# chihyaoma/cyclical-visual-captioning

Hardware: AMD Instinct MI355X
Metric: caption decode-steps/sec (BxT) at N=100,D=2048 (higher is better)
Workload: dtype f32; 1 GPU; cfg2: greedy caption decode; B_per_gpu=64, N=100, F=480, D=2048, A=1024, E=1024, V=5000, T=20, beam=1, hip_graph=True, parallelism=clips sharded over 1 rank(s), no collective, schedule=embedding-gate table (att-LSTM GEMM over K = 2R + one table row per word)

## Files before the change

cyclical-visual-captioning_amd/csrc/blocks.hip:

```cpp
#include <string.h>
#include "cvc_common.h"

namespace {
struct Entry { const char* name; void* fn; };
#define CVC_B(f) {#f, (void*)&f}
const Entry table[] = {
    CVC_B(cvc_attn_scores),
    CVC_B(cvc_attn_wsum),
    CVC_B(cvc_attn_scores_qparts),
    CVC_B(cvc_attn_wsum_quad),
    CVC_B(cvc_attn_wsum_frag),
    CVC_B(cvc_attn_wsum_quad_rm),
    CVC_B(cvc_attn_bwd_pair),
    CVC_B(cvc_ctxfeat_bwd_steps),
    CVC_B(cvc_tile_gemm_big),
    CVC_B(cvc_tile_gemm_plan),
    CVC_B(cvc_dproj_bwd_steps),
    CVC_B(cvc_linear_splitk_fwd),
    CVC_B(cvc_linear_top2_fwd),
    CVC_B(cvc_top2_final),
    CVC_B(cvc_packed_lstm_fwd),
    CVC_B(cvc_packed_linear_fwd),
    CVC_B(cvc_packed_lstm_embgate_fwd),
    CVC_B(cvc_packed_lstm_embgate_ex_fwd),
    CVC_B(cvc_packed_lstm_late_fwd),
    CVC_B(cvc_packed_lstm_train_fwd),
    CVC_B(cvc_packed_lstm_train_pre_fwd),
    CVC_B(cvc_packed_lstm_train_drop_fwd),
    CVC_B(cvc_lstm_pointwise_bwd),
    CVC_B(cvc_lstm_pointwise_bwd3),
    CVC_B(cvc_lstm_pointwise_bwd3_drop),
    CVC_B(cvc_pack_lstm_weights),
    CVC_B(cvc_linear_nn_planes_fwd),
    CVC_B(cvc_linear_nn_planes2_fwd),
    CVC_B(cvc_gru_seq_train_fwd),
    CVC_B(cvc_lstm_pointwise_bwd4_pair),
    CVC_B(cvc_beam_select_parts),
    CVC_B(cvc_sample_select_parts),
    CVC_B(cvc_sample_select_trunc_parts),
    CVC_B(cvc_sample_advance),
    CVC_B(cvc_forced_select_parts),
    CVC_B(cvc_constrained_select_parts),
    CVC_B(cvc_beam_select_hist_parts),
    CVC_B(cvc_beam_select_groups_parts),
    CVC_B(cvc_beam_rank),
    CVC_B(cvc_beam_select_force_parts),
    CVC_B(cvc_beam_rank_force),
    CVC_B(cvc_beam_backtrack_from),
    CVC_B(cvc_tile_lstm_finish),
    CVC_B(cvc_tile_lstm_finish_embgate),
    CVC_B(cvc_tile_reorder_pack),
    CVC_B(cvc_decode_num_launches),
    CVC_B(cvc_gemm_force_generic),
    CVC_B(cvc_tile_gemm_loaders),
    CVC_B(cvc_gru_persistent_waves8),
    CVC_B(cvc_relu_dropout_fwd),
    CVC_B(cvc_relu_dropout_bwd),
    CVC_B(cvc_bn_workspace),
    CVC_B(cvc_bn_relu_train_fwd),
    CVC_B(cvc_bn_relu_train_bwd),
    CVC_B(cvc_class_softmax_bwd),
    CVC_B(cvc_layernorm_cat_bwd),
    CVC_B(cvc_attn_weighted_rows),
    CVC_B(cvc_stable_order),
    CVC_B(cvc_col_sum),
    CVC_B(cvc_col_sum_ws),
    CVC_B(cvc_lstm_persistent_sync_words),
    CVC_B(cvc_lstm_seq_persistent_fwd),
    CVC_B(cvc_lstm_seq_persistent_train_fwd),
    CVC_B(cvc_lstm_seq_fwd),
    CVC_B(cvc_lstm_seq_train_fwd),
    CVC_B(cvc_lstm_seq_bwd_work),
    CVC_B(cvc_lstm_seq_bwd),
    CVC_B(cvc_packed_lstm_bf16w_fwd),
    CVC_B(cvc_packed_linear_bf16w_fwd),
#ifdef CVC_EXPERIMENTAL
    CVC_B(cvc_gsk_plan),
    CVC_B(cvc_gsk_gemm),
    CVC_B(cvc_attn_scores_qslab),
    CVC_B(cvc_top2_slab),
    CVC_B(cvc_packed_lstm_ks_slices),
    CVC_B(cvc_packed_lstm_ks_fwd),
    CVC_B(cvc_packed_lstm_ksf_fwd),
    CVC_B(cvc_packed_lstm_ksx_local),
    CVC_B(cvc_packed_lstm_ksx_fwd),
    CVC_B(cvc_packed_lstm_wg_blocks),
    CVC_B(cvc_packed_linear_select_fwd),
    CVC_B(cvc_gru_persistent_halves),
#endif
};
}

extern "C" void* cvc_block(const char* name) {
    if (name == nullptr) return nullptr;
    for (const Entry& e : table)
        if (strcmp(e.name, name) == 0) return e.fn;
    return nullptr;
}
```

cyclical-visual-captioning_amd/csrc/decode_driver.hip:

```cpp
#include <hip/hip_runtime.h>
#include <new>
#include <stdint.h>
#include "../../include/cvc_hip.h"
#include "../../include/cvc_hip_blocks.h"
#include "../../include/cvc_hip_experimental.h"

struct gsk_launch {
    int U;
    int unit0[2], maxseg[2];
};
struct cvc_decode_plan {
    cvc_decode_desc d;
    int launches;
    gsk_launch ga, go, gl;
};

namespace {

#define CVC_TRY(expr)            \
    do {                         \
        int rc_ = (expr);        \
        ++n;                     \
        if (rc_ != 0) return rc_; \
    } while (0)

inline float* quad_off(float* buf, int k0) { return buf + (size_t)(k0 / 4) * 64 * 4; }
inline void* frag_off(void* xb, int k0) { return (char*)xb + (size_t)(k0 / 16) * 3 * 1024; }

int hip_rc(hipError_t e) { return e == hipSuccess ? 0 : (int)e; }

__global__ __launch_bounds__(256) void reset_kernel(uint4* dst, const uint4* src, size_t n16) {
    const size_t i = (size_t)blockIdx.x * 256 + threadIdx.x;
    if (i < n16) dst[i] = src != nullptr ? src[i] : uint4{0, 0, 0, 0};
}
int reset(void* dst, const void* src, size_t bytes, hipStream_t st) {
    if ((bytes & 15) || ((uintptr_t)dst & 15) || ((uintptr_t)src & 15)) {
        return hip_rc(src ? hipMemcpyAsync(dst, src, bytes, hipMemcpyDeviceToDevice, st) : hipMemsetAsync(dst, 0, bytes, st));
    }
    const size_t n16 = bytes / 16;
    hipLaunchKernelGGL(reset_kernel, dim3((unsigned)((n16 + 255) / 256)), dim3(256), 0, st, (uint4*)dst, (const uint4*)src, n16);
    return hip_rc(hipGetLastError());
}

void attn_sets(const cvc_decode_desc& d, int t, int rows, cvc_attn_set* sets) {
    sets[0] = cvc_attn_set{d.ppool, d.pool, d.mask, nullptr, d.scores_r, nullptr, d.att_steps + (size_t)t * rows * d.N, nullptr,
                           d.N, d.stream_r};
    sets[1] = cvc_attn_set{d.pconv, d.conv, nullptr, nullptr, d.scores_f, nullptr, d.attn_f, nullptr, d.F, d.stream_f};
}

int run_packed(cvc_decode_plan* p, hipStream_t st) {
    const cvc_decode_desc& d = p->d;
    const int rows = d.B, R = d.R, E = d.E, A = d.A, V = d.V, N = d.N;
    const size_t qbytes = (size_t)64 * 4 * sizeof(float);
    int n = 0;
    CVC_TRY(reset(d.xa[0], d.xa0_init, (size_t)((2 * R + E) / 4) * qbytes, st));
    CVC_TRY(reset(d.xl[0], nullptr, (size_t)(3 * R / 4) * qbytes, st));
    CVC_TRY(reset(d.ca[0], nullptr, (size_t)(R / 4) * qbytes, st));
    CVC_TRY(reset(d.cl[0], nullptr, (size_t)(R / 4) * qbytes, st));
    CVC_TRY(reset(d.words, nullptr, (size_t)rows * sizeof(int64_t), st));
    cvc_gemm_seg seg{d.fc, nullptr, d.w_fc, R, R, d.ld_w_fc, 0};
    CVC_TRY(cvc_linear_fwd(&seg, 1, d.b_ih_att, d.b_hh_att, rows, 4 * R, d.gate_fc, 4 * R, st));
    const int nblk_v = (V + 31) / 32;
    for (int t = 0; t < d.T; ++t) {
        const int rd = t & 1, wr = (t + 1) & 1;
        float *XA_r = d.xa[rd], *XA_w = d.xa[wr], *XL_r = d.xl[rd], *XL_w = d.xl[wr];
        CVC_TRY(cvc_packed_lstm_fwd((const float*)d.w_att, XA_r, 2 * R + E, nullptr, nullptr, d.gate_fc, d.ca[rd], rows, R,
                                    quad_off(XL_r, R), quad_off(XA_w, R + E), d.ca[wr], st));
        CVC_TRY(cvc_packed_linear_fwd((const float*)d.w_h, quad_off(XL_r, R), R, nullptr, rows, A, d.qsplit, d.q_parts, A, nullptr, st));
        cvc_attn_set sets[2];
        attn_sets(d, t, rows, sets);
        CVC_TRY(cvc_attn_scores_qparts(d.attn_kind, d.q_parts, d.qsplit, d.b_h, d.w_a, d.b_a, d.inv_temp, sets, 2, d.B, 1, A, st));
        CVC_TRY(cvc_attn_wsum_quad(sets, 2, d.B, 1, R, XL_r, st));
#ifdef CVC_EXPERIMENTAL
        if (d.lang_ksx)
            CVC_TRY(cvc_packed_lstm_ksx_fwd((const float*)d.w_lang, XL_r, 3 * R, d.b_ih_lang, d.b_hh_lang, nullptr, nullptr, nullptr, d.cl[rd],
                                            rows, R, XA_w, quad_off(XL_w, 2 * R), d.cl[wr], d.ksx_slab, d.ksx_flags, (unsigned)(t + 1), st));
        else
#endif
        CVC_TRY(cvc_packed_lstm_fwd((const float*)d.w_lang, XL_r, 3 * R, d.b_ih_lang, d.b_hh_lang, nullptr, d.cl[rd], rows, R, XA_w,
                                    quad_off(XL_w, 2 * R), d.cl[wr], st));
        CVC_TRY(cvc_packed_linear_fwd((const float*)d.w_o, XA_w, R, d.b_o, rows, V, 1, nullptr, V, d.top2_part, st));
        CVC_TRY(cvc_top2_final(d.top2_part, nblk_v, rows, d.unk_idx, d.words + (size_t)(t + 1) * rows, 1,
                               d.logprob ? d.logprob + (size_t)t * rows : nullptr, d.embed, E, quad_off(XA_w, R), 0, st));
    }
    p->launches = n;
    return 0;
}

int run_packed_eg(cvc_decode_plan* p, hipStream_t st) {
    const cvc_decode_desc& d = p->d;
    const int rows = d.B, R = d.R, A = d.A, V = d.V;
    const size_t qbytes = (size_t)64 * 4 * sizeof(float);
    int n = 0;
    CVC_TRY(reset(d.xa[0], nullptr, (size_t)(2 * R / 4) * qbytes, st));
    CVC_TRY(reset(d.xl[0], nullptr, (size_t)(3 * R / 4) * qbytes, st));
    CVC_TRY(reset(d.ca[0], nullptr, (size_t)(R / 4) * qbytes, st));
    CVC_TRY(reset(d.cl[0], nullptr, (size_t)(R / 4) * qbytes, st));
    CVC_TRY(reset(d.words, nullptr, (size_t)rows * sizeof(int64_t), st));
    cvc_gemm_seg seg{d.fc, nullptr, d.w_fc, R, R, d.ld_w_fc, 0};
    CVC_TRY(cvc_linear_fwd(&seg, 1, d.b_ih_att, d.b_hh_att, rows, 4 * R, d.gate_fc, 4 * R, st));
    const long long ws_att = (long long)(2 * R / 4) * 128, ws_lang = (long long)(3 * R / 4) * 128;
    const bool split2 = cvc_gemm_packed_split(-1) == 2;
    for (int t = 0; t < d.T; ++t) {
        const int rd = t & 1, wr = (t + 1) & 1;
        float *XA_r = d.xa[rd], *XA_w = d.xa[wr], *XL_r = d.xl[rd], *XL_w = d.xl[wr];
        const bool first = t == 0 && split2;
        CVC_TRY(cvc_packed_lstm_embgate_ex_fwd((const float*)d.w_att, ws_att, XA_r, first ? 32 : 2 * R, nullptr, nullptr, d.gate_fc,
                                               d.emb_gate, d.words + (size_t)t * rows, d.ca[rd], rows, R, quad_off(XL_r, R),
                                               quad_off(XA_w, R), d.ca[wr], d.att_w_cached, st));
        CVC_TRY(cvc_packed_linear_fwd((const float*)d.w_h, quad_off(XL_r, R), R, nullptr, rows, A, d.qsplit, d.q_parts, A, nullptr, st));
        cvc_attn_set sets[2];
        attn_sets(d, t, rows, sets);
        CVC_TRY(cvc_attn_scores_qparts(d.attn_kind, d.q_parts, d.qsplit, d.b_h, d.w_a, d.b_a, d.inv_temp, sets, 2, d.B, 1, A, st));
        CVC_TRY(cvc_attn_wsum_quad(sets, 2, d.B, 1, R, XL_r, st));
        if (first)
            CVC_TRY(cvc_packed_lstm_late_fwd((const float*)d.w_lang, ws_lang, XL_r, 2 * R, d.b_ih_lang, d.b_hh_lang, nullptr, d.cl[rd], rows,
                                             R, XA_w, quad_off(XL_w, 2 * R), d.cl[wr], nullptr, st));
#ifdef CVC_EXPERIMENTAL
        else if (d.lang_ksx)
            CVC_TRY(cvc_packed_lstm_ksx_fwd((const float*)d.w_lang, XL_r, 3 * R, d.b_ih_lang, d.b_hh_lang, nullptr, nullptr, nullptr, d.cl[rd],
                                            rows, R, XA_w, quad_off(XL_w, 2 * R), d.cl[wr], d.ksx_slab, d.ksx_flags, (unsigned)(t + 1), st));
#endif
        else
        CVC_TRY(cvc_packed_lstm_fwd((const float*)d.w_lang, XL_r, 3 * R, d.b_ih_lang, d.b_hh_lang, nullptr, d.cl[rd], rows, R, XA_w,
                                    quad_off(XL_w, 2 * R), d.cl[wr], st));
        CVC_TRY(cvc_packed_linear_fwd((const float*)d.w_o, XA_w, R, d.b_o, rows, V, 1, nullptr, V, d.top2_part, st));
        CVC_TRY(cvc_top2_final(d.top2_part, (V + 31) / 32, rows, d.unk_idx, d.words + (size_t)(t + 1) * rows, 1,
                               d.logprob ? d.logprob + (size_t)t * rows : nullptr, nullptr, 0, nullptr, 0, st));
    }
    p->launches = n;
    return 0;
}

#ifdef CVC_EXPERIMENTAL
int run_packed_gsk(cvc_decode_plan* p, hipStream_t st) {
    const cvc_decode_desc& d = p->d;
    const int rows = d.B, R = d.R, E = d.E, A = d.A, V = d.V;
    const size_t qbytes = (size_t)64 * 4 * sizeof(float);
    int n = 0;
    CVC_TRY(reset(d.xa[0], d.xa0_init, (size_t)((2 * R + E) / 4) * qbytes, st));
    CVC_TRY(reset(d.xl[0], nullptr, (size_t)(3 * R / 4) * qbytes, st));
    CVC_TRY(reset(d.ca[0], nullptr, (size_t)(R / 4) * qbytes, st));
    CVC_TRY(reset(d.cl[0], nullptr, (size_t)(R / 4) * qbytes, st));
    CVC_TRY(reset(d.words, nullptr, (size_t)rows * sizeof(int64_t), st));
    cvc_gemm_seg seg{d.fc, nullptr, d.w_fc, R, R, d.ld_w_fc, 0};
    CVC_TRY(cvc_linear_fwd(&seg, 1, d.b_ih_att, d.b_hh_att, rows, 4 * R, d.gate_fc, 4 * R, st));
    const long long ws_att = (long long)((2 * R + E) / 4) * 128, ws_lang = (long long)(3 * R / 4) * 128, ws_r = (long long)(R / 4) * 128;
    const float* w_att = (const float*)d.w_att;
    const float* w_lang = (const float*)d.w_lang;
    const int nblk_v = (V + 31) / 32;
    const cvc_gsk_segs seg_att{d.slab_att, p->ga.unit0[0], 2 * R / 32, p->ga.U, p->ga.maxseg[0]};
    const cvc_gsk_segs seg_o_a{d.slab_o, p->ga.unit0[1], R / 32, p->ga.U, p->ga.maxseg[1]};
    const cvc_gsk_segs seg_o_o{d.slab_o, 0, R / 32, p->go.U, p->go.maxseg[0]};
    const cvc_gsk_segs seg_lang{d.slab_lang, p->gl.unit0[0], 2 * R / 32, p->gl.U, p->gl.maxseg[0]};
    const cvc_gsk_segs seg_q{d.slab_q, p->gl.unit0[1], R / 32, p->gl.U, p->gl.maxseg[1]};
    for (int t = 0; t < d.T; ++t) {
        const int rd = t & 1, wr = (t + 1) & 1;
        float *XA_r = d.xa[rd], *XA_w = d.xa[wr], *XL_r = d.xl[rd], *XL_w = d.xl[wr];
        CVC_TRY(cvc_packed_lstm_late_fwd(w_att + (size_t)(R / 4) * 128, ws_att, quad_off(XA_r, R), E, nullptr, nullptr, d.gate_fc,
                                         d.ca[rd], rows, R, quad_off(XL_r, R), quad_off(XA_w, R + E), d.ca[wr],
                                         t == 0 ? nullptr : &seg_att, st));
        cvc_gsk_group gl[2] = {
            {w_lang, ws_lang, XL_r, R / 8, 2 * R / 32, 0, R / 32, d.slab_lang, p->gl.maxseg[0]},
            {(const float*)d.w_h, ws_r, quad_off(XL_r, R), A / 32, R / 32, 0, 0, d.slab_q, p->gl.maxseg[1]}};
        CVC_TRY(cvc_gsk_gemm(gl, 2, p->gl.U, st));
        cvc_attn_set sets[2];
        attn_sets(d, t, rows, sets);
        CVC_TRY(cvc_attn_scores_qslab(d.attn_kind, &seg_q, d.b_h, d.w_a, d.b_a, d.inv_temp, sets, 2, d.B, 1, A, st));
        CVC_TRY(cvc_attn_wsum_quad(sets, 2, d.B, 1, R, XL_r, st));
        CVC_TRY(cvc_packed_lstm_late_fwd(w_lang, ws_lang, XL_r, R, d.b_ih_lang, d.b_hh_lang, nullptr, d.cl[rd], rows, R, XA_w,
                                         quad_off(XL_w, 2 * R), d.cl[wr], &seg_lang, st));
        const bool last = t + 1 == d.T;
        cvc_gsk_group ga[2] = {
            {w_att, ws_att, XA_w, R / 8, 2 * R / 32, R / 32, E / 32, d.slab_att, p->ga.maxseg[0]},
            {(const float*)d.w_o, ws_r, XA_w, nblk_v, R / 32, 0, 0, d.slab_o, last ? p->go.maxseg[0] : p->ga.maxseg[1]}};
        if (last) CVC_TRY(cvc_gsk_gemm(ga + 1, 1, p->go.U, st));
        else CVC_TRY(cvc_gsk_gemm(ga, 2, p->ga.U, st));
        CVC_TRY(cvc_top2_slab(last ? &seg_o_o : &seg_o_a, d.b_o, V, rows, d.unk_idx, d.words + (size_t)(t + 1) * rows, 1,
                              d.logprob ? d.logprob + (size_t)t * rows : nullptr, d.embed, E, quad_off(XA_w, R), 0, st));
    }
    p->launches = n;
    return 0;
}

#endif

int run_tile(cvc_decode_plan* p, hipStream_t st) {
    const cvc_decode_desc& d = p->d;
    const int B = d.B, beam = d.beam, rows = B * beam, R = d.R, E = d.E, A = d.A, V = d.V;
    int n = 0;
    CVC_TRY(reset(d.words, nullptr, (size_t)rows * sizeof(int64_t), st));
    if (beam > 1) {
        CVC_TRY(reset(d.score, nullptr, (size_t)2 * rows * sizeof(float), st));
        CVC_TRY(reset(d.done, nullptr, (size_t)2 * rows, st));
    }
    CVC_TRY(cvc_tile_pack_rows(d.fc, R, nullptr, 0, B, R, d.xff, d.xff_stride, st));
    CVC_TRY(cvc_tile_gemm(d.w_fc_frag, d.xff, d.xff_stride, R, B, 4 * R, d.ks_fc, d.parts_fc, 4 * R, (long long)B * 4 * R, st));
    CVC_TRY(cvc_tile_linear_finish(d.parts_fc, d.ks_fc, (long long)B * 4 * R, 4 * R, d.b_ih_att, d.b_hh_att, B, 4 * R, d.gate_fc,
                                   4 * R, st));
    void* xl_hatt = frag_off(d.xlf, R);
    void* xl_hlang = frag_off(d.xlf, 2 * R);
    const bool eg = d.emb_gate != nullptr;
    const int E_pack = eg ? 0 : E, ka = 2 * R + E_pack;
    CVC_TRY(cvc_tile_reorder_pack(nullptr, d.words, beam, d.zero_state, d.zero_state, d.zero_state, d.zero_state, d.embed, E_pack, V,
                                  d.c_att_prev, d.c_lang_prev, d.xaf, d.xaf_stride, xl_hlang, d.xlf_stride, rows, R, st));
    const long long gs = (long long)rows * 4 * R;
    for (int t = 0; t < d.T; ++t) {
        CVC_TRY(cvc_tile_gemm(d.w_att, d.xaf, d.xaf_stride, ka, rows, 4 * R, d.ks_gate, d.parts_gate, 4 * R, gs, st));
        if (eg)
            CVC_TRY(cvc_tile_lstm_finish_embgate(d.parts_gate, d.ks_gate, gs, nullptr, nullptr, d.gate_fc, beam, d.emb_gate,
                                                 d.words + (size_t)t * rows, V, d.c_att_prev, rows, R, d.c_att, d.h_att, xl_hatt,
                                                 d.xlf_stride, nullptr, 0, st));
        else
            CVC_TRY(cvc_tile_lstm_finish(d.parts_gate, d.ks_gate, gs, nullptr, nullptr, d.gate_fc, beam, d.c_att_prev, rows, R, d.c_att,
                                         d.h_att, xl_hatt, d.xlf_stride, nullptr, 0, st));
        CVC_TRY(cvc_tile_gemm(d.w_h, xl_hatt, d.xlf_stride, R, rows, A, d.ks_q, d.q_parts, A, (long long)rows * A, st));
        CVC_TRY(cvc_tile_linear_finish(d.q_parts, d.ks_q, (long long)rows * A, A, d.b_h, nullptr, rows, A, d.q, A, st));
        cvc_attn_set sets[2];
        attn_sets(d, t, rows, sets);
        CVC_TRY(cvc_attn_scores(d.attn_kind, d.q, d.w_a, d.b_a, d.inv_temp, sets, 2, B, beam, A, st));
        CVC_TRY(cvc_attn_wsum_frag(sets, 2, B, beam, R, d.xlf, d.xlf_stride, st));
        CVC_TRY(cvc_tile_gemm(d.w_lang, d.xlf, d.xlf_stride, 3 * R, rows, 4 * R, d.ks_gate, d.parts_gate, 4 * R, gs, st));
        CVC_TRY(cvc_tile_lstm_finish(d.parts_gate, d.ks_gate, gs, d.b_ih_lang, d.b_hh_lang, nullptr, 1, d.c_lang_prev, rows, R,
                                     d.c_lang, d.h_lang, d.xhf, d.xhf_stride, nullptr, 0, st));
        CVC_TRY(cvc_tile_gemm(d.w_o, d.xhf, d.xhf_stride, R, rows, V, d.ks_o, d.parts_o, V, (long long)rows * V, st));
        static const bool keep_finish = [] { const char* e = getenv("CVC_BEAM_FINISH"); return e && e[0] == '1'; }();
        const bool fused_sel = beam > 1 && !keep_finish && (V & 3) == 0 && (d.ks_o == 2 || d.ks_o == 4 || d.ks_o == 6 || d.ks_o == 8);
        if (!fused_sel)
            CVC_TRY(cvc_tile_linear_finish(d.parts_o, d.ks_o, (long long)rows * V, V, d.b_o, nullptr, rows, V, d.logits, V, st));
        int64_t* word_next = d.words + (size_t)(t + 1) * rows;
        const int64_t* parent = nullptr;
        if (beam == 1) {
            CVC_TRY(cvc_top2_unk(d.logits, rows, V, d.unk_idx, word_next, 1, d.logprob ? d.logprob + (size_t)t * rows : nullptr, st));
        } else {
            const int srd = t & 1, swr = (t + 1) & 1;
            int64_t* par = d.parent + (size_t)t * rows;
            CVC_TRY(cvc_beam_select_parts(fused_sel ? d.parts_o : d.logits, fused_sel ? d.ks_o : 1, fused_sel ? (long long)rows * V : 0,
                                          fused_sel ? d.b_o : nullptr, d.score + (size_t)srd * rows, d.done + (size_t)srd * rows, B, beam, V,
                                          d.unk_idx, t == 0 ? 1 : 0, par, word_next, d.score + (size_t)swr * rows,
                                          d.done + (size_t)swr * rows, d.beam_ws, st));
            parent = par;
        }
        if (t + 1 < d.T)
            CVC_TRY(cvc_tile_reorder_pack(parent, word_next, beam, d.h_att, d.c_att, d.h_lang, d.c_lang, d.embed, E_pack, V, d.c_att_prev,
                                          d.c_lang_prev, d.xaf, d.xaf_stride, xl_hlang, d.xlf_stride, rows, R, st));
    }
    p->launches = n;
    return 0;
}

int validate(const cvc_decode_desc& d) {
    if (d.B < 1 || d.beam < 1 || d.beam > 8 || d.T < 1 || d.N < 1 || d.F < 1 || d.V < 2) return CVC_E_BADARG;
    if (d.attn_kind != CVC_ATTN_ADDITIVE && d.attn_kind != CVC_ATTN_DOT) return CVC_E_BADARG;
    if (!d.fc || !d.conv || !d.pconv || !d.pool || !d.ppool || !d.words || !d.att_steps || !d.embed || !d.b_o || !d.b_h) return CVC_E_BADARG;
    if (d.attn_kind == CVC_ATTN_ADDITIVE && !d.w_a) return CVC_E_BADARG;
    if (!d.w_att || !d.w_lang || !d.w_h || !d.w_o || !d.gate_fc || !d.scores_r || !d.scores_f || !d.attn_f || !d.q_parts) return CVC_E_BADARG;
#ifndef CVC_EXPERIMENTAL
    if (d.gsk_nwg > 0 || d.lang_ksx) return CVC_E_BADARG;
#endif
    if (d.path == 0) {
        if (d.beam != 1 || d.B > 64 || (d.R & 31) || (d.E & 31) || (d.A & 31) || d.qsplit < 1) return CVC_E_BADARG;
        if (!d.w_fc || !d.top2_part || !d.xa[0] || !d.xa[1] || !d.xl[0] || !d.xl[1] || !d.ca[0] || !d.ca[1] || !d.cl[0] || !d.cl[1] ||
            (!d.xa0_init && !d.emb_gate))
            return CVC_E_BADARG;
        if (d.emb_gate != nullptr && d.gsk_nwg > 0) return CVC_E_BADARG;
        if (d.lang_ksx && (!d.ksx_slab || !d.ksx_flags || d.R != 2048 || d.T < 2 || d.gsk_nwg > 0)) return CVC_E_BADARG;
        if (d.gsk_nwg < 0 || (d.gsk_nwg > 0 && ((d.R & 63) || !d.slab_att || !d.slab_lang || !d.slab_q || !d.slab_o))) return CVC_E_BADARG;
    } else if (d.path == 1) {
        if ((d.R & 15) || (d.E & 15) || d.ks_gate < 1 || d.ks_q < 1 || d.ks_o < 1 || d.ks_fc < 1) return CVC_E_BADARG;
        if (!d.w_fc_frag || !d.xaf || !d.xlf || !d.xhf || !d.xff || !d.parts_gate || !d.parts_o || !d.parts_fc || !d.logits || !d.q ||
            !d.h_att || !d.c_att || !d.h_lang || !d.c_lang || !d.c_att_prev || !d.c_lang_prev || !d.zero_state)
            return CVC_E_BADARG;
        if (d.beam > 1 && (!d.score || !d.done || !d.parent || !d.beam_ws)) return CVC_E_BADARG;
    } else {
        return CVC_E_BADARG;
    }
    return 0;
}

}

extern "C" int cvc_decode_plan_create(const cvc_decode_desc* desc, cvc_decode_plan** plan) {
    if (!desc || !plan) return CVC_E_BADARG;
    int rc = validate(*desc);
    if (rc) return rc;
    cvc_decode_plan* p = new (std::nothrow) cvc_decode_plan;
    if (!p) return CVC_E_BADARG;
    p->d = *desc;
    p->launches = 0;
#ifdef CVC_EXPERIMENTAL
    if (desc->path == 0 && desc->gsk_nwg > 0) {
        const int R = desc->R, nt_r = R / 64, nt_v = ((desc->V + 31) / 32 + 7) / 8, nt_a = (desc->A / 32 + 7) / 8;
        const int nta[2] = {nt_r, nt_v}, nca[2] = {2 * R / 32, R / 32};
        const int ntl[2] = {nt_r, nt_a};
        rc = cvc_gsk_plan(nta, nca, 2, desc->gsk_nwg, &p->ga.U, p->ga.unit0, p->ga.maxseg);
        if (!rc) rc = cvc_gsk_plan(nta + 1, nca + 1, 1, desc->gsk_nwg, &p->go.U, p->go.unit0, p->go.maxseg);
        if (!rc) rc = cvc_gsk_plan(ntl, nca, 2, desc->gsk_nwg, &p->gl.U, p->gl.unit0, p->gl.maxseg);
        if (rc) { delete p; return rc; }
    }
#endif
    *plan = p;
    return 0;
}

extern "C" int cvc_decode_plan_set_features(cvc_decode_plan* plan, const float* fc, const float* conv, const float* pconv,
                                            const float* pool, const float* ppool, const uint8_t* mask) {
    if (!plan || !fc || !conv || !pconv || !pool || !ppool) return CVC_E_BADARG;
    plan->d.fc = fc; plan->d.conv = conv; plan->d.pconv = pconv; plan->d.pool = pool; plan->d.ppool = ppool; plan->d.mask = mask;
    return 0;
}

extern "C" void cvc_decode_plan_destroy(cvc_decode_plan* plan) { delete plan; }

extern "C" int cvc_decode_num_launches(const cvc_decode_plan* plan) { return plan ? plan->launches : 0; }

extern "C" int cvc_decode_greedy(cvc_decode_plan* plan, cvc_stream_t stream) {
    if (!plan || plan->d.beam != 1) return CVC_E_BADARG;
    if (plan->d.path == 0) {
        if (plan->d.emb_gate != nullptr) return run_packed_eg(plan, (hipStream_t)stream);
#ifdef CVC_EXPERIMENTAL
        if (plan->d.gsk_nwg > 0) return run_packed_gsk(plan, (hipStream_t)stream);
#endif
        return run_packed(plan, (hipStream_t)stream);
    }
    return run_tile(plan, (hipStream_t)stream);
}

extern "C" int cvc_decode_beam(cvc_decode_plan* plan, cvc_stream_t stream) {
    if (!plan || plan->d.beam < 2 || plan->d.path != 1) return CVC_E_BADARG;
    return run_tile(plan, (hipStream_t)stream);
}
```

cyclical-visual-captioning_amd/csrc/gemm_packed.hip:

```cpp
#include "cvc_common.h"
#include "gemm_split.h"
#include "gsk.h"
#include "dropout_rng.h"

struct PackedArgs {
    const float* wp;
    const float* xq;
    int nquad;
    int M, Nout, R;
    const float* bias;
    const float* bias2;
    const float* gate_bias;
    const float* c_prev_q;
    float* c_out_q;
    float* h_dst1_q;
    float* h_dst2_q;
    float* y;
    int ldy;
    int ksplit;
    long long split_stride;
    float* top2_part;
    const float* c_prev_rm;
    float* h_rm;
    float* c_rm;
    float* gates_rm;
    float* h_rm2;
    float* h_rm3;
    long long gru_w_stride;
    long long gru_h_stride;
    const float* gru_gi[2];
    long long gru_gi_ld;
    float* gru_y[2];
    long long gru_y_ld;
    float* gru_gates[2];
    long long gru_g_ld;
    const float* emb_gate;
    const int64_t* word;
    unsigned* sel_counter;
    int64_t* sel_word; int sel_word_stride; float* sel_logprob; int sel_unk;
    int w_cached;
    DropSpec h3_drop;
    long long wstride;
    GskSegs early;
};

#ifdef CVC_TS
__device__ unsigned long long cvc_ts_buf[2 * 256 * 8 * 4];
extern "C" int cvc_debug_ts_read(unsigned long long* dst) {
    return hipMemcpyFromSymbol(dst, HIP_SYMBOL(cvc_ts_buf), sizeof(cvc_ts_buf)) == hipSuccess ? 0 : -1;
}
#define CVC_TS_MARK(k) do { if (LSTM && !GRU && lane == 0 && blockIdx.x < 256) ts_[k] = wall_clock64(); } while (0)
#else
#define CVC_TS_MARK(k) do {} while (0)
#endif

#ifndef CVC_LIN_W_NT
#define CVC_LIN_W_NT 0
#endif

template <int MT>
struct PFrag {
    f32x4 w[4];
    f32x4 x[MT][4];
#if defined(CVC_PABL) && CVC_PABL == 6
    f32x4 x2[MT][2];
#endif
};
template <int MT>
struct BFrag {
    u32x4 w[2];
    f32x4 x[MT][4];
};

template <int NW>
__device__ __forceinline__ float sum_partials(const float* red, int row, int ldm, int m) {
    float v = (red[(0 * 32 + row) * ldm + m] + red[(1 * 32 + row) * ldm + m]) +
              (red[(2 * 32 + row) * ldm + m] + red[(3 * 32 + row) * ldm + m]);
    if constexpr (NW == 8)
        v += (red[(4 * 32 + row) * ldm + m] + red[(5 * 32 + row) * ldm + m]) +
             (red[(6 * 32 + row) * ldm + m] + red[(7 * 32 + row) * ldm + m]);
    return v;
}

struct SelState { float t1, t2, gm, gs; int j1, j2; };
__device__ __forceinline__ SelState sel_init() { return SelState{-__builtin_inff(), -__builtin_inff(), -__builtin_inff(), 0.f, 0x7fffffff, 0x7fffffff}; }
__device__ __forceinline__ bool sel_better(float va, int ia, float vb, int ib) { return (va > vb) | ((va == vb) & (ia < ib)); }
__device__ __forceinline__ SelState sel_merge(SelState s, float u1, int k1, float u2, int k2, float um, float us) {
    if (sel_better(u1, k1, s.t1, s.j1)) {
        if (sel_better(s.t1, s.j1, u2, k2)) { s.t2 = s.t1; s.j2 = s.j1; } else { s.t2 = u2; s.j2 = k2; }
        s.t1 = u1; s.j1 = k1;
    } else if (sel_better(u1, k1, s.t2, s.j2)) { s.t2 = u1; s.j2 = k1; }
    const float nm = fmaxf(s.gm, um);
    s.gs = (nm == -__builtin_inff()) ? 0.f : s.gs * __expf(s.gm - nm) + us * __expf(um - nm);
    s.gm = nm;
    return s;
}

template <int MT, bool LSTM, int DEPTH, bool SPLIT, int NW, bool GRU = false, int NB = 1, bool SLAB = false, bool WC = false, bool WB16 = false>
__global__ __launch_bounds__(NW * 64) void skinny_gemm_packed_kernel(PackedArgs a) {
    static_assert(!WB16 || (SPLIT && NW == 8 && !GRU && NB == 1 && !SLAB), "bf16-stored weights: 8-wave split-product form only");
    using Frag = std::conditional_t<WB16, BFrag<MT>, PFrag<MT>>;
    using WT = std::conditional_t<WB16, uint16_t, float>;
    static_assert(!GRU || LSTM, "the GRU step shares the LSTM form's work split");
    static_assert(!SLAB || (LSTM && !GRU && NB == 1 && NW == 8), "slab sum: LSTM decode form, 8 waves, one block per workgroup");
    static_assert(NB == 1 || (LSTM && !GRU && NW == 8 && NB == 2), "two blocks per workgroup: LSTM form, 8 waves");
    constexpr int NWK = NW / NB;
    if constexpr (GRU) {
        a.wp += (size_t)blockIdx.y * a.gru_w_stride;
        a.xq += (size_t)blockIdx.y * a.gru_h_stride;
        a.h_dst1_q += (size_t)blockIdx.y * a.gru_h_stride;
        a.bias += (size_t)blockIdx.y * 3 * a.R;
        a.bias2 += (size_t)blockIdx.y * 3 * a.R;
    }
    static_assert(NW == 4 || NW == 8, "4 or 8 waves per workgroup");
    constexpr int LDM = MT * 32 + 1;
    __shared__ float red[(NW + (SLAB ? 1 : 0)) * 32 * LDM + NW * 64 * 6];
    const int tid = threadIdx.x, lane = tid & 63;
    const int wave = __builtin_amdgcn_readfirstlane(tid >> 6);
    const int i = lane & 31, kh = lane >> 5;
    const int M = a.M, R = a.R;
#ifdef CVC_TS
    unsigned long long ts_[4] = {0, 0, 0, 0};
#endif
    CVC_TS_MARK(0);

    int nchunk = a.nquad >> 3, c0 = 0;
    if (!LSTM && a.ksplit > 1) {
        const int lo = nchunk * (int)blockIdx.y / a.ksplit, hi = nchunk * ((int)blockIdx.y + 1) / a.ksplit;
        c0 = lo;
        nchunk = hi - lo;
    }
    const int wblk = NB == 1 ? 0 : wave / NWK, kw = NB == 1 ? wave : wave % NWK;
    const int n_my = nchunk > kw ? (nchunk - kw + NWK - 1) / NWK : 0;
    const WT* wl = reinterpret_cast<const WT*>(a.wp) + (size_t)((int)blockIdx.x * NB + wblk) * a.wstride + (size_t)i * (WB16 ? 8 : 4) +
                   (size_t)(c0 + kw) * 8 * 128 + kh * 4 * 128;
    const float* xl = a.xq + (size_t)i * 4 + (size_t)(c0 + kw) * 8 * 256 + kh * 4 * 256;
    constexpr size_t WSTEP = (size_t)NWK * 8 * 128, XSTEP = (size_t)NWK * 8 * 256;
#ifndef CVC_ROT_MUL
#define CVC_ROT_MUL 5
#endif
    const int rot = n_my > 0 ? (int)((blockIdx.x * CVC_ROT_MUL) % (unsigned)n_my) : 0;

    auto load = [&](Frag& f, int j) __attribute__((always_inline)) {
#if defined(CVC_PABL) && CVC_PABL == 1
        if (j > 0) { asm volatile("" : "+v"(f.w[0])); return; }
#endif
        int jr = j + rot;
        jr = jr >= n_my ? jr - n_my : jr;
        const WT* w = wl + (size_t)jr * WSTEP;
#if defined(CVC_PABL) && CVC_PABL == 4
        const float* x = a.xq + (size_t)i * 4 + kh * 4 * 256;
#else
        const float* x = xl + (size_t)jr * XSTEP;
#endif
        if constexpr (WB16) {
#pragma unroll
            for (int s2 = 0; s2 < 2; ++s2) {
                if constexpr (LSTM && !WC) f.w[s2] = __builtin_nontemporal_load(reinterpret_cast<const u32x4*>(w + s2 * 256));
                else f.w[s2] = *reinterpret_cast<const u32x4*>(w + s2 * 256);
#pragma unroll
                for (int q = 2 * s2; q < 2 * s2 + 2; ++q)
#pragma unroll
                    for (int mt = 0; mt < MT; ++mt) f.x[mt][q] = ld4(x + q * 256 + mt * 128);
            }
        } else {
#pragma unroll
            for (int q = 0; q < 4; ++q) {
                if constexpr (((LSTM && !GRU) || CVC_LIN_W_NT) && !WC) f.w[q] = __builtin_nontemporal_load(reinterpret_cast<const f32x4*>(w + q * 128));
                else f.w[q] = ld4(w + q * 128);
#if defined(CVC_PABL) && CVC_PABL == 3
                if (j > 0) continue;
#endif
#pragma unroll
                for (int mt = 0; mt < MT; ++mt) f.x[mt][q] = ld4(x + q * 256 + mt * 128);
            }
#if defined(CVC_PABL) && CVC_PABL == 6
            {
                int ja = jr + (n_my >> 1);
                ja = ja >= n_my ? ja - n_my : ja;
                const float* xa = xl + (size_t)ja * XSTEP;
#pragma unroll
                for (int s2 = 0; s2 < 2; ++s2)
#pragma unroll
                    for (int mt = 0; mt < MT; ++mt) f.x2[mt][s2] = ld4(xa + (s2 + 2) * 256 + mt * 128 + 64);
            }
#endif
        }
    };

    f32x4 eadd4[4] = {{0, 0, 0, 0}, {0, 0, 0, 0}, {0, 0, 0, 0}, {0, 0, 0, 0}};
    if constexpr (LSTM && !GRU) {
        if (a.emb_gate != nullptr && tid < NB * 2 * 64) {
            const int em0 = tid & 63;
            const long long eword = a.word[em0 < a.M ? em0 : a.M - 1];
            const float* trow = a.emb_gate + (size_t)eword * 4 * a.R + (size_t)((int)blockIdx.x * NB + (tid >> 7)) * 8 + ((tid >> 6) & 1) * 4;
#pragma unroll
            for (int g = 0; g < 4; ++g) eadd4[g] = ld4(trow + (size_t)g * a.R);
        }
    }

    f32x16 acc[MT];
#pragma unroll
    for (int mt = 0; mt < MT; ++mt)
#pragma unroll
        for (int r = 0; r < 16; ++r) acc[mt][r] = 0.f;

    auto mma = [&](const Frag& f) __attribute__((always_inline)) {
        if constexpr (WB16) {
#pragma unroll
            for (int s2 = 0; s2 < 2; ++s2) {
#pragma unroll
                for (int mt = 0; mt < MT; ++mt) {
                    const Split3 X = split8(f.x[mt][2 * s2], f.x[mt][2 * s2 + 1]);
                    acc[mt] = mfma_bf16(f.w[s2], X.lo, acc[mt]);
                    acc[mt] = mfma_bf16(f.w[s2], X.mid, acc[mt]);
                    acc[mt] = mfma_bf16(f.w[s2], X.hi, acc[mt]);
                }
            }
        } else {
#if defined(CVC_PABL) && CVC_PABL >= 2 && CVC_PABL <= 4
#pragma unroll
            for (int q = 0; q < 4; ++q) {
                asm volatile("" ::"v"(f.w[q]));
#pragma unroll
                for (int mt = 0; mt < MT; ++mt) asm volatile("" ::"v"(f.x[mt][q]));
            }
            return;
#endif
            if constexpr (SPLIT) {
#pragma unroll
                for (int s2 = 0; s2 < 2; ++s2) {
                    const Split3 W = split8(f.w[2 * s2], f.w[2 * s2 + 1]);
#pragma unroll
                    for (int mt = 0; mt < MT; ++mt) {
#if defined(CVC_PABL) && (CVC_PABL == 5 || CVC_PABL == 6)
                        Split3 X;
                        X.hi = __builtin_bit_cast(u32x4, f.x[mt][2 * s2]); X.mid = __builtin_bit_cast(u32x4, f.x[mt][2 * s2 + 1]);
#if CVC_PABL == 6
                        X.lo = __builtin_bit_cast(u32x4, f.x2[mt][s2]);
#else
                        X.lo = X.hi;
#endif
#else
                        const Split3 X = split8(f.x[mt][2 * s2], f.x[mt][2 * s2 + 1]);
#endif
                        acc[mt] = mfma_bf16(W.mid, X.mid, acc[mt]);
                        acc[mt] = mfma_bf16(W.lo, X.hi, acc[mt]);
                        acc[mt] = mfma_bf16(W.hi, X.lo, acc[mt]);
                        acc[mt] = mfma_bf16(W.mid, X.hi, acc[mt]);
                        acc[mt] = mfma_bf16(W.hi, X.mid, acc[mt]);
                        acc[mt] = mfma_bf16(W.hi, X.hi, acc[mt]);
                    }
                }
            } else {
#pragma unroll
                for (int q = 0; q < 4; ++q)
#pragma unroll
                    for (int e = 0; e < 4; ++e)
#pragma unroll
                        for (int mt = 0; mt < MT; ++mt)
                            acc[mt] = __builtin_amdgcn_mfma_f32_32x32x2f32(f.w[q][e], f.x[mt][q][e], acc[mt], 0, 0, 0);
            }
        }
    };

    Frag ring[DEPTH];
    if (n_my >= DEPTH) {
#pragma unroll
        for (int s = 0; s < DEPTH - 1; ++s) load(ring[s], s);
        int j = 0;
        for (; j + 2 * DEPTH - 1 <= n_my; j += DEPTH) {
#pragma unroll
            for (int s = 0; s < DEPTH; ++s) {
                load(ring[(s + DEPTH - 1) % DEPTH], j + s + DEPTH - 1);
                mma(ring[s]);
#ifdef CVC_TS
                if (s == 0 && j == 0) CVC_TS_MARK(1);
// ... 15 lines not shown
#pragma unroll
                    for (int g = 0; g < 4 + 4 * MT; ++g) {
                        __builtin_amdgcn_sched_group_barrier(0x002, 18, 0);
                        __builtin_amdgcn_sched_group_barrier(0x008, MT, 0);
                        __builtin_amdgcn_sched_group_barrier(0x020, 1, 0);
                    }
                } else {
#pragma unroll
                    for (int g = 0; g < 4 + 4 * MT; ++g) {
                        __builtin_amdgcn_sched_group_barrier(0x008, 2, 0);
                        __builtin_amdgcn_sched_group_barrier(0x020, 1, 0);
                        __builtin_amdgcn_sched_group_barrier(0x002, 2, 0);
                    }
                }
                __builtin_amdgcn_sched_barrier(0);
            }
        }
#pragma unroll
        for (int s = 0; s < DEPTH; ++s) {
            if (j + s + DEPTH - 1 < n_my) load(ring[(s + DEPTH - 1) % DEPTH], j + s + DEPTH - 1);
            if (j + s < n_my) mma(ring[s]);
        }
#pragma unroll
        for (int s = 0; s < DEPTH - 1; ++s)
            if (j + DEPTH + s < n_my) mma(ring[s]);
    } else {
        for (int j = 0; j < n_my; ++j) {
            load(ring[0], j);
            mma(ring[0]);
        }
    }

    CVC_TS_MARK(2);
    const int em = tid & 63, eqd = (tid >> 6) & 1, eb = tid >> 7;
    const bool ework = LSTM && tid < NB * 2 * 64 && em < M && em < MT * 32;
    const int ejq = ((int)blockIdx.x * NB + eb) * 8 + eqd * 4;
    const float* ered = red + (NB == 1 ? 0 : eb * NWK * 32 * LDM);
    const size_t eqoff = ((size_t)(ejq / 4) * 64 + em) * 4;
    f32x4 ecp = {0, 0, 0, 0}, eadd[4] = {{0, 0, 0, 0}, {0, 0, 0, 0}, {0, 0, 0, 0}, {0, 0, 0, 0}};
    f32x4 eadd2[4] = {{0, 0, 0, 0}, {0, 0, 0, 0}, {0, 0, 0, 0}, {0, 0, 0, 0}}, eadd3[4] = {{0, 0, 0, 0}, {0, 0, 0, 0}, {0, 0, 0, 0}, {0, 0, 0, 0}};

    if (GRU && ework) {
        const float* gi = (blockIdx.y == 0 ? a.gru_gi[0] : a.gru_gi[1]) + (size_t)em * a.gru_gi_ld + ejq;
        ecp = ld4(a.xq + eqoff);
#pragma unroll
        for (int g = 0; g < 3; ++g) {
            eadd[g] = ld4(gi + g * R) + ld4(a.bias + g * R + ejq);
            if (g < 2) eadd[g] += ld4(a.bias2 + g * R + ejq);
        }
        eadd[3] = ld4(a.bias2 + 2 * R + ejq);
    } else if (ework) {
        ecp = a.c_prev_rm != nullptr ? ld4(a.c_prev_rm + (size_t)em * R + ejq) : ld4(a.c_prev_q + eqoff);
        if (a.bias != nullptr) {
#pragma unroll
            for (int g = 0; g < 4; ++g) eadd[g] = ld4(a.bias + g * R + ejq);
        }
        if (a.bias2 != nullptr) {
#pragma unroll
            for (int g = 0; g < 4; ++g) eadd2[g] = ld4(a.bias2 + g * R + ejq);
        }
        if (a.gate_bias != nullptr) {
#pragma unroll
            for (int g = 0; g < 4; ++g) eadd3[g] = ld4(a.gate_bias + (size_t)em * 4 * R + g * R + ejq);
        }
    }

    constexpr int SLAB_MAXS = 10;
    f32x4 sv[SLAB ? SLAB_MAXS : 1];
    int s_nseg = 0;
    const float* s_p0 = nullptr;
    if constexpr (SLAB) {
        const int tile = (int)blockIdx.x >> 3, j = (int)blockIdx.x & 7;
        s_nseg = gsk_nseg(a.early, tile);
        s_p0 = gsk_part(a.early, tile, 0, j) + (size_t)tid * 4;
#pragma unroll
        for (int s = 0; s < SLAB_MAXS; ++s) sv[s] = ld4(s_p0 + (size_t)(s < s_nseg ? s : s_nseg - 1) * (8 * 2048));
    }

    constexpr int ECPW = 32 / NW;
    float ebias[ECPW];
#pragma unroll
    for (int c = 0; c < ECPW; ++c) {
        const int n = (int)blockIdx.x * 32 + wave * ECPW + c;
        ebias[c] = (!LSTM && a.top2_part != nullptr && a.bias != nullptr) ? a.bias[n < a.Nout ? n : a.Nout - 1] : 0.f;
    }

#pragma unroll
    for (int mt = 0; mt < MT; ++mt)
#pragma unroll
        for (int r = 0; r < 16; ++r) {
            const int row = (r & 3) + 8 * (r >> 2) + 4 * kh;
            red[(wave * 32 + row) * LDM + mt * 32 + i] = acc[mt][r];
        }
    if constexpr (SLAB) {
        f32x4 t = sv[0];
#pragma unroll
        for (int s = 1; s < SLAB_MAXS; ++s) t += s < s_nseg ? sv[s] : f32x4{0.f, 0.f, 0.f, 0.f};
        for (int s = SLAB_MAXS; s < s_nseg; ++s) t += ld4(s_p0 + (size_t)s * (8 * 2048));
        if ((tid >> 3) < MT * 32) {
#pragma unroll
            for (int e = 0; e < 4; ++e) red[(NW * 32 + (tid & 7) * 4 + e) * LDM + (tid >> 3)] = t[e];
        }
    }
    __syncthreads();

    if constexpr (GRU) {
        if (ework) {
            f32x4 hv, gr, gz, gn, gh;
#pragma unroll
            for (int e = 0; e < 4; ++e) {
                const int jj = eqd * 4 + e;
                float pre[3];
#pragma unroll
                for (int g = 0; g < 3; ++g) pre[g] = sum_partials<NWK>(ered, g * 8 + jj, LDM, em);
                const float rg = fast_sigmoid(pre[0] + eadd[0][e]), zg = fast_sigmoid(pre[1] + eadd[1][e]);
                const float hn = pre[2] + eadd[3][e];
                const float ng = fast_tanh(eadd[2][e] + rg * hn);
                hv[e] = ng + zg * (ecp[e] - ng);
                gr[e] = rg; gz[e] = zg; gn[e] = ng; gh[e] = hn;
            }
            st4(a.h_dst1_q + eqoff, hv);
            st4((blockIdx.y == 0 ? a.gru_y[0] : a.gru_y[1]) + (size_t)em * a.gru_y_ld + ejq, hv);
            float* gp = blockIdx.y == 0 ? a.gru_gates[0] : a.gru_gates[1];
            if (gp != nullptr) {
                gp += (size_t)em * a.gru_g_ld + ejq;
                st4(gp, gr); st4(gp + a.R, gz); st4(gp + 2 * a.R, gn); st4(gp + 3 * a.R, gh);
            }
        }
    } else if (LSTM) {
        if (ework) {
            f32x4 hv, cv, gv[4];
#pragma unroll
            for (int g = 0; g < 4; ++g) eadd[g] = ((eadd[g] + eadd2[g]) + eadd3[g]) + eadd4[g];
#pragma unroll
            for (int e = 0; e < 4; ++e) {
                const int jj = eqd * 4 + e;
                float pre[4];
#pragma unroll
                for (int g = 0; g < 4; ++g) {
                    float sp = sum_partials<NWK>(ered, g * 8 + jj, LDM, em);
                    if constexpr (SLAB) sp += red[(NW * 32 + g * 8 + jj) * LDM + em];
                    pre[g] = sp + eadd[g][e];
                }
                const float ig = fast_sigmoid(pre[0]), fg = fast_sigmoid(pre[1]);
                const float gg = fast_tanh(pre[2]), og = fast_sigmoid(pre[3]);
                const float c2 = fg * ecp[e] + ig * gg;
                cv[e] = c2;
                hv[e] = og * fast_tanh(c2);
                gv[0][e] = ig; gv[1][e] = fg; gv[2][e] = gg; gv[3][e] = og;
            }
            if (a.c_out_q != nullptr) st4(a.c_out_q + eqoff, cv);
            if (a.h_dst1_q != nullptr) st4(a.h_dst1_q + eqoff, hv);
            if (a.h_dst2_q != nullptr) st4(a.h_dst2_q + eqoff, hv);
            if (a.h_rm != nullptr) st4(a.h_rm + (size_t)em * R + ejq, hv);
            if (a.h_rm2 != nullptr) st4(a.h_rm2 + (size_t)em * R + ejq, hv);
            if (a.h_rm3 != nullptr) {
                f32x4 hd = hv;
                if (a.h3_drop.state != nullptr) {
                    const uint32_t s0 = a.h3_drop.state[0], s1 = a.h3_drop.state[1], s2 = a.h3_drop.state[2];
                    const uint32_t i0 = (uint32_t)em * (uint32_t)R + (uint32_t)ejq;
#pragma unroll
                    for (int e = 0; e < 4; ++e) hd[e] *= cvc_drop_mult(a.h3_drop, s0, s1, s2, i0 + e);
                }
                st4(a.h_rm3 + (size_t)em * R + ejq, hd);
            }
            if (a.c_rm != nullptr) st4(a.c_rm + (size_t)em * R + ejq, cv);
            if (a.gates_rm != nullptr) {
#pragma unroll
                for (int g = 0; g < 4; ++g) st4(a.gates_rm + (size_t)em * 4 * R + g * R + ejq, gv[g]);
            }
        }
#ifdef CVC_TS
        asm volatile("s_waitcnt vmcnt(0)" ::: "memory");
        CVC_TS_MARK(3);
        if (lane == 0 && blockIdx.x < 256) {
            unsigned long long* d = cvc_ts_buf + ((size_t)((a.nquad >= 1536 ? 0 : 1) * 256 + blockIdx.x) * 8 + wave) * 4;
            d[0] = ts_[0]; d[1] = ts_[1]; d[2] = ts_[2]; d[3] = ts_[3];
        }
#endif
    } else {
        const int n0 = blockIdx.x * 32;
        const bool lead = blockIdx.y == 0;
        float* y = a.y != nullptr ? a.y + (long long)blockIdx.y * a.split_stride : nullptr;
        if (y != nullptr) {
            for (int u = tid; u < 32 * MT * 32; u += NW * 64) {
                const int nl = u & 31, m = u >> 5;
                const int n = n0 + nl;
                if (m >= M || n >= a.Nout) continue;
                float v = sum_partials<NW>(red, nl, LDM, m);
                if (lead && a.bias != nullptr) v += a.bias[n];
                y[(size_t)m * a.ldy + n] = v;
            }
        }
        if (a.top2_part != nullptr) {
            float* scratch = red + NW * 32 * LDM;
            float v1 = -__builtin_inff(), v2 = -__builtin_inff(), mx = -__builtin_inff(), se = 0.f;
            int i1 = 0x7fffffff, i2 = 0x7fffffff;
            const int m = lane < MT * 32 ? lane : MT * 32 - 1;
            constexpr int CPW = 32 / NW;
#pragma unroll
            for (int c = 0; c < CPW; ++c) {
                const int nl = wave * CPW + c, n = n0 + nl;
                if (n >= a.Nout) break;
                const float v = sum_partials<NW>(red, nl, LDM, m) + ebias[c];
                if (v > v1) { v2 = v1; i2 = i1; v1 = v; i1 = n; }
                else if (v > v2) { v2 = v; i2 = n; }
                const float nm = fmaxf(mx, v);
                se = se * __expf(mx - nm) + __expf(v - nm);
                mx = nm;
            }
            float* r4 = scratch + ((size_t)wave * 64 + lane) * 6;
            r4[0] = v1; r4[1] = __int_as_float(i1); r4[2] = v2; r4[3] = __int_as_float(i2); r4[4] = mx; r4[5] = se;
            __syncthreads();
            if (wave == 0 && lane < M) {
                for (int w = 1; w < NW; ++w) {
                    const float* q4 = scratch + ((size_t)w * 64 + lane) * 6;
                    const float u1 = q4[0], u2 = q4[2];
                    const int k1 = __float_as_int(q4[1]), k2 = __float_as_int(q4[3]);
                    if (u1 > v1) { if (v1 >= u2) { v2 = v1; i2 = i1; } else { v2 = u2; i2 = k2; } v1 = u1; i1 = k1; }
                    else if (u1 > v2) { v2 = u1; i2 = k1; }
                    const float nm = fmaxf(mx, q4[4]);
                    se = (nm == -__builtin_inff()) ? 0.f : se * __expf(mx - nm) + q4[5] * __expf(q4[4] - nm);
                    mx = nm;
                }
                float* rec = a.top2_part + ((size_t)blockIdx.x * 64 + lane) * 6;
                if (a.sel_counter != nullptr) {
                    const float r6[6] = {v1, __int_as_float(i1), v2, __int_as_float(i2), mx, se};
#pragma unroll
                    for (int k = 0; k < 6; ++k) __hip_atomic_store(rec + k, r6[k], __ATOMIC_RELAXED, __HIP_MEMORY_SCOPE_AGENT);
                } else {
                    rec[0] = v1; rec[1] = __int_as_float(i1); rec[2] = v2; rec[3] = __int_as_float(i2); rec[4] = mx; rec[5] = se;
                }
            }
            if (a.sel_counter != nullptr) {
                asm volatile("s_waitcnt vmcnt(0)" ::: "memory");
                __syncthreads();
                int* flag = reinterpret_cast<int*>(scratch);
                if (tid == 0) {
                    const unsigned old = __hip_atomic_fetch_add(a.sel_counter, 1u, __ATOMIC_RELAXED, __HIP_MEMORY_SCOPE_AGENT);
                    const bool last = old == gridDim.x - 1;
                    if (last) {
                        __hip_atomic_store(a.sel_counter, 0u, __ATOMIC_RELAXED, __HIP_MEMORY_SCOPE_AGENT);
                        __builtin_amdgcn_fence(__ATOMIC_ACQUIRE, "agent");
                    }
                    flag[0] = last ? 1 : 0;
                }
                __syncthreads();
                if (flag[0] == 0) return;
                __syncthreads();
                const int nb = (int)gridDim.x;
                SelState ss = sel_init();
                const int mrow = lane < M ? lane : M - 1;
                constexpr int RB = 8;
                for (int b0 = wave; b0 < nb; b0 += NW * RB) {
                    f32x2 r0[RB], r1[RB], r2[RB];
#pragma unroll
                    for (int k = 0; k < RB; ++k) {
                        const int b = b0 + k * NW;
                        const f32x2* q2 = reinterpret_cast<const f32x2*>(a.top2_part + ((size_t)(b < nb ? b : nb - 1) * 64 + mrow) * 6);
                        r0[k] = q2[0]; r1[k] = q2[1]; r2[k] = q2[2];
                    }
#pragma unroll
                    for (int k = 0; k < RB; ++k)
                        if (b0 + k * NW < nb) ss = sel_merge(ss, r0[k].x, __float_as_int(r0[k].y), r1[k].x, __float_as_int(r1[k].y), r2[k].x, r2[k].y);
                }
                float* r8 = scratch + ((size_t)wave * 64 + lane) * 6;
                r8[0] = ss.t1; r8[1] = __int_as_float(ss.j1); r8[2] = ss.t2; r8[3] = __int_as_float(ss.j2); r8[4] = ss.gm; r8[5] = ss.gs;
                __syncthreads();
                if (wave == 0 && lane < M) {
                    for (int w = 1; w < NW; ++w) {
                        const float* q4 = scratch + ((size_t)w * 64 + lane) * 6;
                        ss = sel_merge(ss, q4[0], __float_as_int(q4[1]), q4[2], __float_as_int(q4[3]), q4[4], q4[5]);
                    }
                    const bool use2 = (ss.j1 == a.sel_unk) && ss.j2 != 0x7fffffff;
                    int wsel = use2 ? ss.j2 : ss.j1;
                    if (wsel == 0x7fffffff || wsel < 0) wsel = 0;
                    a.sel_word[(size_t)lane * a.sel_word_stride] = wsel;
// ... 308 lines not shown
    long long ldx[6];
    int nseg, M;
    float* xq;
};

__global__ __launch_bounds__(256) void pack_quad_segs_kernel(PackXArgs a) {
    const int t = blockIdx.x * 256 + threadIdx.x;
    const int m = t & 63, q = t >> 6;
    if (q >= a.q_end[a.nseg - 1]) return;
    int s = 0;
#pragma unroll
    for (int i = 0; i < 5; ++i) s += (i < a.nseg - 1 && q >= a.q_end[i]) ? 1 : 0;
    const int qs = q - (s ? a.q_end[s - 1] : 0);
    f32x4 v = {0, 0, 0, 0};
    if (m < a.M) v = ld4(a.x[s] + (size_t)m * a.ldx[s] + qs * 4);
    st4(a.xq + ((size_t)q * 64 + m) * 4, v);
}

}

extern "C" int cvc_pack_lstm_segs(const float* const* ws, const long long* lds, const int* widths, int nseg, int R, float* wp,
                                  cvc_stream_t stream) {
    if (!ws || !lds || !widths || !wp || nseg < 1 || nseg > 4 || R < 8 || (R & 7)) return CVC_E_BADARG;
    PackWArgs a{};
    int q = 0;
    for (int s = 0; s < nseg; ++s) {
        if (!ws[s] || widths[s] < 4 || (widths[s] & 3) || lds[s] < widths[s] || (lds[s] & 3) || ((uintptr_t)ws[s] & 15)) return CVC_E_BADARG;
        q += widths[s] / 4;
        a.w[s] = ws[s]; a.ld[s] = lds[s]; a.q_end[s] = q;
    }
    if (q & 7) return CVC_E_BADARG;
    a.nseg = nseg; a.R = R; a.wp = wp;
    hipLaunchKernelGGL(pack_lstm_w_kernel, dim3(R / 8, (q + 63) / 64), dim3(256), 0, (hipStream_t)stream, a);
    return cvc_launch_status();
}

extern "C" int cvc_pack_lstm_weights(const float* w_ih, int K_ih, const float* w_hh, int K_hh, int R, float* wp,
                                     cvc_stream_t stream) {
    if (!w_ih || !w_hh || !wp || K_ih < 4 || K_hh < 4 || (K_ih & 3) || (K_hh & 3) || ((K_ih + K_hh) & 31) || R < 8 || (R & 7))
        return CVC_E_BADARG;
    const float* ws[2] = {w_ih, w_hh};
    const long long lds[2] = {K_ih, K_hh};
    const int widths[2] = {K_ih, K_hh};
    return cvc_pack_lstm_segs(ws, lds, widths, 2, R, wp, stream);
}

extern "C" int cvc_pack_quad_segs(const float* const* xs, const long long* ldx, const int* widths, int nseg, int M, float* xq,
                                  cvc_stream_t stream) {
    if (!xs || !ldx || !widths || !xq || nseg < 1 || nseg > 6 || M < 1 || M > 64) return CVC_E_BADARG;
    PackXArgs a{};
    int q = 0;
    for (int s = 0; s < nseg; ++s) {
        if (!xs[s] || widths[s] < 4 || (widths[s] & 3) || (ldx[s] & 3) || ((uintptr_t)xs[s] & 15)) return CVC_E_BADARG;
        q += widths[s] / 4;
        a.x[s] = xs[s]; a.ldx[s] = ldx[s]; a.q_end[s] = q;
    }
    a.nseg = nseg; a.M = M; a.xq = xq;
    hipLaunchKernelGGL(pack_quad_segs_kernel, dim3((q * 64 + 255) / 256), dim3(256), 0, (hipStream_t)stream, a);
    return cvc_launch_status();
}

extern "C" int cvc_packed_linear_select_fwd(const float* wp, const float* xq, int K, const float* bias, int M, int Nout,
                                            float* top2_part, unsigned* counter, int unk_idx, int64_t* word, int word_stride,
                                            float* logprob, cvc_stream_t stream) {
    if (!wp || !xq || (K & 31) || Nout < 2 || !top2_part || !counter || !word || word_stride < 1 || M < 1 || M > 64) return CVC_E_BADARG;
    PackedArgs a{};
    a.wp = wp; a.xq = xq; a.nquad = K / 4; a.M = M; a.Nout = Nout; a.R = 0;
    a.bias = bias; a.ksplit = 1; a.top2_part = top2_part;
    a.sel_counter = counter; a.sel_unk = unk_idx; a.sel_word = word; a.sel_word_stride = word_stride; a.sel_logprob = logprob;
    return launch_packed<false>(a, (Nout + 31) / 32, (hipStream_t)stream);
}

extern "C" int cvc_packed_linear_fwd(const float* wp, const float* xq, int K, const float* bias, int M, int Nout,
                                     int ksplit, float* y, int ldy, float* top2_part, cvc_stream_t stream) {
    if (!wp || !xq || (K & 31) || Nout < 1 || ksplit < 1 || (!y && !top2_part)) return CVC_E_BADARG;
    if (ksplit > 1 && top2_part != nullptr) return CVC_E_BADARG;
    if (y != nullptr && ldy < Nout) return CVC_E_BADARG;
    PackedArgs a{};
    a.wp = wp; a.xq = xq; a.nquad = K / 4; a.M = M; a.Nout = Nout; a.R = 0;
    a.bias = bias; a.y = y; a.ldy = ldy; a.ksplit = ksplit; a.split_stride = (long long)M * ldy; a.top2_part = top2_part;
    return launch_packed<false>(a, (Nout + 31) / 32, (hipStream_t)stream);
}

extern "C" int cvc_packed_linear_bf16w_fwd(const uint16_t* wp, const float* xq, int K, const float* bias, int M, int Nout,
                                           int ksplit, float* y, int ldy, float* top2_part, cvc_stream_t stream) {
    if (!wp || !xq || (K & 31) || K < 32 || Nout < 1 || ksplit < 1 || (!y && !top2_part) || M < 1 || M > 64) return CVC_E_BADARG;
    if (ksplit > 1 && top2_part != nullptr) return CVC_E_BADARG;
    if (y != nullptr && ldy < Nout) return CVC_E_BADARG;
    if (((uintptr_t)wp & 15) || ((uintptr_t)xq & 15)) return CVC_E_BADARG;
    PackedArgs a{};
    a.wp = reinterpret_cast<const float*>(wp); a.xq = xq; a.nquad = K / 4; a.M = M; a.Nout = Nout; a.R = 0;
    a.bias = bias; a.y = y; a.ldy = ldy; a.ksplit = ksplit; a.split_stride = (long long)M * ldy; a.top2_part = top2_part;
    return launch_packed_bf16w<false>(a, (Nout + 31) / 32, (hipStream_t)stream);
}
```

cyclical-visual-captioning_amd/csrc/vocab.hip:

```cpp
#include "row_block.h"
#include "gsk.h"
#include "dropout_rng.h"
#include <math.h>

namespace {

__global__ __launch_bounds__(WG) void embed_relu_fwd_kernel(const float* table, const int64_t* idx, const float* drop, DropSpec rng,
                                                            int M, int E, float* out) {
    const int m = blockIdx.y;
    const int e = (blockIdx.x * WG + threadIdx.x) * 4;
    if (e >= E) return;
    f32x4 v = ld4(table + (size_t)idx[m] * E + e);
    v.x = fmaxf(v.x, 0.f); v.y = fmaxf(v.y, 0.f); v.z = fmaxf(v.z, 0.f); v.w = fmaxf(v.w, 0.f);
    if (drop != nullptr) v *= ld4(drop + (size_t)m * E + e);
    if (rng.state != nullptr) {
        const uint32_t s0 = rng.state[0], s1 = rng.state[1], s2 = rng.state[2], i0 = (uint32_t)m * (uint32_t)E + (uint32_t)e;
#pragma unroll
        for (int k = 0; k < 4; ++k) v[k] *= cvc_drop_mult(rng, s0, s1, s2, i0 + k);
    }
    st4(out + (size_t)m * E + e, v);
}

__global__ __launch_bounds__(WG) void dropout_rng_kernel(const float* x, DropSpec rng, size_t n, float* y) {
    const size_t i = ((size_t)blockIdx.x * WG + threadIdx.x) * 4;
    if (i >= n) return;
    const uint32_t s0 = rng.state[0], s1 = rng.state[1], s2 = rng.state[2];
    if (i + 4 <= n) {
        f32x4 v = ld4(x + i);
#pragma unroll
        for (int k = 0; k < 4; ++k) v[k] *= cvc_drop_mult(rng, s0, s1, s2, (uint32_t)(i + k));
        st4(y + i, v);
    } else {
        for (size_t k = i; k < n; ++k) y[k] = x[k] * cvc_drop_mult(rng, s0, s1, s2, (uint32_t)k);
    }
}

constexpr int EMB_CHUNK = 16;

__global__ __launch_bounds__(WG) void embed_bwd_pieces_kernel(const int64_t* idx, const int64_t* order, const float* drop, DropSpec rng,
                                                              const float* d_out, int M, int E, float* part) {
    const int r0 = blockIdx.y * EMB_CHUNK;
    const int e = (blockIdx.x * WG + threadIdx.x) * 4;
    if (e >= E) return;
    const int r1 = min(M, r0 + EMB_CHUNK);
    int start = r0;
    int64_t w = idx[order[r0]];
    f32x4 acc = {0, 0, 0, 0};
    for (int r = r0; r < r1; ++r) {
        const int64_t m = order[r];
        const int64_t wr = idx[m];
        if (wr != w) {
            st4(part + (size_t)start * E + e, acc);
            acc = f32x4{0, 0, 0, 0};
            start = r;
            w = wr;
        }
        f32x4 g = ld4(d_out + (size_t)m * E + e);
        if (drop != nullptr) g *= ld4(drop + (size_t)m * E + e);
        if (rng.state != nullptr) {
            const uint32_t s0 = rng.state[0], s1 = rng.state[1], s2 = rng.state[2], i0 = (uint32_t)m * (uint32_t)E + (uint32_t)e;
#pragma unroll
            for (int k = 0; k < 4; ++k) g[k] *= cvc_drop_mult(rng, s0, s1, s2, i0 + k);
        }
        acc += g;
    }
    st4(part + (size_t)start * E + e, acc);
}

__global__ __launch_bounds__(WG) void embed_bwd_runs_kernel(const float* table, const int64_t* idx, const int64_t* order,
                                                            const float* part, int M, int E, float* d_table) {
    const int r0 = blockIdx.y;
    const int64_t w = idx[order[r0]];
    if (r0 > 0 && idx[order[r0 - 1]] == w) return;
    const int e = (blockIdx.x * WG + threadIdx.x) * 4;
    if (e >= E) return;
    f32x4 acc = ld4(part + (size_t)r0 * E + e);
    for (int r = (r0 / EMB_CHUNK + 1) * EMB_CHUNK; r < M && idx[order[r]] == w; r += EMB_CHUNK)
        acc += ld4(part + (size_t)r * E + e);
    const f32x4 t = ld4(table + (size_t)w * E + e);
    acc.x = t.x > 0.f ? acc.x : 0.f; acc.y = t.y > 0.f ? acc.y : 0.f;
    acc.z = t.z > 0.f ? acc.z : 0.f; acc.w = t.w > 0.f ? acc.w : 0.f;
    st4(d_table + (size_t)w * E + e, ld4(d_table + (size_t)w * E + e) + acc);
}
// ... 49 lines not shown
    const int row = blockIdx.x;
    const float* x = logits + (size_t)row * V;
    Top2 t{-INFINITY, 0x7fffffff, -INFINITY, 0x7fffffff};
    for (int v = threadIdx.x; v < V; v += WG) {
        const float xv = x[v];
        if (better(xv, v, t.v1, t.i1)) { t.v2 = t.v1; t.i2 = t.i1; t.v1 = xv; t.i1 = v; }
        else if (better(xv, v, t.v2, t.i2)) { t.v2 = xv; t.i2 = v; }
    }
#pragma unroll
    for (int o = 32; o > 0; o >>= 1) {
        Top2 u;
        u.v1 = __shfl_xor(t.v1, o, 64); u.i1 = __shfl_xor(t.i1, o, 64);
        u.v2 = __shfl_xor(t.v2, o, 64); u.i2 = __shfl_xor(t.i2, o, 64);
        t = merge(t, u);
    }
    const int lane = threadIdx.x & 63, wave = threadIdx.x >> 6;
    if (lane == 0) tred[wave] = t;
    __syncthreads();
    t = merge(merge(tred[0], tred[1]), merge(tred[2], tred[3]));
    const float m = t.v1;
    float s = 0.f;
    for (int v = threadIdx.x; v < V; v += WG) s += expf(x[v] - m);
    s = block_sum(s, red);
    if (threadIdx.x == 0) {
        const bool use2 = (t.i1 == unk) && V > 1;
        int w = use2 ? t.i2 : t.i1;
        if ((unsigned)w >= (unsigned)V) w = 0;
        word[(size_t)row * wstride] = w;
        if (logprob != nullptr) logprob[row] = (use2 ? t.v2 : t.v1) - (m + logf(s));
    }
}

__global__ __launch_bounds__(WG) void top2_final_kernel(const float* part, int nblocks, int unk, int64_t* word, int wstride,
                                                        float* logprob, const float* table, int E, float* emb_out, int emb_ld) {
    __shared__ float red[4];
    __shared__ Top2 tred[4];
    __shared__ int chosen;
    const int row = blockIdx.x;
    Top2 t{-INFINITY, 0x7fffffff, -INFINITY, 0x7fffffff};
    float mx = -INFINITY;
    for (int b = threadIdx.x; b < nblocks; b += WG) {
        const float* rec = part + ((size_t)b * 64 + row) * 6;
        Top2 u{rec[0], __float_as_int(rec[1]), rec[2], __float_as_int(rec[3])};
        t = merge(t, u);
        mx = fmaxf(mx, rec[4]);
    }
#pragma unroll
    for (int o = 32; o > 0; o >>= 1) {
        Top2 u;
        u.v1 = __shfl_xor(t.v1, o, 64); u.i1 = __shfl_xor(t.i1, o, 64);
        u.v2 = __shfl_xor(t.v2, o, 64); u.i2 = __shfl_xor(t.i2, o, 64);
        t = merge(t, u);
    }
    const int lane = threadIdx.x & 63, wave = threadIdx.x >> 6;
    if (lane == 0) tred[wave] = t;
    mx = block_max(mx, red);
    t = merge(merge(tred[0], tred[1]), merge(tred[2], tred[3]));
    float se = 0.f;
    for (int b = threadIdx.x; b < nblocks; b += WG) {
        const float* rec = part + ((size_t)b * 64 + row) * 6;
        se += rec[5] * expf(rec[4] - mx);
    }
    se = block_sum(se, red);
    if (threadIdx.x == 0) {
        const bool use2 = (t.i1 == unk) && t.i2 != 0x7fffffff;
        int w = use2 ? t.i2 : t.i1;
        if (w == 0x7fffffff || w < 0) w = 0;
        word[(size_t)row * wstride] = w;
        if (logprob != nullptr) logprob[row] = (use2 ? t.v2 : t.v1) - (mx + logf(se));
        chosen = w;
    }
    if (emb_out != nullptr) {
        __syncthreads();
        const float* src = table + (size_t)chosen * E;
        for (int e = threadIdx.x * 4; e < E; e += WG * 4) {
            f32x4 v = ld4(src + e);
            v.x = fmaxf(v.x, 0.f); v.y = fmaxf(v.y, 0.f); v.z = fmaxf(v.z, 0.f); v.w = fmaxf(v.w, 0.f);
            if (emb_ld > 0) st4(emb_out + (size_t)row * emb_ld + e, v);
            else st4(emb_out + ((size_t)(e >> 2) * 64 + row) * 4, v);
        }
    }
}

template <int ITEMS>
__global__ __launch_bounds__(WG) void top2_slab_kernel(GskSegs g, const float* bias, int V, int unk, int64_t* word, int wstride,
                                                       float* logprob, const float* table, int E, float* emb_out, int emb_ld) {
    __shared__ float red[4];
    __shared__ Top2 tred[4];
    __shared__ int chosen;
    constexpr int MAXS = 6;
    const int row = blockIdx.x;
    const int nitem = ((V + 31) >> 5) * 8;
    f32x4 sv[ITEMS][MAXS], bv[ITEMS];
    int nseg[ITEMS], col0[ITEMS];
    const float* p0[ITEMS];
#pragma unroll
    for (int k = 0; k < ITEMS; ++k) {
        const int it = min((int)threadIdx.x + k * WG, nitem - 1);
        const int blk = it >> 3, rq = it & 7;
        nseg[k] = gsk_nseg(g, blk >> 3);
        col0[k] = (int)threadIdx.x + k * WG < nitem ? blk * 32 + rq * 4 : V;
        p0[k] = gsk_part(g, blk >> 3, 0, blk & 7) + (size_t)row * 32 + rq * 4;
#pragma unroll
        for (int s = 0; s < MAXS; ++s) sv[k][s] = ld4(p0[k] + (size_t)(s < nseg[k] ? s : nseg[k] - 1) * (8 * 2048));
#pragma unroll
        for (int e = 0; e < 4; ++e) bv[k][e] = (bias != nullptr && col0[k] + e < V) ? bias[col0[k] + e] : 0.f;
    }
    Top2 t{-INFINITY, 0x7fffffff, -INFINITY, 0x7fffffff};
    float mx = -INFINITY;
    f32x4 val[ITEMS];
#pragma unroll
    for (int k = 0; k < ITEMS; ++k) {
        f32x4 x = sv[k][0];
#pragma unroll
        for (int s = 1; s < MAXS; ++s) x += s < nseg[k] ? sv[k][s] : f32x4{0.f, 0.f, 0.f, 0.f};
        for (int s = MAXS; s < nseg[k]; ++s) x += ld4(p0[k] + (size_t)s * (8 * 2048));
        x += bv[k];
#pragma unroll
        for (int e = 0; e < 4; ++e) {
            const int v = col0[k] + e;
            const float xv = v < V ? x[e] : -INFINITY;
            val[k][e] = xv;
            if (v < V) {
                if (better(xv, v, t.v1, t.i1)) { t.v2 = t.v1; t.i2 = t.i1; t.v1 = xv; t.i1 = v; }
                else if (better(xv, v, t.v2, t.i2)) { t.v2 = xv; t.i2 = v; }
                mx = fmaxf(mx, xv);
            }
        }
    }
#pragma unroll
    for (int o = 32; o > 0; o >>= 1) {
        Top2 u;
        u.v1 = __shfl_xor(t.v1, o, 64); u.i1 = __shfl_xor(t.i1, o, 64);
        u.v2 = __shfl_xor(t.v2, o, 64); u.i2 = __shfl_xor(t.i2, o, 64);
        t = merge(t, u);
    }
    const int lane = threadIdx.x & 63, wave = threadIdx.x >> 6;
    if (lane == 0) tred[wave] = t;
    mx = block_max(mx, red);
    t = merge(merge(tred[0], tred[1]), merge(tred[2], tred[3]));
    float se = 0.f;
#pragma unroll
    for (int k = 0; k < ITEMS; ++k)
#pragma unroll
        for (int e = 0; e < 4; ++e) se += val[k][e] == -INFINITY ? 0.f : expf(val[k][e] - mx);
    se = block_sum(se, red);
    if (threadIdx.x == 0) {
        const bool use2 = (t.i1 == unk) && t.i2 != 0x7fffffff;
        int w = use2 ? t.i2 : t.i1;
        if (w == 0x7fffffff || w < 0) w = 0;
        word[(size_t)row * wstride] = w;
        if (logprob != nullptr) logprob[row] = (use2 ? t.v2 : t.v1) - (mx + logf(se));
        chosen = w;
    }
    if (emb_out != nullptr) {
        __syncthreads();
        const float* src = table + (size_t)chosen * E;
        for (int e = threadIdx.x * 4; e < E; e += WG * 4) {
            f32x4 v = ld4(src + e);
            v.x = fmaxf(v.x, 0.f); v.y = fmaxf(v.y, 0.f); v.z = fmaxf(v.z, 0.f); v.w = fmaxf(v.w, 0.f);
            if (emb_ld > 0) st4(emb_out + (size_t)row * emb_ld + e, v);
            else st4(emb_out + ((size_t)(e >> 2) * 64 + row) * 4, v);
        }
    }
}

// ... 126 lines not shown
    hipLaunchKernelGGL(embed_relu_fwd_kernel, dim3((E / 4 + WG - 1) / WG, M), dim3(WG), 0, (hipStream_t)stream, table, idx,
                       drop, rng, M, E, out);
    return cvc_launch_status();
}

static int embed_bwd_impl(const float* table, const int64_t* idx, const int64_t* order, const float* drop, DropSpec rng,
                          const float* d_out, int M, int E, float* d_table, float* workspace, cvc_stream_t stream) {
    if (!table || !idx || !order || !d_out || !d_table || !workspace || M < 1 || E < 4 || (E & 3)) return CVC_E_BADARG;
    const int gx = (E / 4 + WG - 1) / WG;
    hipLaunchKernelGGL(embed_bwd_pieces_kernel, dim3(gx, (M + EMB_CHUNK - 1) / EMB_CHUNK), dim3(WG), 0, (hipStream_t)stream, idx,
                       order, drop, rng, d_out, M, E, workspace);
    hipLaunchKernelGGL(embed_bwd_runs_kernel, dim3(gx, M), dim3(WG), 0, (hipStream_t)stream, table, idx, order, workspace, M, E,
                       d_table);
    return cvc_launch_status();
}

extern "C" int cvc_embed_relu_fwd(const float* table, const int64_t* idx, const float* drop, int M, int E, float* out,
                                  cvc_stream_t stream) {
    return embed_fwd_impl(table, idx, drop, cvc_drop_spec(nullptr, 0, 0.f), M, E, out, stream);
}

extern "C" int cvc_embed_relu_bwd(const float* table, const int64_t* idx, const int64_t* order, const float* drop,
                                  const float* d_out, int M, int E, float* d_table, float* workspace, cvc_stream_t stream) {
    return embed_bwd_impl(table, idx, order, drop, cvc_drop_spec(nullptr, 0, 0.f), d_out, M, E, d_table, workspace, stream);
}

extern "C" int cvc_embed_relu_rng_fwd(const float* table, const int64_t* idx, const uint32_t* rng_state, unsigned site, float p, int M,
                                      int E, float* out, cvc_stream_t stream) {
    if (!rng_state || p < 0.f || p >= 1.f) return CVC_E_BADARG;
    return embed_fwd_impl(table, idx, nullptr, cvc_drop_spec(rng_state, site, p), M, E, out, stream);
}

extern "C" int cvc_embed_relu_rng_bwd(const float* table, const int64_t* idx, const int64_t* order, const uint32_t* rng_state,
                                      unsigned site, float p, const float* d_out, int M, int E, float* d_table, float* workspace,
                                      cvc_stream_t stream) {
    if (!rng_state || p < 0.f || p >= 1.f) return CVC_E_BADARG;
    return embed_bwd_impl(table, idx, order, nullptr, cvc_drop_spec(rng_state, site, p), d_out, M, E, d_table, workspace, stream);
}

extern "C" int cvc_dropout_rng(const float* x, long long n, const uint32_t* rng_state, unsigned site, float p, float* y,
                               cvc_stream_t stream) {
    if (!x || !y || !rng_state || n < 1 || n > 0xffffffffll || p < 0.f || p >= 1.f || ((uintptr_t)x & 15) || ((uintptr_t)y & 15))
        return CVC_E_BADARG;
    hipLaunchKernelGGL(dropout_rng_kernel, dim3((unsigned)((n / 4 + WG) / WG)), dim3(WG), 0, (hipStream_t)stream, x,
                       cvc_drop_spec(rng_state, site, p), (size_t)n, y);
    return cvc_launch_status();
}

extern "C" int cvc_log_softmax_fwd(const float* logits, int M, int V, float* logp, cvc_stream_t stream) {
    if (!logits || !logp || M < 1 || V < 1) return CVC_E_BADARG;
    hipLaunchKernelGGL(log_softmax_kernel, dim3(M), dim3(WG), 0, (hipStream_t)stream, logits, V, logp);
    return cvc_launch_status();
}

extern "C" int cvc_log_softmax_bwd(const float* logp, const float* d_logp, int M, int V, float* d_logits,
                                   cvc_stream_t stream) {
    if (!logp || !d_logp || !d_logits || M < 1 || V < 1) return CVC_E_BADARG;
    hipLaunchKernelGGL(log_softmax_bwd_kernel, dim3(M), dim3(WG), 0, (hipStream_t)stream, logp, d_logp, V, d_logits);
    return cvc_launch_status();
}

extern "C" int cvc_nll_bwd(const int64_t* target, const float* w, const float* g, int M, int V, float* d_logp,
                           cvc_stream_t stream) {
    if (!target || !w || !g || !d_logp || M < 1 || V < 1) return CVC_E_BADARG;
    hipLaunchKernelGGL(nll_bwd_kernel, dim3((V + WG - 1) / WG, M), dim3(WG), 0, (hipStream_t)stream, target, w, g, V, d_logp);
    return cvc_launch_status();
}

extern "C" int cvc_top2_unk(const float* logits, int M, int V, int unk_idx, int64_t* word, int word_stride,
                            float* logprob, cvc_stream_t stream) {
    if (!logits || !word || M < 1 || V < 1 || word_stride < 1) return CVC_E_BADARG;
    hipLaunchKernelGGL(top2_unk_kernel, dim3(M), dim3(WG), 0, (hipStream_t)stream, logits, V, unk_idx, word, word_stride,
                       logprob);
    return cvc_launch_status();
}

extern "C" int cvc_top2_final(const float* part, int nblocks, int M, int unk_idx, int64_t* word, int word_stride,
                              float* logprob, const float* table, int E, float* emb_out, int emb_ld,
                              cvc_stream_t stream) {
    if (!part || !word || nblocks < 1 || M < 1 || M > 64 || word_stride < 1) return CVC_E_BADARG;
    if (emb_out != nullptr && (!table || E < 4 || (E & 3) || (emb_ld & 3) || (emb_ld != 0 && emb_ld < E))) return CVC_E_BADARG;
    hipLaunchKernelGGL(top2_final_kernel, dim3(M), dim3(WG), 0, (hipStream_t)stream, part, nblocks, unk_idx, word, word_stride,
                       logprob, table, E, emb_out, emb_ld);
    return cvc_launch_status();
}

extern "C" int cvc_top2_slab(const cvc_gsk_segs* logits, const float* bias, int V, int M, int unk_idx, int64_t* word,
                             int word_stride, float* logprob, const float* table, int E, float* emb_out, int emb_ld,
                             cvc_stream_t stream) {
    if (!logits || !logits->slab || logits->nchunk < 1 || logits->U < 1 || logits->maxseg < 1 || logits->unit0 < 0 || !word || V < 2 ||
        M < 1 || M > 64 || word_stride < 1)
        return CVC_E_BADARG;
    if (emb_out != nullptr && (!table || E < 4 || (E & 3) || (emb_ld & 3) || (emb_ld != 0 && emb_ld < E))) return CVC_E_BADARG;
    const int nitem = ((V + 31) / 32) * 8;
    hipStream_t st = (hipStream_t)stream;
    if (nitem <= 5 * WG)
        hipLaunchKernelGGL(top2_slab_kernel<5>, dim3(M), dim3(WG), 0, st, *logits, bias, V, unk_idx, word, word_stride, logprob, table, E,
                           emb_out, emb_ld);
    else if (nitem <= 8 * WG)
        hipLaunchKernelGGL(top2_slab_kernel<8>, dim3(M), dim3(WG), 0, st, *logits, bias, V, unk_idx, word, word_stride, logprob, table, E,
                           emb_out, emb_ld);
    else
        return CVC_E_TOOBIG;
    return cvc_launch_status();
}

extern "C" int cvc_nll_fwd(const float* logp, const int64_t* target, const float* w, int M, int V, float* loss_sum,
                           cvc_stream_t stream) {
    if (!logp || !target || !w || !loss_sum || M < 1 || V < 1) return CVC_E_BADARG;
    hipLaunchKernelGGL(nll_fwd_kernel, dim3(1), dim3(WG), 0, (hipStream_t)stream, logp, target, w, M, V, loss_sum);
    return cvc_launch_status();
}

extern "C" int cvc_vocab_nll_fwd(const float* logits, const int64_t* target, const float* w, int M, int V, float* lse,
                                 int64_t* argmax, float* row_loss, float* loss_sum, cvc_stream_t stream) {
    if (!logits || !target || !w || !lse || !row_loss || !loss_sum || M < 1 || V < 1) return CVC_E_BADARG;
    hipLaunchKernelGGL(vocab_nll_fwd_kernel, dim3(M), dim3(WG), 0, (hipStream_t)stream, logits, target, w, V, lse, argmax,
                       row_loss);
    hipLaunchKernelGGL(row_sum_kernel, dim3(1), dim3(WG), 0, (hipStream_t)stream, row_loss, M, loss_sum);
    return cvc_launch_status();
}

extern "C" int cvc_vocab_head_nll_fwd(const float* parts, int nparts, long long part_stride, int ld, const float* bias,
                                      const int64_t* target, const float* w, int M, int V, float* pre, int ld_pre, int64_t* argmax,
                                      float* row_loss, float* loss_sum, cvc_stream_t stream) {
    if (!parts || nparts < 1 || !target || !w || !pre || !row_loss || !loss_sum || M < 1 || V < 1 || V > WG * NLL_CACHE || ld < V ||
        ld_pre < V)
        return CVC_E_BADARG;
    hipLaunchKernelGGL(vocab_head_nll_kernel, dim3(M), dim3(WG), 0, (hipStream_t)stream, parts, nparts, part_stride, ld, bias, target, w, V,
                       pre, ld_pre, argmax, row_loss);
    hipLaunchKernelGGL(row_sum_kernel, dim3(1), dim3(WG), 0, (hipStream_t)stream, row_loss, M, loss_sum);
    return cvc_launch_status();
}

extern "C" int cvc_vocab_nll_bwd(const float* logits, const float* lse, const int64_t* target, const float* w,
                                 const float* g, int M, int V, float* d_logits, cvc_stream_t stream) {
    if (!logits || !lse || !target || !w || !g || !d_logits || M < 1 || V < 1) return CVC_E_BADARG;
    hipLaunchKernelGGL(vocab_nll_bwd_kernel, dim3((V + WG - 1) / WG, M), dim3(WG), 0, (hipStream_t)stream, logits, lse,
                       target, w, g, V, d_logits);
    return cvc_launch_status();
}
```

cyclical-visual-captioning_amd/cvc/decode/engine.py:

```python
from __future__ import annotations

import ctypes as C
import os
from typing import Dict, List, Optional, Tuple


import numpy as np
import torch

from .. import hip
from .weights import *
from .weights import _segs
from .path_packed import PackedPath
from .path_tile import TilePath
from .path_ring import RingPath
from .path_experimental import ExperimentalPaths

CONSTRAINT_T_MAX = 64
CONSTRAINT_LIST_MAX = 256


def _constraints(no_repeat_ngram, no_immediate_repeat, min_len, ban_words, bad_endings):
    is_int = lambda v: isinstance(v, (int, np.integer)) and not isinstance(v, bool)
    for name, v, hi in (("no_repeat_ngram", no_repeat_ngram, CONSTRAINT_T_MAX), ("min_len", min_len, None)):
        if not is_int(v) or v < 0 or (hi is not None and v > hi):
            raise RuntimeError(f"DecodeEngine: {name} must be an integer >= 0 (0 = off)" + (f" and <= {hi}" if hi else "") + f", got {v!r}")
    if not isinstance(no_immediate_repeat, (bool, np.bool_)) and no_immediate_repeat not in (0, 1):
        raise RuntimeError(f"DecodeEngine: no_immediate_repeat must be a bool, got {no_immediate_repeat!r}")
    lists = []
    for name, ids in (("ban_words", ban_words), ("bad_endings", bad_endings)):
        ids = [] if ids is None else list(ids) if isinstance(ids, (list, tuple, set, frozenset, np.ndarray)) else None
        if ids is None or not all(is_int(v) and v >= 0 for v in ids):
            raise RuntimeError(f"DecodeEngine: {name} must be a list of word ids (integers >= 0), got {ban_words if name == 'ban_words' else bad_endings!r}")
        ids = tuple(sorted({int(v) for v in ids}))
        if len(ids) > CONSTRAINT_LIST_MAX:
            raise RuntimeError(f"DecodeEngine: {name} takes at most {CONSTRAINT_LIST_MAX} ids, got {len(ids)}")
        lists.append(ids)
    return int(no_repeat_ngram), bool(no_immediate_repeat), int(min_len), lists[0], lists[1]


def _capture_mode() -> str:
    import torch.distributed as dist
    if dist.is_available() and dist.is_initialized() and dist.get_backend() == "nccl":
        return "thread_local"
    return "global"


class DecodeEngine(PackedPath, TilePath, RingPath, ExperimentalPaths):
    _warm = set()

    def __init__(self, weights: DecodeWeights, feats: Dict[str, torch.Tensor], T: int, unk_idx: int, beam: int = 1,
                 inv_temp: float = 1.0, own_features: bool = False, path: str = "auto", gate_ksplit: Optional[bool] = None,
                 driver: bool = True, gsk: Optional[bool] = None, embgate: Optional[bool] = None, lang_ksx: Optional[bool] = None,
                 sample_n: int = 1, temperature: Optional[float] = None, seed: Optional[int] = None, weights_dtype: str = "fp32",
                 top_k: int = 0, top_p: float = 1.0, forced_n: int = 0, no_repeat_ngram: int = 0, no_immediate_repeat: bool = False,
                 min_len: int = 0, ban_words=None, bad_endings=None, beam_groups: int = 1, diversity: float = 0.0,
                 length_penalty: float = 0.0, force_n: int = 0, beam_history: bool = False):
        W = self.W = weights
        self.T, self.unk, self.beam = int(T), int(unk_idx), int(beam)
        if weights_dtype not in WEIGHTS_DTYPES:
            raise RuntimeError(f"DecodeEngine: weights_dtype must be one of {WEIGHTS_DTYPES}, got {weights_dtype!r}")
        self.weights_dtype = weights_dtype
        self.bf16w = weights_dtype == "bf16"
        if isinstance(forced_n, bool) or not isinstance(forced_n, (int, np.integer)) or forced_n < 0:
            raise RuntimeError(f"DecodeEngine: forced_n must be an integer >= 0 (0 = off), got {forced_n!r}")
        self.forced = int(forced_n) >= 1
        if self.forced:
            if self.beam != 1:
                raise RuntimeError("DecodeEngine: the forced mode (forced_n) and beam search (beam > 1) exclude each other")
            if temperature is not None:
                raise RuntimeError("DecodeEngine: the forced mode (forced_n) follows given words: it takes no sampling temperature")
            if gsk or gate_ksplit or lang_ksx:
                raise RuntimeError("DecodeEngine: the forced mode runs on the default schedules only (no gsk / gate_ksplit / lang_ksx)")
            gate_ksplit, lang_ksx = False, False
        self.cons = _constraints(no_repeat_ngram, no_immediate_repeat, min_len, ban_words, bad_endings)
        self.constrained = bool(self.cons[0] or self.cons[1] or self.cons[2] or self.cons[3] or self.cons[4])
        if not isinstance(beam_history, (bool, np.bool_)):
            raise RuntimeError(f"DecodeEngine: beam_history must be a bool, got {beam_history!r}")
        self.beam_hist = bool(beam_history)
        if self.beam_hist:
            if self.beam == 1:
                raise RuntimeError("DecodeEngine: beam_history keeps the histories of beam search: it needs beam > 1")
            if self.T > CONSTRAINT_T_MAX:
                raise RuntimeError(f"DecodeEngine: beam_history covers T <= {CONSTRAINT_T_MAX} steps, got T = {self.T}")
            if gsk or gate_ksplit or lang_ksx:
                raise RuntimeError("DecodeEngine: beam_history runs on the default schedules only (no gsk / gate_ksplit / lang_ksx)")
        if isinstance(beam_groups, bool) or not isinstance(beam_groups, (int, np.integer)) or beam_groups < 1:
            raise RuntimeError(f"DecodeEngine: beam_groups must be an integer >= 1 (1 = off), got {beam_groups!r}")
        if not (0.0 <= float(diversity) < float("inf")):
            raise RuntimeError(f"DecodeEngine: diversity must be a finite number >= 0 (negative values are refused), got {diversity!r}")
        if not (0.0 <= float(length_penalty) < float("inf")):
            raise RuntimeError(f"DecodeEngine: length_penalty must be a finite number >= 0, got {length_penalty!r}")
        self.groups, self.diversity, self.length_penalty = int(beam_groups), float(diversity), float(length_penalty)
        self.grouped = self.groups > 1
        if isinstance(force_n, bool) or not isinstance(force_n, (int, np.integer)) or not 0 <= force_n <= 3:
            raise RuntimeError(f"DecodeEngine: force_n must be an integer in 0 .. 3 (0 = off), got {force_n!r}")
        self.force_n = int(force_n)
        self.forcing = self.force_n >= 1
        if self.forcing:
            if self.beam == 1:
                raise RuntimeError("DecodeEngine: force_n is an option of beam search: it needs beam > 1")
            if not self.beam_hist:
                raise RuntimeError("DecodeEngine: force_n needs beam_history=True (the forced words a hypothesis has met are read from "
                                   "its own history)")
            if self.beam % (self.force_n + 1) != 0:
                raise RuntimeError(f"DecodeEngine: force_n = {self.force_n} needs beam % (force_n + 1) == 0 (one bank per number of "
                                   f"forced words met), got beam = {self.beam}")
            if self.grouped:
                raise RuntimeError("DecodeEngine: force_n and beam_groups > 1 exclude each other (banks and groups both divide the "
                                   "clip's slots)")
        self.ranked = self.grouped or self.length_penalty != 0.0 or self.forcing
        if self.ranked:
            what = "beam_groups > 1" if self.grouped else "length_penalty != 0"
            if self.beam == 1:
                raise RuntimeError(f"DecodeEngine: {what} is an option of beam search: it needs beam > 1")
            if not self.beam_hist:
                raise RuntimeError(f"DecodeEngine: {what} needs beam_history=True (the groups and the ranking read the hypotheses' "
                                   "own histories)")
            if self.beam % self.groups != 0:
                raise RuntimeError(f"DecodeEngine: beam_groups = {self.groups} must divide beam = {self.beam}")
        if self.diversity != 0.0 and not self.grouped:
            raise RuntimeError("DecodeEngine: diversity acts between groups: it needs beam_groups > 1")
        if self.constrained:
            if self.beam != 1 and not self.beam_hist:
                raise RuntimeError("DecodeEngine: constrained decoding under beam search (beam > 1) needs beam_history=True (a "
                                   "hypothesis' history follows its parents: it has to travel with it)")
            if self.forced:
                raise RuntimeError("DecodeEngine: the forced mode (forced_n) follows given words: it takes no constraints")
            if gsk or gate_ksplit or lang_ksx:
                raise RuntimeError("DecodeEngine: constrained decoding runs on the default schedules only (no gsk / gate_ksplit / lang_ksx)")
            if self.T > CONSTRAINT_T_MAX:
                raise RuntimeError(f"DecodeEngine: constrained decoding covers T <= {CONSTRAINT_T_MAX} steps, got T = {self.T}")
            bad = [v for v in self.cons[3] + self.cons[4] if v >= W.V]
            if bad:
                raise RuntimeError(f"DecodeEngine: ban_words / bad_endings ids outside [0, V = {W.V}): {bad}")
            gate_ksplit, lang_ksx = False, False
        if self.bf16w:
            why = None
            if self.beam != 1:
                why = f"beam search (beam = {self.beam}) runs on the tile path"
# ... 86 lines not shown
        if self.sampling:
            self.rng = torch.zeros(4, device=dev, dtype=torch.int32)
            self.seed(0 if seed is None else seed)
        if self.forced:
            self.rank = torch.zeros(self.T, rows, dtype=torch.int32, device=dev)
            self.fmask = self.fm_steps = None
        if self.trunc:
            self.cutoff = z(self.T, rows)
            self.kept = torch.zeros(self.T, rows, dtype=torch.int32, device=dev)
        if self.constrained:
            n_, imm_, len_, ban_, bad_ = self.cons
            i32 = lambda ids: torch.tensor(list(ids) or [0], dtype=torch.int32, device=dev)
            self.nbanned = torch.zeros(self.T, rows, dtype=torch.int32, device=dev)
            self.ban_ids, self.bad_ids = i32(ban_), i32(bad_)
            self._cons_desc = hip.Constraint(n_, int(imm_), len_, len(ban_), self.ban_ids.data_ptr(), self.bad_ids.data_ptr(), len(bad_))
        if self.beam > 1:
            self.score = z(2, rows)
            self.done = torch.zeros(2, rows, dtype=torch.uint8, device=dev)
            self.parent = torch.zeros(self.T, rows, dtype=torch.int64, device=dev)
            self.bt_seq = torch.zeros(self.B, self.T, dtype=torch.int64, device=dev)
            self.bt_att = z(self.B, self.T, N)
            self.gather_tmp = [z(rows, R) for _ in range(4)]
            self.beam_ws = z((21 if self.forcing else 17) * rows)
            if self.beam_hist:
                self.bhist = torch.zeros(2, self.T, rows, dtype=torch.int64, device=dev)
            if self.ranked:
                self.order = torch.zeros(self.B, self.beam, dtype=torch.int64, device=dev)
                self.norm = z(self.B, self.beam)
                self.hyp_len = torch.zeros(self.B, self.beam, dtype=torch.int32, device=dev)
            if self.forcing:
                self.force_words = torch.full((self.B, self.force_n), -1, dtype=torch.int32, device=dev)
                self.nmet = torch.zeros(self.T, rows, dtype=torch.int32, device=dev)
                self.final_nmet = torch.zeros(self.B, self.beam, dtype=torch.int32, device=dev)
        self.inv_temp = float(inv_temp)
        self.graph: Optional[torch.cuda.CUDAGraph] = None
        self._keep: List = []
        self.packed = packed
        self.gate_ksplit = GATE_KSPLIT_DEFAULT if gate_ksplit is None else gate_ksplit
        self.gate_fused = self.gate_ksplit == "fused"
        self.gate_ksplit = bool(self.gate_ksplit)
        gsk_ok = self.packed and R % 64 == 0 and not self.gate_ksplit and hip.gemm_packed_split(-1) == 2
        if gsk and not gsk_ok:
            raise RuntimeError("DecodeEngine: the stream-K schedule needs the packed path, R % 64 == 0 and cvc_gemm_packed_split(2)")
        self.gsk = False if gsk is None else bool(gsk)
        self.tile = (not self.packed) and (self.nq > 1 or rows > 64 or path == "tile") and R % 16 == 0 and W.E % 16 == 0 and path != "ring"
        eg_ok = (self.packed and not self.gsk and not self.gate_ksplit) or self.tile
        if embgate and not eg_ok:
            raise RuntimeError("DecodeEngine: the embedding-gate schedule needs the packed path (without gsk / gate_ksplit) or the tile path")
        self.embgate = (eg_ok and 4 * V * 4 * R <= EMBGATE_MAX_BYTES) if embgate is None else bool(embgate)
        if self.given and self.packed and not self.embgate:
            raise RuntimeError(f"DecodeEngine: {'sampling' if self.sampling else 'the forced mode' if self.forced else 'constrained decoding'} on the packed path needs the "
                               "embedding-gate schedule (the attention cell reads the word from words[t])")
        if self.bf16w and not (self.packed and self.embgate):
            raise RuntimeError('DecodeEngine: weights_dtype="bf16" needs the embedding-gate schedule, and its table '
                               f"({4 * V * 4 * R} bytes) is over EMBGATE_MAX_BYTES")
        bpw = 2 if self.bf16w else 4
        keep = cache_plan(bpw * (V * R + A * R), {"ppool": nb(ppool), "pconv": nb(pconv), "pool": nb(pool), "conv": nb(conv)},
                          gate_weight_bytes=bpw * 4 * R * 2 * R if (self.packed and self.embgate and (rows > 32 or self.bf16w)) else None,
                          lang_weight_bytes=bpw * 4 * R * 3 * R if self.bf16w else None)
        self.cache_keep = keep
        self.att_w_cached = bool(keep.get("att_w", False))
        self.lang_w_cached = bool(keep.get("lang_w", False))
        self.stream_r = (0 if keep["ppool"] else 1) | (0 if keep["pool"] else 2)
        self.stream_f = (0 if keep["pconv"] else 1) | (0 if keep["conv"] else 2)
        self._plan = None
        self._driver = driver
        exp = hip.experimental_built()
        if not exp and (self.gsk or self.gate_ksplit or lang_ksx):
            raise RuntimeError("DecodeEngine: gsk / gate_ksplit / lang_ksx are experimental schedules (include/cvc_hip_experimental.h): "
                               "this libcvc_hip.so was built without CVC_EXPERIMENTAL=1")
        ksx_ok = (exp and self.packed and not self.gsk and not self.gate_ksplit and R == 2048 and self.T > 1 and
                  hip.gemm_packed_split(-1) == 2 and int(hip.lib().cvc_packed_lstm_ks_slices(3 * R, R)) == 8)
        if lang_ksx and not ksx_ok:
            raise RuntimeError("DecodeEngine: lang_ksx needs the packed path at R = 2048, T > 1, split-product arithmetic")
        self.lang_ksx = ksx_ok and not self.bf16w and (LANG_KSX_DEFAULT if lang_ksx is None else bool(lang_ksx))
        self._ksx_checked = False
        if self.lang_ksx:
            self.ksx_slab = torch.empty(8 * (R // 8) * 2048, device=dev, dtype=torch.float32)
            self.ksx_flags = torch.zeros(R // 8 + 1, device=dev, dtype=torch.int32)
        if self.packed:
            self._alloc_packed()
        elif self.tile:
            self._alloc_tile()
        self._launches = self._build_launches()
        if driver and not self.given and not self.bf16w and not self.beam_hist and (self.tile or (self.packed and not (self.ks_att or self.ks_lang))):
            self._bind_driver()


    def _bind_driver(self):
        W, L = self.W, hip.lib()
        ptr = lambda t: None if t is None else t.data_ptr()
        d = hip.DecodeDesc()
        d.B, d.beam, d.T, d.N, d.F, d.R, d.A, d.E, d.V = self.B, self.beam, self.T, self.N, self.F, W.R, W.A, W.E, W.V
        d.unk_idx, d.attn_kind, d.inv_temp = self.unk, W.kind, self.inv_temp
        d.stream_r, d.stream_f = self.stream_r, self.stream_f
        for k in ("b_ih_att", "b_hh_att", "b_ih_lang", "b_hh_lang", "b_h", "w_a", "b_a", "b_o", "embed"):
            setattr(d, k, ptr(getattr(W, k)))
        fc, conv, pconv, pool, ppool = self.feats
        d.fc, d.conv, d.pconv, d.pool, d.ppool, d.mask = ptr(fc), ptr(conv), ptr(pconv), ptr(pool), ptr(ppool), ptr(self.mask)
        d.words, d.att_steps, d.logprob = ptr(self.words), ptr(self.att_steps), ptr(self.logprob)
        d.scores_r, d.scores_f, d.attn_f = ptr(self.scores_r), ptr(self.scores_f), ptr(self.attn_f)
        if self.packed:
            R = W.R
            d.path, d.qsplit = 0, self.QSPLIT
            d.w_att, d.w_lang, d.w_h, d.w_o = ptr(W.p_att2 if self.embgate else W.p_att), ptr(W.p_lang), ptr(W.p_h), ptr(W.p_o)
            w_fc = W.w_ih_att[:, R:2 * R]
            d.w_fc, d.ld_w_fc = w_fc.data_ptr(), w_fc.stride(0)
            d.gate_fc, d.q_parts, d.top2_part = ptr(self.gate_fc), ptr(self.q_parts), ptr(self.top2_part)
            for name, bufs in (("xa", self.XA), ("xl", self.XL), ("ca", self.cA), ("cl", self.cL)):
                arr = getattr(d, name)
                arr[0], arr[1] = ptr(bufs[0]), ptr(bufs[1])
            d.xa0_init = ptr(self.XA0_init)
            if self.embgate:
                d.w_att = ptr(W.p_att2)
                d.emb_gate, d.sel_counter = ptr(W.t_embgate), ptr(self.sel_counter)
                d.att_w_cached = int(self.att_w_cached)
            if self.lang_ksx:
                d.lang_ksx, d.ksx_slab, d.ksx_flags = 1, ptr(self.ksx_slab), ptr(self.ksx_flags)
            if self.gsk:
                d.gsk_nwg = self.gsk_nwg
                d.slab_att, d.slab_lang, d.slab_q, d.slab_o = (ptr(self.slab_att), ptr(self.slab_lang), ptr(self.slab_q),
                                                              ptr(self.slab_o))
        else:
            d.path = 1
            d.ks_gate, d.ks_q, d.ks_o, d.ks_fc = self.ks_gate, self.ks_q, self.ks_o, self.ks_fc
            d.w_att, d.w_lang, d.w_h, d.w_o, d.w_fc_frag = ptr(W.t_att2 if self.embgate else W.t_att), ptr(W.t_lang), ptr(W.t_h), ptr(W.t_o), ptr(W.t_fc)
            if self.embgate:
                d.emb_gate = ptr(W.t_embgate)
            d.gate_fc, d.q, d.q_parts, d.logits = ptr(self.gate_fc_clip), ptr(self.q), ptr(self.parts_q), ptr(self.logits)
            for name, t in (("xaf", self.XAf), ("xlf", self.XLf), ("xhf", self.XHf), ("xff", self.XFf)):
                p_, s_ = hip._frag_ptr(t)
                setattr(d, name, p_)
                setattr(d, name + "_stride", s_)
            d.parts_gate, d.parts_o, d.parts_fc = ptr(self.parts_gate), ptr(self.parts_o), ptr(self.parts_fc)
            d.h_att, d.c_att, d.h_lang, d.c_lang = ptr(self.t_h_att), ptr(self.t_c_att), ptr(self.t_h_lang), ptr(self.t_c_lang)
            d.c_att_prev, d.c_lang_prev, d.zero_state = ptr(self.t_c_att_prev), ptr(self.t_c_lang_prev), ptr(self.t_zero)
            if self.beam > 1:
                d.score, d.done, d.parent, d.beam_ws = ptr(self.score), ptr(self.done), ptr(self.parent), ptr(self.beam_ws)
        plan = C.c_void_p()
        hip._check(L.cvc_decode_plan_create(C.byref(d), C.byref(plan)), "cvc_decode_plan_create")
        self._desc, self._plan = d, plan
        self._plan_call = L.cvc_decode_beam if self.beam > 1 else L.cvc_decode_greedy

    def __del__(self):
        plan = getattr(self, "_plan", None)
        if plan is not None and plan.value:
            try:
                hip.lib().cvc_decode_plan_destroy(plan)
            except Exception:
                pass
            self._plan = None

    def _run_driver(self):
        hip._check(self._plan_call(self._plan, torch.cuda.current_stream().cuda_stream), "cvc_decode_greedy/beam")


    def _reset(self):
        if self.tile:
            self.words[0].zero_()
            if self.beam > 1:
                self.score.zero_()
                self.done.zero_()
            return
        if self.packed:
            self.XA[0].copy_(self.XA0_init)
            self.XL[0].zero_()
            self.cA[0].zero_()
            self.cL[0].zero_()
            self.words[0].zero_()
            return
        for bufs in (self.h_att, self.c_att, self.h_lang, self.c_lang):
            bufs[0].zero_()
        self.words[0].zero_()
        if self.beam > 1:
            self.score.zero_()
            self.done.zero_()

    def _run_launches(self, timers=None):
        stream = torch.cuda.current_stream().cuda_stream
        for name, fn, args in self._python_launches():
            if timers is not None:
                e0, e1 = torch.cuda.Event(enable_timing=True), torch.cuda.Event(enable_timing=True)
                e0.record()
            if fn == "copy":
                args[0].copy_(args[1])
            else:
                rc = fn(*args, stream)
                if rc != 0:
                    hip._check(rc, name)
            if timers is not None:
                e1.record()
                timers.setdefault(name, []).append((e0, e1))

    def load_features(self, feats: Dict[str, torch.Tensor]):
        if not self.own_features:
            raise RuntimeError("DecodeEngine.load_features needs own_features=True")
        pool = feats["pool_feats"]
        mask = feats["pnt_mask"][:, 1:] if feats["pnt_mask"].shape[1] == pool.shape[1] + 1 else feats["pnt_mask"]
        for dst, src in zip(self.feats, (feats["fc_feats"], feats["conv_feats"], feats["p_conv_feats"], pool, feats["p_pool_feats"])):
            if dst.shape != src.shape:
                raise RuntimeError(f"DecodeEngine.load_features: shape {tuple(src.shape)} != bound {tuple(dst.shape)}")
            dst.copy_(src)
        self.mask.copy_(hip._mask(mask))
        return self

    def load_captions(self, words: torch.Tensor, frame_mask: Optional[torch.Tensor] = None):
        if not self.forced:
            raise RuntimeError("DecodeEngine.load_captions: this engine is not in the forced mode (forced_n = 0)")
        if tuple(words.shape) != (self.rows, self.T) or words.dtype != torch.int64:
            raise RuntimeError(f"DecodeEngine.load_captions: words must be int64 [{self.rows}, {self.T}], got {words.dtype} "
                               f"{tuple(words.shape)}")
        if frame_mask is not None:
            if tuple(frame_mask.shape) != (self.T, self.rows, self.N):
                raise RuntimeError(f"DecodeEngine.load_captions: frame_mask has shape {tuple(frame_mask.shape)}, expected "
                                   f"{(self.T, self.rows, self.N)}")
            if self.fmask is None:
                if self.graph is not None:
                    raise RuntimeError("DecodeEngine.load_captions: the captured graph has no frame-masked output; bind the first "
                                       "frame mask before capture()")
                dev = self.words.device
                self.fmask = torch.zeros(self.T, self.rows, self.N, dtype=torch.uint8, device=dev)
                self.fm_steps = torch.zeros(self.T, self.rows, self.N, dtype=torch.float32, device=dev)
                self._launches = None
            self.fmask.copy_(hip._mask(frame_mask))
        elif self.fmask is not None:
            self.fmask.zero_()
        self.words[1:].copy_(words.t())
        return self

    def load_force_words(self, words):
        if not self.forcing:
            raise RuntimeError("DecodeEngine.load_force_words: this engine forces no words (force_n = 0)")
        w = torch.as_tensor(np.asarray(words.cpu()) if isinstance(words, torch.Tensor) else np.asarray(words))
        if tuple(w.shape) != (self.B, self.force_n) or w.dtype.is_floating_point or w.dtype == torch.bool:
            raise RuntimeError(f"DecodeEngine.load_force_words: words must be integers [{self.B}, {self.force_n}], got {w.dtype} "
                               f"{tuple(w.shape)}")
        big = sorted({int(v) for v in w.reshape(-1).tolist() if v >= self.W.V})
        if big:
            raise RuntimeError(f"DecodeEngine.load_force_words: ids outside [0, V = {self.W.V}): {big}")
        both = sorted({int(v) for v in w.reshape(-1).tolist()} & set(self.cons[3]))
        if both:
            raise RuntimeError(f"DecodeEngine.load_force_words: words that ban_words forbids cannot be forced: {both}")
        self.force_words.copy_(w.to(torch.int32))
        return self

    def _region_set(self, t):
        fc, conv, pconv, pool, ppool = self.feats
        ptr = lambda x: None if x is None else x.data_ptr()
        fm_in = fm_out = None
        if self.forced and self.fmask is not None:
            fm_in, fm_out = ptr(self.fmask[t]), ptr(self.fm_steps[t])
        return hip.AttnSet(ptr(ppool), ptr(pool), ptr(self.mask), fm_in, ptr(self.scores_r), fm_out, ptr(self.att_steps[t]), None,
# ... 38 lines not shown
        tail = (self.rng.data_ptr(), t, self.words[t + 1].data_ptr(), 1, self.logprob[t].data_ptr())
        if not self.trunc:
            return ("word_select", L.cvc_sample_select_parts, head + tail)
        return ("word_select", L.cvc_sample_select_trunc_parts, head + (self.top_k, self.top_p) + tail +
                (self.cutoff[t].data_ptr(), self.kept[t].data_ptr()))

    def _word_select_beam(self, t, parts, nparts, part_stride, bias):
        L, B, beam, V = hip.lib(), self.B, self.beam, self.W.V
        srd, swr = t & 1, (t + 1) & 1
        head = (parts, nparts, part_stride, bias, self.score[srd].data_ptr(), self.done[srd].data_ptr(), B, beam, V, self.unk)
        tail = (self.parent[t].data_ptr(), self.words[t + 1].data_ptr(), self.score[swr].data_ptr(), self.done[swr].data_ptr())
        ws = self.beam_ws.data_ptr()
        if not self.beam_hist:
            return ("word_select", L.cvc_beam_select_parts, head + (1 if t == 0 else 0,) + tail + (ws,))
        cons = (self._cons_desc, self.nbanned[t].data_ptr()) if self.constrained else (None, None)
        hist = (t, self.bhist[srd].data_ptr(), self.bhist[swr].data_ptr(), self.rows, cons[0])
        if self.grouped:
            return ("word_select", L.cvc_beam_select_groups_parts, head + hist + (self.groups, self.diversity) + tail + (cons[1], ws))
        if self.forcing:
            return ("word_select", L.cvc_beam_select_force_parts, head + hist + (self.force_words.data_ptr(), self.force_n) + tail +
                    (cons[1], self.nmet[t].data_ptr(), ws))
        return ("word_select", L.cvc_beam_select_hist_parts, head + hist + tail + (cons[1], ws))

    def hypotheses(self, ranked: bool = False):
        if not self.beam_hist:
            raise RuntimeError("DecodeEngine.hypotheses needs beam_history=True")
        B, beam, T = self.B, self.beam, self.T
        seq, score = self.bhist[T & 1].view(T, B, beam).permute(1, 2, 0), self.score[T & 1].view(B, beam)
        if not ranked:
            return seq, score
        if not self.ranked:
            raise RuntimeError("DecodeEngine.hypotheses(ranked=True) needs beam_groups > 1, a length_penalty or force_n")
        o = self.order
        return (seq.gather(1, o.unsqueeze(2).expand(B, beam, T)), score.gather(1, o), self.norm.gather(1, o),
                self.final_nmet.gather(1, o) if self.forcing else o // (beam // self.groups))

    def _python_launches(self):
        if self._launches is None:
            self._keep = []
            self._launches = self._build_launches()
        return self._launches

    def run_timed(self):
        timers = {}
        self._reset()
        self._run_launches(timers)
        torch.cuda.synchronize()
        return {k: [a.elapsed_time(b) for a, b in v] for k, v in timers.items()}

    def _run_once(self):
        if self._plan is not None:
            self._run_driver()
        else:
            self._reset()
            self._run_launches()
        if self.beam > 1 and self.ranked:
            L, T = hip.lib(), self.T
            if self.forcing:
                hip._check(L.cvc_beam_rank_force(self.bhist[T & 1].data_ptr(), self.rows, self.score[T & 1].data_ptr(),
                                                 self.force_words.data_ptr(), self.force_n, self.B, self.beam, T, self.W.V, self.unk,
                                                 self.length_penalty, self.order.data_ptr(), self.norm.data_ptr(),
                                                 self.hyp_len.data_ptr(), self.final_nmet.data_ptr(), hip._stream()), "cvc_beam_rank_force")
            else:
                hip._check(L.cvc_beam_rank(self.bhist[T & 1].data_ptr(), self.rows, self.score[T & 1].data_ptr(), self.B, self.beam, T,
                                           self.length_penalty, self.order.data_ptr(), self.norm.data_ptr(), self.hyp_len.data_ptr(),
                                           hip._stream()), "cvc_beam_rank")
            hip._check(L.cvc_beam_backtrack_from(self.words[1:].data_ptr(), self.parent.data_ptr(), self.att_steps.data_ptr(), self.B,
                                                 self.beam, T, self.N, self.order.data_ptr(), self.beam, self.bt_seq.data_ptr(),
                                                 self.bt_att.data_ptr(), hip._stream()), "cvc_beam_backtrack_from")
        elif self.beam > 1:
            hip._check(hip.lib().cvc_beam_backtrack(self.words[1:].data_ptr(), self.parent.data_ptr(), self.att_steps.data_ptr(),
                                                    self.B, self.beam, self.T, self.N, self.bt_seq.data_ptr(),
                                                    self.bt_att.data_ptr(), hip._stream()), "cvc_beam_backtrack")

    def capture(self):
        if self.lang_ksx and not self._ksx_checked:
            s = torch.cuda.Stream()
            s.wait_stream(torch.cuda.current_stream())
            with torch.cuda.stream(s):
                self._run_once()
            torch.cuda.current_stream().wait_stream(s)
            self.check_ksx()
        key = (self.packed, self.tile, self.beam > 1, self.sampling, self.weights_dtype, self.trunc, self.forced, self.constrained,
               self.beam_hist, self.grouped, self.ranked, self.forcing)
        if key not in DecodeEngine._warm:
            saved = self.rng.clone() if self.sampling else None
            s = torch.cuda.Stream()
            s.wait_stream(torch.cuda.current_stream())
            with torch.cuda.stream(s):
                self._run_once()
            torch.cuda.current_stream().wait_stream(s)
            if saved is not None:
                self.rng.copy_(saved)
            DecodeEngine._warm.add(key)
        g = torch.cuda.CUDAGraph()
        with torch.cuda.graph(g, capture_error_mode=_capture_mode()):
            self._run_once()
        self.graph = g
        return self

    def seed(self, s: int):
        if not self.sampling:
            raise RuntimeError("DecodeEngine.seed: this engine does not sample (temperature=None)")
        s = int(s) & 0xFFFFFFFFFFFFFFFF
        words = np.array([s & 0xFFFFFFFF, s >> 32, 0, 0], dtype=np.uint32).view(np.int32)
        self.rng.copy_(torch.from_numpy(words))
        return self

    def run(self):
        if self.graph is not None:
            self.graph.replay()
        else:
            self._run_once()
            if self.lang_ksx and not self._ksx_checked and self.check_ksx():
                self._run_once()
        if self.forced:
            return self.words[1:].t(), self.att_steps.permute(1, 0, 2), self.logprob.t(), self.rank.t()
        if self.sampling or (self.constrained and self.beam == 1):
            return self.words[1:].t(), self.att_steps.permute(1, 0, 2), self.logprob.t()
        if self.beam == 1:
            return self.words[1:].t(), self.att_steps.permute(1, 0, 2)
        return self._backtrack()

    def _backtrack(self):
        return self.bt_seq, self.bt_att, self.score[self.T & 1].view(self.B, self.beam)

    def _backtrack_host(self):
        B, beam, T, N = self.B, self.beam, self.T, self.N
        words = self.words[1:].view(T, B, beam)
        parent = self.parent.view(T, B, beam)
        att = self.att_steps.view(T, B, beam, N)
        k = torch.zeros(B, dtype=torch.int64, device=words.device)
        ar = torch.arange(B, device=words.device)
        seq, atts = [], []
        for t in range(T - 1, -1, -1):
            seq.append(words[t, ar, k])
            k_parent = parent[t, ar, k]
            atts.append(att[t, ar, k_parent])
            k = k_parent
        seq.reverse()
        atts.reverse()
        final_scores = self.score[self.T & 1].view(B, beam)
        return torch.stack(seq, 1), torch.stack(atts, 1), final_scores
```

cyclical-visual-captioning_amd/cvc/decode/path_packed.py:

```python
from __future__ import annotations

import ctypes as C
import os
from typing import Dict, List, Optional, Tuple

import torch

from .. import hip
from .weights import *
from .weights import _segs


class PackedPath:
    def _alloc_packed(self):
        W, R, E = self.W, self.W.R, self.W.E
        dev = self.fc.device
        if self.bf16w:
            bind_bf16(W)
        if not self.embgate and not hasattr(W, "p_att"):
            W.p_att = pack_weights(torch.cat([W.w_ih_att[:, 0:R], W.w_ih_att[:, 2 * R:2 * R + E], W.w_hh_att], 1), R)
        if not self.bf16w and not hasattr(W, "p_lang"):
            W.p_lang = pack_weights(torch.cat([W.w_ih_lang, W.w_hh_lang], 1), R)
            W.p_h = pack_weights(W.w_h)
            W.p_o = pack_weights(W.w_o)
# ... 32 lines not shown
            self.slab_lang = slab(nt_r, self.plan_l["maxseg"][0])
            self.slab_q = slab(nt_a, self.plan_l["maxseg"][1])

    def _build_packed(self):
        L, W = hip.lib(), self.W
        B, N, Fr, R, A, E, V, rows = self.B, self.N, self.F, W.R, W.A, W.E, W.V, self.rows
        fc, conv, pconv, pool, ppool = self.feats
        ptr = lambda t: None if t is None else t.data_ptr()
        qoff = lambda buf, k0: buf.data_ptr() + (k0 // 4) * 64 * 4 * 4
        out = []
        seg_fc = _segs([(fc, None, W.r_w_fc if self.bf16w else W.w_ih_att[:, R:2 * R], False)])
        out.append(("gate_fc", L.cvc_linear_fwd, (seg_fc, 1, ptr(W.b_ih_att), ptr(W.b_hh_att), rows, 4 * R, ptr(self.gate_fc),
                                                  4 * R)))
        self._keep.append(seg_fc)
        nblk_v = (V + 31) // 32
        if self.gsk:
            return out + self._build_gsk_steps()
        if self.embgate:
            return out + self._build_embgate_steps()
        for t in range(self.T):
            rd, wr = t & 1, (t + 1) & 1
            XA_r, XA_w, XL_r, XL_w = self.XA[rd], self.XA[wr], self.XL[rd], self.XL[wr]
            if self.ks_att and self.gate_fused:
                out.append(("att_lstm", L.cvc_packed_lstm_ksf_fwd, (ptr(W.p_att), ptr(XA_r), 2 * R + E, None, None, ptr(self.gate_fc),
                                                                    ptr(self.cA[rd]), rows, R, qoff(XL_r, R), qoff(XA_w, R + E),
                                                                    ptr(self.cA[wr]), ptr(self.gate_slab), ptr(self.gate_counters))))
            elif self.ks_att:
                wp_att = W.p_att_ks if self.ks_pad else W.p_att
                out.append(("att_lstm", L.cvc_packed_lstm_ks_fwd, (ptr(wp_att), ptr(XA_r), 2 * R + E, None, None, ptr(self.gate_fc),
                                                                   ptr(self.cA[rd]), rows, R, qoff(XL_r, R), qoff(XA_w, R + E),
                                                                   ptr(self.cA[wr]), ptr(self.gate_slab), wp_att.stride(0))))
            else:
                out.append(("att_lstm", L.cvc_packed_lstm_fwd, (ptr(W.p_att), ptr(XA_r), 2 * R + E, None, None, ptr(self.gate_fc),
                                                                ptr(self.cA[rd]), rows, R, qoff(XL_r, R), qoff(XA_w, R + E),
                                                                ptr(self.cA[wr]))))
            out.append(("h2attn", L.cvc_packed_linear_fwd, (ptr(W.p_h), qoff(XL_r, R), R, None, rows, A, self.QSPLIT,
                                                            ptr(self.q_parts), A, None)))
            sets = (hip.AttnSet * 2)()
            sets[0] = hip.AttnSet(ptr(ppool), ptr(pool), ptr(self.mask), None, ptr(self.scores_r), None,
                                  ptr(self.att_steps[t]), None, N, self.stream_r)
            sets[1] = hip.AttnSet(ptr(pconv), ptr(conv), None, None, ptr(self.scores_f), None, ptr(self.attn_f), None, Fr,
                                  self.stream_f)
            out.append(("attn_scores", L.cvc_attn_scores_qparts, (W.kind, ptr(self.q_parts), self.QSPLIT, ptr(W.b_h), ptr(W.w_a),
                                                                  ptr(W.b_a), self.inv_temp, sets, 2, B, 1, A)))
            out.append(("attn_wsum", L.cvc_attn_wsum_quad, (sets, 2, B, 1, R, ptr(XL_r))))
            if self.ks_lang and self.gate_fused:
                out.append(("lang_lstm", L.cvc_packed_lstm_ksf_fwd, (ptr(W.p_lang), ptr(XL_r), 3 * R, ptr(W.b_ih_lang),
                                                                     ptr(W.b_hh_lang), None, ptr(self.cL[rd]), rows, R, ptr(XA_w),
                                                                     qoff(XL_w, 2 * R), ptr(self.cL[wr]), ptr(self.gate_slab),
                                                                     ptr(self.gate_counters))))
            elif self.ks_lang:
                wp_lang = W.p_lang_ks if self.ks_pad else W.p_lang
                out.append(("lang_lstm", L.cvc_packed_lstm_ks_fwd, (ptr(wp_lang), ptr(XL_r), 3 * R, ptr(W.b_ih_lang),
                                                                    ptr(W.b_hh_lang), None, ptr(self.cL[rd]), rows, R, ptr(XA_w),
                                                                    qoff(XL_w, 2 * R), ptr(self.cL[wr]), ptr(self.gate_slab),
                                                                    wp_lang.stride(0))))
            elif self.lang_ksx:
                out.append(self._lang_ksx_launch(t, XL_r, XA_w, XL_w, rd, wr))
            else:
                out.append(("lang_lstm", L.cvc_packed_lstm_fwd, (ptr(W.p_lang), ptr(XL_r), 3 * R, ptr(W.b_ih_lang), ptr(W.b_hh_lang),
                                                                 None, ptr(self.cL[rd]), rows, R, ptr(XA_w), qoff(XL_w, 2 * R),
                                                                 ptr(self.cL[wr]))))
            out.append(("logits", L.cvc_packed_linear_fwd, (ptr(W.p_o), ptr(XA_w), R, ptr(W.b_o), rows, V, 1, None, V,
                                                            ptr(self.top2_part))))
            out.append(("word_select", L.cvc_top2_final, (ptr(self.top2_part), nblk_v, rows, self.unk, ptr(self.words[t + 1]), 1,
                                                          ptr(self.logprob[t]), ptr(W.embed), E, qoff(XA_w, R), 0)))
            self._keep.append(sets)
        return out

    def _build_embgate_steps(self):
        L, W = hip.lib(), self.W
        B, N, Fr, R, A, V, rows = self.B, self.N, self.F, W.R, W.A, W.V, self.rows
        fc, conv, pconv, pool, ppool = self.feats
        ptr = lambda t: None if t is None else t.data_ptr()
        qoff = lambda buf, k0: buf.data_ptr() + (k0 // 4) * 64 * 4 * 4
        out = []
        nblk_v = (V + 31) // 32
        if self.bf16w:
            att_fn, linear_fn = L.cvc_packed_lstm_bf16w_fwd, L.cvc_packed_linear_bf16w_fwd
            w_att, att_stride, embgate, w_h, w_o = W.pb_att2, 2 * R * 32, W.r_embgate, W.pb_h, W.pb_o
        else:
            att_fn, linear_fn = L.cvc_packed_lstm_embgate_ex_fwd, L.cvc_packed_linear_fwd
            w_att, att_stride, embgate, w_h, w_o = W.p_att2, (2 * R // 4) * 128, W.t_embgate, W.p_h, W.p_o
        for t in range(self.T):
            rd, wr = t & 1, (t + 1) & 1
            XA_r, XA_w, XL_r, XL_w = self.XA[rd], self.XA[wr], self.XL[rd], self.XL[wr]
            first = t == 0 and (self.bf16w or hip.gemm_packed_split(-1) == 2)
            out.append(("att_lstm", att_fn, (ptr(w_att), att_stride, ptr(XA_r), 32 if first else 2 * R, None, None,
                                             ptr(self.gate_fc), ptr(embgate), ptr(self.words[t]), ptr(self.cA[rd]),
                                             rows, R, qoff(XL_r, R), qoff(XA_w, R), ptr(self.cA[wr]),
                                             1 if self.att_w_cached else 0)))
            out.append(("h2attn", linear_fn, (ptr(w_h), qoff(XL_r, R), R, None, rows, A, self.QSPLIT, ptr(self.q_parts), A, None)))
            sets = (hip.AttnSet * 2)()
            sets[0] = self._region_set(t)
            sets[1] = hip.AttnSet(ptr(pconv), ptr(conv), None, None, ptr(self.scores_f), None, ptr(self.attn_f), None, Fr,
                                  self.stream_f)
            out.append(("attn_scores", L.cvc_attn_scores_qparts, (W.kind, ptr(self.q_parts), self.QSPLIT, ptr(W.b_h), ptr(W.w_a),
                                                                  ptr(W.b_a), self.inv_temp, sets, 2, B, 1, A)))
            out.append(("attn_wsum", L.cvc_attn_wsum_quad, (sets, 2, B, 1, R, ptr(XL_r))))
            if self.bf16w:
                out.append(("lang_lstm", L.cvc_packed_lstm_bf16w_fwd, (ptr(W.pb_lang), 3 * R * 32, ptr(XL_r), 2 * R if first else 3 * R,
                                                                       ptr(W.b_ih_lang), ptr(W.b_hh_lang), None, None, None, ptr(self.cL[rd]),
                                                                       rows, R, ptr(XA_w), qoff(XL_w, 2 * R), ptr(self.cL[wr]),
                                                                       1 if self.lang_w_cached else 0)))
            elif first:
                out.append(("lang_lstm", L.cvc_packed_lstm_late_fwd, (ptr(W.p_lang), (3 * R // 4) * 128, ptr(XL_r), 2 * R, ptr(W.b_ih_lang),
                                                                      ptr(W.b_hh_lang), None, ptr(self.cL[rd]), rows, R, ptr(XA_w),
                                                                      qoff(XL_w, 2 * R), ptr(self.cL[wr]), None)))
            elif self.lang_ksx:
                out.append(self._lang_ksx_launch(t, XL_r, XA_w, XL_w, rd, wr))
            else:
                out.append(("lang_lstm", L.cvc_packed_lstm_fwd, (ptr(W.p_lang), ptr(XL_r), 3 * R, ptr(W.b_ih_lang), ptr(W.b_hh_lang),
                                                                 None, ptr(self.cL[rd]), rows, R, ptr(XA_w), qoff(XL_w, 2 * R),
                                                                 ptr(self.cL[wr]))))
            if self.given:
                out.append(("logits", linear_fn, (ptr(w_o), ptr(XA_w), R, ptr(W.b_o), rows, V, 1, ptr(self.logits), V, None)))
                out.append(self._word_select_sampled(t, ptr(self.logits), 1, 0, None))
            else:
                out.append(("logits", linear_fn, (ptr(w_o), ptr(XA_w), R, ptr(W.b_o), rows, V, 1, None, V, ptr(self.top2_part))))
                out.append(("word_select", L.cvc_top2_final, (ptr(self.top2_part), nblk_v, rows, self.unk, ptr(self.words[t + 1]), 1,
                                                              ptr(self.logprob[t]), None, 0, None, 0)))
            self._keep.append(sets)
        return out
```

cyclical-visual-captioning_amd/cvc/decode/weights.py:

```python
from __future__ import annotations

import ctypes as C
import os
from typing import Dict, List, Optional

import torch

from .. import hip


class DecodeWeights:

    def __init__(self, sd: Dict[str, torch.Tensor], softattn_type: str = "additive"):
        g = lambda k: sd[k].detach().contiguous()
        self.w_ih_att, self.w_hh_att = g("decoder_core.att_lstm.weight_ih"), g("decoder_core.att_lstm.weight_hh")
        self.b_ih_att, self.b_hh_att = g("decoder_core.att_lstm.bias_ih"), g("decoder_core.att_lstm.bias_hh")
        self.w_ih_lang, self.w_hh_lang = g("decoder_core.lang_lstm.weight_ih"), g("decoder_core.lang_lstm.weight_hh")
        self.b_ih_lang, self.b_hh_lang = g("decoder_core.lang_lstm.bias_ih"), g("decoder_core.lang_lstm.bias_hh")
        self.w_h, self.b_h = g("decoder_core.soft_attn.h2attn.weight"), g("decoder_core.soft_attn.h2attn.bias")
        self.kind = hip.ATTN_ADDITIVE if softattn_type == "additive" else hip.ATTN_DOT
        if self.kind == hip.ATTN_ADDITIVE:
            self.w_a = g("decoder_core.soft_attn.alpha_net.weight").reshape(-1)
            self.b_a = g("decoder_core.soft_attn.alpha_net.bias")
        else:
# ... 78 lines not shown
        out = torch.empty_like(w)
        out[lstm_packed_rows(lstm_R, w.device)] = w
        w = out
    return w if n is None else w[:n]


def bind_bf16(W: "DecodeWeights") -> "DecodeWeights":
    if hasattr(W, "pb_lang"):
        return W
    R, E = W.R, W.E
    W.pb_att2 = pack_weights_bf16(torch.cat([W.w_ih_att[:, 0:R], W.w_hh_att], 1), R)
    W.pb_h = pack_weights_bf16(W.w_h)
    W.pb_o = pack_weights_bf16(W.w_o)
    W.r_w_fc = bf16_round(W.w_ih_att[:, R:2 * R])
    W.r_embgate = hip.tile_mm(torch.relu(W.embed), bf16_round(W.w_ih_att[:, 2 * R:2 * R + E]))
    W.pb_lang = pack_weights_bf16(torch.cat([W.w_ih_lang, W.w_hh_lang], 1), R)
    return W


EMBGATE_MAX_BYTES = 1 << 30


def embgate_table(W: "DecodeWeights") -> torch.Tensor:
    R, E = W.R, W.E
    return hip.tile_mm(torch.relu(W.embed), W.w_ih_att[:, 2 * R:2 * R + E])


def to_quad(x: torch.Tensor) -> torch.Tensor:
    m, k = x.shape
    out = x.new_zeros(k // 4, 64, 4)
    out[:, :m] = x.view(m, k // 4, 4).permute(1, 0, 2)
    return out


def from_quad(xq: torch.Tensor, m: int) -> torch.Tensor:
    return xq[:, :m].permute(1, 0, 2).reshape(m, -1)


def split3_bf16(x: torch.Tensor):
    def top(v):
        return (v.view(torch.int32) & -65536).view(torch.float32)
    hi = top(x)
    r1 = x - hi
    mid = top(r1)
    lo = top(r1 - mid)
    bits = lambda v: (v.view(torch.int32) >> 16).to(torch.int16)
    return bits(hi), bits(mid), bits(lo)


def to_frag(x: torch.Tensor, rows_alloc: Optional[int] = None) -> torch.Tensor:
    m, k = x.shape
    assert k % 16 == 0, k
    ra = rows_alloc if rows_alloc is not None else (m + 31) // 32 * 32
    xp = x.new_zeros(ra, k)
    xp[:m] = x
    planes = torch.stack(split3_bf16(xp.contiguous()), 0)
    return planes.view(3, ra // 32, 32, k // 16, 2, 8).permute(1, 3, 0, 4, 2, 5).contiguous()


def from_frag(xb: torch.Tensor, m: int) -> torch.Tensor:
    nb, ks = xb.shape[0], xb.shape[1]
    f = (xb.to(torch.int32) << 16).view(torch.float32)
    x = f.sum(2).permute(0, 3, 1, 2, 4).reshape(nb * 32, ks * 16)
    return x[:m]


def pack_weights_tile(w: torch.Tensor, lstm_R: Optional[int] = None) -> torch.Tensor:
    n, k = w.shape
    assert k % 16 == 0, k
    if lstm_R is not None:
        R = lstm_R
        assert n == 4 * R and R % 8 == 0
        i = torch.arange(32, device=w.device)
        rows = ((i >> 3) * R + (i & 7)).view(1, 32) + (torch.arange(R // 8, device=w.device) * 8).view(-1, 1)
        w = w[rows.reshape(-1)]
    return to_frag(w, (n + 127) // 128 * 128)


GATE_KSPLIT_DEFAULT = False
KS_PAD_QUADS = 0

CACHE_BUDGET = int(os.environ.get("CVC_CACHE_BUDGET_MB", "208")) << 20
LANG_KSX_DEFAULT = os.environ.get("CVC_LANG_KSX", "0") == "1"
CACHE_LANG_GATE_WEIGHTS = os.environ.get("CVC_LANG_W_CACHED", "1") != "0"
CACHE_GATE_WEIGHTS = os.environ.get("CVC_ATT_W_CACHED", "1") != "0"


def cache_plan(linear_weight_bytes: int, feature_bytes: Dict[str, int], budget: int = CACHE_BUDGET,
               gate_weight_bytes: Optional[int] = None, lang_weight_bytes: Optional[int] = None) -> Dict[str, bool]:
    names = list(feature_bytes)
    room = budget - linear_weight_bytes
    plan = {}
    if gate_weight_bytes is not None:
        plan["att_w"] = bool(CACHE_GATE_WEIGHTS and 0 < gate_weight_bytes <= room)
        if plan["att_w"]:
            room -= gate_weight_bytes
    if lang_weight_bytes is not None:
        plan["lang_w"] = bool(CACHE_GATE_WEIGHTS and CACHE_LANG_GATE_WEIGHTS and plan.get("att_w", False) and 0 < lang_weight_bytes <= room)
        if plan["lang_w"]:
            room -= lang_weight_bytes
    best, best_bytes = (), 0
    for pick in range(1 << len(names)):
        chosen = [n for i, n in enumerate(names) if pick >> i & 1]
        tot = sum(feature_bytes[n] for n in chosen)
        if best_bytes < tot <= room:
            best, best_bytes = tuple(chosen), tot
    plan.update({n: n in best for n in names})
    return plan
```

cyclical-visual-captioning_amd/cvc/hip.py:

```python
from __future__ import annotations

import ctypes as C
import functools
import os
from typing import List, Optional, Sequence

import torch

_HERE = os.path.dirname(os.path.abspath(__file__))
LIB_PATH = os.environ.get("CVC_LIB") or os.path.join(_HERE, "lib", "libcvc_hip.so")

ATTN_ADDITIVE, ATTN_DOT = 0, 1


class AttnSet(C.Structure):
    _fields_ = [("proj", C.c_void_p), ("ctx", C.c_void_p), ("mask", C.c_void_p), ("frame_mask", C.c_void_p),
                ("scores", C.c_void_p), ("frame_masked", C.c_void_p), ("attn", C.c_void_p), ("ctx_out", C.c_void_p),
                ("n", C.c_int), ("stream", C.c_int)]


class GemmSeg(C.Structure):
    _fields_ = [("x", C.c_void_p), ("idx", C.c_void_p), ("w", C.c_void_p),
                ("k", C.c_int), ("ldx", C.c_int), ("ldw", C.c_int), ("relu", C.c_int)]


class NNSeg(C.Structure):
    _fields_ = [("w", C.c_void_p), ("dst", C.c_void_p), ("ldw", C.c_int), ("ncols", C.c_int), ("ld_dst", C.c_int)]


_P, _I, _F, _LL = C.c_void_p, C.c_int, C.c_float, C.c_longlong


class OptimSeg(C.Structure):
    _fields_ = [("p", C.c_void_p), ("g", C.c_void_p), ("m", C.c_void_p), ("v", C.c_void_p), ("step", C.c_void_p), ("n", C.c_longlong),
                ("lr", C.c_float), ("weight_decay", C.c_float)]


class OptimChunk(C.Structure):
    _fields_ = [("seg", C.c_int), ("pad", C.c_int), ("start", C.c_longlong)]


class GskGroup(C.Structure):
    _fields_ = [("wp", C.c_void_p), ("w_blk_stride", C.c_longlong), ("xq", C.c_void_p), ("nblk", C.c_int), ("nchunk", C.c_int),
                ("skip_at", C.c_int), ("skip_n", C.c_int), ("slab", C.c_void_p), ("maxseg", C.c_int)]


class GskSegs(C.Structure):
    _fields_ = [("slab", C.c_void_p), ("unit0", C.c_int), ("nchunk", C.c_int), ("U", C.c_int), ("maxseg", C.c_int)]


class DecodeDesc(C.Structure):
    _fields_ = (
        [(n, C.c_int) for n in ("B", "beam", "T", "N", "F", "R", "A", "E", "V", "unk_idx", "attn_kind")] +
        [("inv_temp", C.c_float)] +
        [(n, C.c_int) for n in ("stream_r", "stream_f", "path", "qsplit", "ks_gate", "ks_q", "ks_o", "ks_fc")] +
        [(n, C.c_void_p) for n in ("b_ih_att", "b_hh_att", "b_ih_lang", "b_hh_lang", "b_h", "w_a", "b_a", "b_o", "embed")] +
        [("w_fc", C.c_void_p), ("ld_w_fc", C.c_int)] +
        [(n, C.c_void_p) for n in ("w_att", "w_lang", "w_h", "w_o", "w_fc_frag")] +
        [(n, C.c_void_p) for n in ("fc", "conv", "pconv", "pool", "ppool", "mask")] +
        [(n, C.c_void_p) for n in ("words", "att_steps", "logprob", "score", "done", "parent")] +
        [(n, C.c_void_p) for n in ("gate_fc", "scores_r", "scores_f", "attn_f", "q", "q_parts", "top2_part")] +
        [("xa", C.c_void_p * 2), ("xl", C.c_void_p * 2), ("ca", C.c_void_p * 2), ("cl", C.c_void_p * 2), ("xa0_init", C.c_void_p)] +
        [(n, C.c_void_p) for n in ("xaf", "xlf", "xhf", "xff")] +
        [(n, C.c_longlong) for n in ("xaf_stride", "xlf_stride", "xhf_stride", "xff_stride")] +
        [(n, C.c_void_p) for n in ("parts_gate", "parts_o", "parts_fc", "logits")] +
        [(n, C.c_void_p) for n in ("h_att", "c_att", "h_lang", "c_lang", "c_att_prev", "c_lang_prev", "zero_state")] +
        [("beam_ws", C.c_void_p)] +
        [("gsk_nwg", C.c_int)] + [(n, C.c_void_p) for n in ("slab_att", "slab_lang", "slab_q", "slab_o", "emb_gate", "sel_counter")] +
        [("att_w_cached", C.c_int), ("lang_ksx", C.c_int), ("ksx_slab", C.c_void_p), ("ksx_flags", C.c_void_p)])

class GradSrc(C.Structure):
    _fields_ = [("p", C.c_void_p), ("ld", C.c_longlong), ("plane_stride", C.c_longlong), ("nplanes", C.c_int)]


class PwBwdArgs(C.Structure):
    _fields_ = ([("d_h", GradSrc * 3), ("d_hd", C.c_void_p), ("rng_state", C.c_void_p), ("site", C.c_uint), ("p", C.c_float)] +
                [(n, C.c_void_p) for n in ("d_c", "gates", "c_prev", "c_new")] + [("M", C.c_int)] +
                [(n, C.c_void_p) for n in ("d_gates", "d_c_prev", "d_gates_q", "dg_sum")] + [("q_row0", C.c_int)])


class LstmStep(C.Structure):
    _fields_ = ([("wp", C.c_void_p), ("xq", C.c_void_p), ("K", C.c_int), ("M", C.c_int), ("R", C.c_int)] +
                [(n, C.c_void_p) for n in ("b_ih", "b_hh", "gate_pre", "row_bias", "row_index", "c_prev", "c_out", "gates_out", "h_out",
                                           "h_out2", "h_drop_out", "rng_state")] +
                [("site", C.c_uint), ("p", C.c_float), ("h_dst1_q", C.c_void_p), ("h_dst2_q", C.c_void_p), ("w_cached", C.c_int)])


class Constraint(C.Structure):
    _fields_ = [("no_repeat_ngram", C.c_int), ("no_immediate_repeat", C.c_int), ("min_len", C.c_int), ("nban", C.c_int),
                ("ban", C.c_void_p), ("bad_end", C.c_void_p), ("nbad", C.c_int)]


class TrainLoop(C.Structure):
    _fields_ = (
        [(n, C.c_int) for n in ("kind", "B", "T", "R", "A", "N", "F", "attn_kind")] + [("inv_temp", C.c_float)] +
        [(n, C.c_void_p) for n in ("wp_att", "wp_lang", "b_ih_att", "b_hh_att", "b_ih_lang", "b_hh_lang", "w_ih_att", "w_hh_att",
                                   "w_ih_lang", "w_hh_lang")] +
        [("ld_ih_att", C.c_int), ("ld_ih_lang", C.c_int)] +
        [(n, C.c_void_p) for n in ("w_h", "b_h", "wp_h")] + [("q_split", C.c_int)] +
        [(n, C.c_void_p) for n in ("w_a", "b_a", "gpre_att", "row_bias", "row_index", "gpre_lang", "pool", "ppool", "conv",
                                   "pconv", "mask", "frame_mask", "rng_state")] +
        [("site0", C.c_uint), ("p", C.c_float)] +
        [(n, C.c_void_p) for n in ("out", "h_att", "h_att_prev", "h_lang_prev", "c_att", "c_lang", "g_att", "g_lang", "ctx", "q", "attn_r",
                                   "attn_f", "fm", "scores_ws")] +
        [("xa", C.c_void_p * 2), ("xl", C.c_void_p * 2)] +
        [(n, C.c_void_p) for n in ("d_out", "d_fm", "dg_att", "dg_lang", "dgsum_att", "dgsum_lang", "dq", "dwa_part", "ds_r", "ds_f", "d_pool", "d_ppool", "d_conv",
                                   "d_pconv", "bwd_ws", "d_ctx_all")])


SIGNATURES = {
    "cvc_packed_lstm_step_fwd": [C.POINTER(LstmStep), _P],
    "cvc_attn_wsum_quad_rm": [C.POINTER(AttnSet), _I, _I, _I, _P, _P, _P],
    "cvc_attn_bwd_pair": [_I, C.POINTER(GradSrc), _P, _P, _F, C.POINTER(AttnSet), _I, C.POINTER(GradSrc), _I, _I, _I, _I, _P, _P, _P,
                          C.POINTER(_P), C.POINTER(_P), _P],
    "cvc_ctxfeat_bwd_steps": [_P, _P, _I, _I, _I, _I, _P, _P],
    "cvc_tile_gemm_big": [_I, _I],
    "cvc_tile_gemm_plan": [_I, _I, _I, _P, _P, _P],
    "cvc_dproj_bwd_steps": [_P, _LL, _LL, _I, _P, _P, _P, _P, _I, _I, _I, _I, _P, _P],
    "cvc_lstm_pointwise_bwd4": [C.POINTER(GradSrc), _P, _P, C.c_uint, _F, _P, _P, _P, _P, _I, _I, _P, _P, _P, _P, _I, _P],
    "cvc_vocab_head_nll_fwd": [_P, _I, _LL, _I, _P, _P, _P, _I, _I, _P, _I, _P, _P, _P, _P],
    "cvc_scale_by_scalar": [_P, _P, _LL, _P, _P],
    "cvc_relu_dropout_fwd": [_P, _P, _LL, _I, _P, C.c_uint, _F, _P, _P],
    "cvc_relu_dropout_bwd": [_P, _P, _LL, _P, C.c_uint, _F, _P, _P],
    "cvc_bn_workspace": [_LL, _I],
    "cvc_bn_relu_train_fwd": [_P, _P, _P, _F, _F, _P, _P, _LL, _I, _P, _P, _P, _P, _P],
    "cvc_bn_relu_train_bwd": [_P, _P, _P, _P, _P, _P, _LL, _I, _P, _P, _P, _P, _P],
    "cvc_class_softmax_bwd": [_P, _P, _P, _P, _I, _I, _I, _P, _P],
    "cvc_layernorm_cat_bwd": [C.POINTER(_P), C.POINTER(_LL), C.POINTER(_I), _I, _LL, _F, _P, _LL, C.POINTER(_P), C.POINTER(_LL), _P],
    "cvc_bbox_overlaps_fwd": [_P, _I, _P, _I, _P, _P, _I, _I, _I, _I, _P, _P],
    "cvc_label_glue_fwd": [_P, _P, _LL, _LL, _LL, _P, _P, _I, _I, _I, _I, _P, _P, _P, _P],
    "cvc_attn_nll_fwd": [_P, _LL, _LL, _P, _LL, _LL, _P, _I, _I, _I, _P, _P, _P],
    "cvc_attn_nll_bwd": [_P, _LL, _LL, _P, _LL, _LL, _P, _I, _I, _I, _P, _P, _P, _P, _P, _P],
    "cvc_train_loop_bwd_ws": [_I, _I, _I],
    "cvc_train_loop_fwd": [C.POINTER(TrainLoop), _P],
    "cvc_train_loop_bwd": [C.POINTER(TrainLoop), _P],
    "cvc_train_loops_bwd_joint": [C.POINTER(TrainLoop), C.POINTER(TrainLoop), _P],
    "cvc_stable_order": [_P, _I, _P, _P],
    "cvc_attn_weighted_rows": [_P, _P, _I, _I, _I, _I, _F, _P, _P],
    "cvc_col_sum": [_P, _LL, _I, _I, _P, _P, _P, _P],
    "cvc_col_sum_ws": [_I, _I],
    "cvc_train_loop_profile": [_I],
    "cvc_train_loop_profile_read": [C.POINTER(_I), C.POINTER(_I), C.POINTER(_F), _I],
    "cvc_attn_fwd": [_I, _P, _P, _P, _F, C.POINTER(AttnSet), _I, _I, _I, _I, _I, _P, _P],
    "cvc_attn_scores": [_I, _P, _P, _P, _F, C.POINTER(AttnSet), _I, _I, _I, _I, _P],
    "cvc_attn_scores_qparts": [_I, _P, _I, _P, _P, _P, _F, C.POINTER(AttnSet), _I, _I, _I, _I, _P],
    "cvc_linear_splitk_fwd": [C.POINTER(GemmSeg), _I, _P, _I, _I, _I, _P, _P],
    "cvc_linear_top2_fwd": [C.POINTER(GemmSeg), _I, _P, _I, _I, _P, _P, _P],
    "cvc_top2_final": [_P, _I, _I, _I, _P, _I, _P, _P, _I, _P, _I, _P],
    "cvc_attn_wsum_quad": [C.POINTER(AttnSet), _I, _I, _I, _I, _P, _P],
    "cvc_packed_lstm_fwd": [_P, _P, _I, _P, _P, _P, _P, _I, _I, _P, _P, _P, _P],
    "cvc_packed_linear_fwd": [_P, _P, _I, _P, _I, _I, _I, _P, _I, _P, _P],
    "cvc_packed_lstm_wg_blocks": [_I],
# ... 2 lines not shown
    "cvc_packed_linear_select_fwd": [_P, _P, _I, _P, _I, _I, _P, _P, _I, _P, _I, _P, _P],
    "cvc_gsk_plan": [C.POINTER(_I), C.POINTER(_I), _I, _I, C.POINTER(_I), C.POINTER(_I), C.POINTER(_I)],
    "cvc_gsk_gemm": [C.POINTER(GskGroup), _I, _I, _P],
    "cvc_packed_lstm_late_fwd": [_P, _LL, _P, _I, _P, _P, _P, _P, _I, _I, _P, _P, _P, C.POINTER(GskSegs), _P],
    "cvc_attn_scores_qslab": [_I, C.POINTER(GskSegs), _P, _P, _P, _F, C.POINTER(AttnSet), _I, _I, _I, _I, _P],
    "cvc_top2_slab": [C.POINTER(GskSegs), _P, _I, _I, _I, _P, _I, _P, _P, _I, _P, _I, _P],
    "cvc_packed_lstm_train_fwd": [_P, _P, _I, _P, _P, _P, _I, _I, _P, _P, _P, _P, _P, _P],
    "cvc_pack_lstm_weights": [_P, _I, _P, _I, _I, _P, _P],
    "cvc_pack_lstm_segs": [C.POINTER(_P), C.POINTER(_LL), C.POINTER(_I), _I, _I, _P, _P],
    "cvc_packed_lstm_train_pre_fwd": [_P, _P, _I, _P, _P, _P, _P, _I, _I, _P, _P, _P, _P, _P, _P],
    "cvc_pack_quad_segs": [C.POINTER(_P), C.POINTER(_LL), C.POINTER(_I), _I, _I, _P, _P],
    "cvc_beam_backtrack": [_P, _P, _P, _I, _I, _I, _I, _P, _P, _P],
    "cvc_gru_seq_fwd": [_P, _P, _LL, _LL, _P, _P, _I, _I, _I, _I, _P, _P, _LL, _LL, _P],
    "cvc_gru_seq_train_fwd": [_P, _P, _LL, _LL, _P, _P, _I, _I, _I, _I, _P, _P, _LL, _LL, _P, _LL, _LL, _P],
    "cvc_lstm_pointwise_bwd4_pair": [C.POINTER(PwBwdArgs), C.POINTER(PwBwdArgs), _I, _P],
    "cvc_gru_persistent_halves": [_I],
    "cvc_gru_persistent_waves8": [_I],
    "cvc_gru_persistent_sync_words": [],
    "cvc_gru_seq_persistent_train_fwd": [_P, _P, _LL, _LL, _P, _P, _I, _I, _I, _I, _P, _P, _LL, _LL, _P, _LL, _LL, _P, _P],
    "cvc_gru_seq_bwd_ksplit": [_I],
    "cvc_gru_bwd_persistent_sync_words": [],
    "cvc_gru_seq_bwd_persistent": [_P, _LL, _LL, _P, _LL, _LL, _P, _LL, _LL, _P, _I, _I, _I, _I, _P, _P, _P, _P, _P],
    "cvc_linear_nn_planes_fwd": [_P, _I, _I, C.POINTER(NNSeg), _I, _I, _P, _P],
    "cvc_linear_nn_planes2_fwd": [_P, _P, _I, _I, _I, C.POINTER(NNSeg), _I, _I, _P, _I, _P],
    "cvc_gru_seq_bwd": [_P, _LL, _LL, _P, _LL, _LL, _P, _LL, _LL, _P, _I, _I, _I, _I, _P, _P, _P, _P],
    "cvc_gru_seq_persistent_fwd": [_P, _P, _LL, _LL, _P, _P, _I, _I, _I, _I, _P, _P, _LL, _LL, _P, _P],
    "cvc_lstm_persistent_sync_words": [],
    "cvc_lstm_seq_persistent_fwd": [_P, _P, _LL, _LL, _P, _P, _I, _I, _I, _I, _P, _P, _LL, _LL, _P, _P],
    "cvc_lstm_seq_persistent_train_fwd": [_P, _P, _LL, _LL, _P, _P, _I, _I, _I, _I, _P, _P, _LL, _LL, _P, _LL, _LL, _P, _LL, _LL, _P, _P],
    "cvc_lstm_seq_fwd": [_P, _P, _LL, _LL, _P, _P, _I, _I, _I, _I, _P, _P, _LL, _LL, _P],
    "cvc_lstm_seq_train_fwd": [_P, _P, _LL, _LL, _P, _P, _I, _I, _I, _I, _P, _P, _LL, _LL, _P, _LL, _LL, _P, _LL, _LL, _P],
    "cvc_lstm_seq_bwd_work": [_I, _I, _I],
    "cvc_lstm_seq_bwd": [_P, _LL, _LL, _P, _LL, _LL, _P, _LL, _LL, _P, _I, _I, _I, _I, _P, _P, _P],
    "cvc_packed_lstm_ks_slices": [_I, _I],
    "cvc_packed_lstm_ks_fwd": [_P, _P, _I, _P, _P, _P, _P, _I, _I, _P, _P, _P, _P, _LL, _P],
    "cvc_packed_lstm_ksf_fwd": [_P, _P, _I, _P, _P, _P, _P, _I, _I, _P, _P, _P, _P, _P, _P],
    "cvc_packed_lstm_ksx_local": [_I],
    "cvc_packed_lstm_ksx_fwd": [_P, _P, _I, _P, _P, _P, _P, _P, _P, _I, _I, _P, _P, _P, _P, _P, C.c_uint, _P],
    "cvc_attn_wsum": [C.POINTER(AttnSet), _I, _I, _I, _I, _P, _P],
    "cvc_attn_bwd": [_I, _P, _P, _F, _P, _P, _P, _P, _P, _I, _I, _I, _I, _I, _P, _P, _P, _P, _P, _P],
    "cvc_linear_fwd": [C.POINTER(GemmSeg), _I, _P, _P, _I, _I, _P, _I, _P],
    "cvc_gemm_force_generic": [_I],
    "cvc_gemm_packed_split": [_I],
    "cvc_lstm_cell_fwd": [C.POINTER(GemmSeg), _I, _P, _P, _P, _P, _I, _I, _P, _P, _P, _P],
    "cvc_lstm_pointwise_bwd": [_P, _P, _P, _P, _P, _I, _I, _P, _P, _P, _P],
    "cvc_lstm_pointwise_bwd3": [_P, _P, _P, _P, _P, _P, _P, _I, _I, _P, _P, _P, _P],
    "cvc_linear_nn_fwd": [_P, _I, _I, C.POINTER(NNSeg), _I, _I, _P, _P],
    "cvc_pack_quad": [_P, _LL, _I, _I, _P, _P],
    "cvc_embed_relu_fwd": [_P, _P, _P, _I, _I, _P, _P],
    "cvc_embed_relu_bwd": [_P, _P, _P, _P, _P, _I, _I, _P, _P, _P],
    "cvc_embed_relu_rng_fwd": [_P, _P, _P, C.c_uint, _F, _I, _I, _P, _P],
    "cvc_embed_relu_rng_bwd": [_P, _P, _P, _P, C.c_uint, _F, _P, _I, _I, _P, _P, _P],
    "cvc_dropout_rng": [_P, _LL, _P, C.c_uint, _F, _P, _P],
    "cvc_packed_lstm_train_drop_fwd": [_P, _P, _I, _P, _P, _P, _P, _I, _I, _P, _P, _P, _P, _P, _P, C.c_uint, _F, _P],
    "cvc_lstm_pointwise_bwd3_drop": [_P, _P, _P, _P, C.c_uint, _F, _P, _P, _P, _P, _I, _I, _P, _P, _P, _P],
    "cvc_log_softmax_fwd": [_P, _I, _I, _P, _P],
    "cvc_log_softmax_bwd": [_P, _P, _I, _I, _P, _P],
    "cvc_nll_bwd": [_P, _P, _P, _I, _I, _P, _P],
    "cvc_top2_unk": [_P, _I, _I, _I, _P, _I, _P, _P],
    "cvc_nll_fwd": [_P, _P, _P, _I, _I, _P, _P],
    "cvc_vocab_nll_fwd": [_P, _P, _P, _I, _I, _P, _P, _P, _P, _P],
    "cvc_vocab_nll_bwd": [_P, _P, _P, _P, _P, _I, _I, _P, _P],
    "cvc_grounder_fwd": [_P, _P, _P, _P, _I, _I, _I, _I, _P, _P],
    "cvc_grounder_bwd": [_P, _P, _P, _I, _I, _I, _I, _P, _P, _P],
    "cvc_beam_select": [_P, _P, _P, _I, _I, _I, _I, _I, _P, _P, _P, _P, _P, _P],
    "cvc_beam_select_parts": [_P, _I, _LL, _P, _P, _P, _I, _I, _I, _I, _I, _P, _P, _P, _P, _P, _P],
    "cvc_sample_select_parts": [_P, _I, _LL, _P, _I, _I, _I, _F, _P, _I, _P, _I, _P, _P],
    "cvc_sample_select_trunc_parts": [_P, _I, _LL, _P, _I, _I, _I, _F, _I, _F, _P, _I, _P, _I, _P, _P, _P, _P],
    "cvc_sample_advance": [_P, _P],
    "cvc_forced_select_parts": [_P, _I, _LL, _P, _I, _I, _P, _I, _P, _P, _P],
    "cvc_constrained_select_parts": [_P, _I, _LL, _P, _I, _I, _I, _F, _I, _F, _P, _I, _P, _I, _P, _P, _P, _P, _LL, C.POINTER(Constraint),
                                     _P, _P],
    "cvc_beam_select_hist_parts": [_P, _I, _LL, _P, _P, _P, _I, _I, _I, _I, _I, _P, _P, _LL, C.POINTER(Constraint), _P, _P, _P, _P, _P,
                                   _P, _P],
    "cvc_beam_select_groups_parts": [_P, _I, _LL, _P, _P, _P, _I, _I, _I, _I, _I, _P, _P, _LL, C.POINTER(Constraint), _I, _F, _P, _P, _P,
                                     _P, _P, _P, _P],
    "cvc_beam_rank": [_P, _LL, _P, _I, _I, _I, _F, _P, _P, _P, _P],
    "cvc_beam_backtrack_from": [_P, _P, _P, _I, _I, _I, _I, _P, _LL, _P, _P, _P],
    "cvc_beam_select_force_parts": [_P, _I, _LL, _P, _P, _P, _I, _I, _I, _I, _I, _P, _P, _LL, C.POINTER(Constraint), _P, _I, _P, _P, _P,
                                    _P, _P, _P, _P, _P],
    "cvc_beam_rank_force": [_P, _LL, _P, _P, _I, _I, _I, _I, _I, _I, _F, _P, _P, _P, _P, _P],
    "cvc_packed_lstm_bf16w_fwd": [_P, _LL, _P, _I, _P, _P, _P, _P, _P, _P, _I, _I, _P, _P, _P, _I, _P],
    "cvc_packed_linear_bf16w_fwd": [_P, _P, _I, _P, _I, _I, _I, _P, _I, _P, _P],
    "cvc_gather_rows": [_P, _P, _I, _I, _I, _P, _P],
    "cvc_tile_rows_alloc": [_I],
    "cvc_tile_gemm_loaders": [_I],
    "cvc_tile_gemm": [_P, _P, _LL, _I, _I, _I, _I, _P, _I, _LL, _P],
    "cvc_tile_lstm_finish": [_P, _I, _LL, _P, _P, _P, _I, _P, _I, _I, _P, _P, _P, _LL, _P, _LL, _P],
    "cvc_tile_lstm_finish_embgate": [_P, _I, _LL, _P, _P, _P, _I, _P, _P, _I, _P, _I, _I, _P, _P, _P, _LL, _P, _LL, _P],
    "cvc_tile_linear_finish": [_P, _I, _LL, _I, _P, _P, _I, _I, _P, _I, _P],
    "cvc_tile_pack_rows": [_P, _I, _P, _I, _I, _I, _P, _LL, _P],
    "cvc_tile_pack_rows_any": [_P, _LL, _I, _I, _P, _LL, _P],
    "cvc_tile_pack_cols": [_P, _LL, _I, _I, _P, _LL, _P],
    "cvc_tile_reorder_pack": [_P, _P, _I, _P, _P, _P, _P, _P, _I, _I, _P, _P, _P, _LL, _P, _LL, _I, _I, _P],
    "cvc_attn_wsum_frag": [C.POINTER(AttnSet), _I, _I, _I, _I, _P, _LL, _P],
    "cvc_class_softmax_fwd": [_P, _LL, _P, _P, _I, _I, _I, _P, _P, _P],
    "cvc_layernorm_cat_fwd": [C.POINTER(_P), C.POINTER(_LL), C.POINTER(_I), _I, _LL, _F, _P, _LL, _P],
    "cvc_frame_embed_fwd": [_P, _P, _I, _P, _P, _I, _P, _P, _LL, _P, _P],
    "cvc_decode_plan_create": [C.POINTER(DecodeDesc), C.POINTER(C.c_void_p)],
    "cvc_decode_plan_destroy": [_P],
    "cvc_decode_plan_set_features": [_P, _P, _P, _P, _P, _P, _P],
    "cvc_decode_num_launches": [_P],
    "cvc_decode_greedy": [_P, _P],
    "cvc_decode_beam": [_P, _P],
    "cvc_optim_chunk_elems": [],
    "cvc_adam_clip_step": [_P, _I, _P, _I, _F, _F, _F, _F, _F, _I, _P, _P, _P, _P],
    "cvc_comm_unique_id": [_P],
    "cvc_comm_init": [_I, _I, _P, C.POINTER(C.c_void_p)],
    "cvc_allreduce_grads": [_P, _P, _LL, _P],
    "cvc_comm_destroy": [_P],
}
_VOID_RETURN = {"cvc_decode_plan_destroy"}
BLOCKS = {
    "cvc_attn_scores", "cvc_attn_wsum", "cvc_attn_scores_qparts", "cvc_attn_wsum_quad", "cvc_attn_wsum_frag", "cvc_attn_wsum_quad_rm",
    "cvc_attn_bwd_pair", "cvc_ctxfeat_bwd_steps", "cvc_dproj_bwd_steps", "cvc_tile_gemm_big", "cvc_tile_gemm_plan", "cvc_linear_splitk_fwd", "cvc_linear_top2_fwd", "cvc_top2_final", "cvc_packed_lstm_fwd", "cvc_packed_linear_fwd",
    "cvc_packed_lstm_embgate_fwd", "cvc_packed_lstm_embgate_ex_fwd", "cvc_packed_lstm_late_fwd", "cvc_packed_lstm_train_fwd",
    "cvc_packed_lstm_train_pre_fwd", "cvc_packed_lstm_train_drop_fwd", "cvc_lstm_pointwise_bwd", "cvc_lstm_pointwise_bwd3",
    "cvc_lstm_pointwise_bwd3_drop", "cvc_pack_lstm_weights", "cvc_linear_nn_planes_fwd", "cvc_linear_nn_planes2_fwd", "cvc_gru_seq_train_fwd", "cvc_lstm_pointwise_bwd4_pair", "cvc_beam_select_parts", "cvc_sample_select_parts", "cvc_sample_select_trunc_parts", "cvc_sample_advance", "cvc_forced_select_parts", "cvc_constrained_select_parts", "cvc_beam_select_hist_parts", "cvc_beam_select_groups_parts", "cvc_beam_rank", "cvc_beam_select_force_parts", "cvc_beam_rank_force", "cvc_beam_backtrack_from", "cvc_tile_lstm_finish",
    "cvc_tile_lstm_finish_embgate", "cvc_tile_reorder_pack", "cvc_decode_num_launches", "cvc_gemm_force_generic",
    "cvc_tile_gemm_loaders", "cvc_gru_persistent_waves8", "cvc_relu_dropout_fwd", "cvc_relu_dropout_bwd", "cvc_bn_workspace",
    "cvc_bn_relu_train_fwd", "cvc_bn_relu_train_bwd", "cvc_class_softmax_bwd", "cvc_layernorm_cat_bwd", "cvc_stable_order", "cvc_col_sum", "cvc_col_sum_ws", "cvc_attn_weighted_rows",
    "cvc_lstm_persistent_sync_words", "cvc_lstm_seq_persistent_fwd", "cvc_lstm_seq_persistent_train_fwd", "cvc_lstm_seq_fwd", "cvc_lstm_seq_train_fwd", "cvc_lstm_seq_bwd_work", "cvc_lstm_seq_bwd",
    "cvc_packed_lstm_bf16w_fwd", "cvc_packed_linear_bf16w_fwd"}
EXPERIMENTAL = {
    "cvc_gsk_plan", "cvc_gsk_gemm", "cvc_attn_scores_qslab", "cvc_top2_slab", "cvc_packed_lstm_ks_slices", "cvc_packed_lstm_ks_fwd",
    "cvc_packed_lstm_ksf_fwd", "cvc_packed_lstm_ksx_local", "cvc_packed_lstm_ksx_fwd", "cvc_packed_lstm_wg_blocks",
    "cvc_packed_linear_select_fwd", "cvc_gru_persistent_halves"}

_lib = None


def _missing(name):
    def fn(*_a, **_k):
        raise RuntimeError(f"{name} is an experimental form (include/cvc_hip_experimental.h): this libcvc_hip.so was built without "
                           "CVC_EXPERIMENTAL=1 (`CVC_EXPERIMENTAL=1 python cyclical-visual-captioning_amd/build_hip.py --force`)")
    return fn


def lib() -> C.CDLL:
    global _lib
    if _lib is None:
        if not os.path.exists(LIB_PATH):
            raise RuntimeError(
                f"{LIB_PATH} is missing: build it with `python cyclical-visual-captioning_amd/build_hip.py` "
                "(hipcc --offload-arch=gfx950).  There is no CPU fallback for the caption-decode hot path.")
        l = C.CDLL(LIB_PATH)
        l.cvc_block.restype = C.c_void_p
        l.cvc_block.argtypes = [C.c_char_p]
        for name, argtypes in SIGNATURES.items():
            restype = None if name in _VOID_RETURN else (C.c_longlong if name in ("cvc_train_loop_bwd_ws", "cvc_bn_workspace", "cvc_col_sum_ws") else C.c_int)
            if name in BLOCKS or name in EXPERIMENTAL:
                addr = l.cvc_block(name.encode())
                if not addr:
                    if name in BLOCKS:
                        raise RuntimeError(f"{LIB_PATH}: building block {name} is not in the library's table (stale build?)")
                    setattr(l, name, _missing(name))
                    continue
                setattr(l, name, C.CFUNCTYPE(restype, *argtypes)(addr))
                continue
            fn = getattr(l, name)
            fn.argtypes = argtypes
            fn.restype = restype
        l.cvc_version.restype = C.c_char_p
        l.cvc_version.argtypes = []
        _lib = l
    return _lib


def experimental_built() -> bool:
    return b"+experimental" in lib().cvc_version()


def version() -> str:
    return lib().cvc_version().decode()


_weights_generation = 0


def weights_generation() -> int:
    return _weights_generation


_warned = set()


def warn_once(key: str, msg: str):
    if key not in _warned:
        _warned.add(key)
        import warnings
        warnings.warn("cvc: " + msg, RuntimeWarning, stacklevel=3)


def bump_weights_generation() -> int:
    global _weights_generation
    _weights_generation += 1
    return _weights_generation


_step_status: dict = {}
_deferred_status = None


def step_status(device) -> torch.Tensor:
    dev = torch.device(device)
    key = dev.index if dev.index is not None else torch.cuda.current_device()
# ... 749 lines not shown
```

include/cvc_hip.h:

```cpp
#ifndef CVC_HIP_H
#define CVC_HIP_H

#include <stdint.h>

#ifdef __cplusplus
extern "C" {
#endif

typedef void* cvc_stream_t;

#define CVC_API __attribute__((visibility("default")))

#define CVC_E_BADARG (-1)
#define CVC_E_TOOBIG (-2)
#define CVC_E_NORCCL (-3)

#define CVC_ATTN_ADDITIVE 0
#define CVC_ATTN_DOT 1

CVC_API const char* cvc_version(void);
CVC_API void* cvc_block(const char* name);

typedef struct {
    const float* proj;
// ... 134 lines not shown
CVC_API int cvc_scale_by_scalar(const float* x, const float* g, long long n, float* y, cvc_stream_t stream);

CVC_API int cvc_grounder_fwd(const float* xt, const float* feats, const float* bias, const uint8_t* mask,
                     int B, int T, int N, int G, float* out, cvc_stream_t stream);
CVC_API int cvc_grounder_bwd(const float* d, const float* xt, const float* feats, int B, int T, int N, int G,
                     float* d_xt, float* d_feats, cvc_stream_t stream);

CVC_API int cvc_bbox_overlaps_fwd(const float* rois, int ld_roi, const float* gt, int ld_gt, const uint8_t* frm_mask,
                          const uint8_t* pnt_mask, int ld_pnt, int B, int N, int K, float* ov, cvc_stream_t stream);
CVC_API int cvc_label_glue_fwd(const float* ov, const uint8_t* box_mask, long long bm_stride_b, long long bm_stride_k,
                       long long bm_stride_t, const uint8_t* frm_mask, const uint8_t* pnt_mask, int B, int N, int K, int T,
                       uint8_t* labels, uint8_t* frm_mask_output, uint8_t* step_fmask, cvc_stream_t stream);
CVC_API int cvc_attn_nll_fwd(const float* x0, long long x0_stride_b, long long x0_stride_t, const float* x1, long long x1_stride_b,
                     long long x1_stride_t, const uint8_t* target, int B, int T, int N, float* workspace, float* loss,
                     cvc_stream_t stream);
CVC_API int cvc_attn_nll_bwd(const float* x0, long long x0_stride_b, long long x0_stride_t, const float* x1, long long x1_stride_b,
                     long long x1_stride_t, const uint8_t* target, int B, int T, int N, const float* workspace,
                     const float* g0, const float* g1, float* d_x0, float* d_x1, cvc_stream_t stream);

CVC_API int cvc_beam_select(const float* logits, const float* score_in, const uint8_t* done_in,
                    int B, int beam, int V, int unk_idx, int first_step,
                    int64_t* parent, int64_t* word, float* score_out, uint8_t* done_out,
                    float* workspace , cvc_stream_t stream);
CVC_API int cvc_beam_backtrack(const int64_t* words, const int64_t* parent, const float* att, int B, int beam, int T, int N,
                       int64_t* seq, float* att_out, cvc_stream_t stream);

CVC_API int cvc_gather_rows(const float* src, const int64_t* parent, int rows, int beam, int width,
                    float* dst, cvc_stream_t stream);


CVC_API int cvc_tile_rows_alloc(int M);
CVC_API int cvc_tile_gemm(const void* wb, const void* xb, long long x_mblk_stride, int K, int M, int N, int ksplit,
                  float* parts, int ld, long long part_stride, cvc_stream_t stream);
CVC_API int cvc_tile_linear_finish(const float* parts, int nparts, long long part_stride, int ld, const float* bias,
                           const float* bias2, int M, int N, float* y, int ldy, cvc_stream_t stream);
CVC_API int cvc_tile_pack_rows(const float* x, int ldx, const int64_t* idx, int relu, int M, int K, void* xb,
                       long long x_mblk_stride, cvc_stream_t stream);
CVC_API int cvc_tile_pack_rows_any(const float* x, long long ldx, int M, int K, void* xb, long long x_mblk_stride, cvc_stream_t stream);
CVC_API int cvc_tile_pack_cols(const float* x, long long ldx, int S, int C, void* xb, long long x_mblk_stride, cvc_stream_t stream);

CVC_API int cvc_class_softmax_fwd(const float* logits, long long ld_logits, const float* bias, const uint8_t* pad, int B, int N,
                          int C, float* out, float* out_rows, cvc_stream_t stream);
CVC_API int cvc_layernorm_cat_fwd(const float* const* xs, const long long* ldx, const int* widths, int nseg, long long rows, float eps,
                          float* out, long long ld_out, cvc_stream_t stream);
CVC_API int cvc_frame_embed_fwd(const float* y0, const float* b0, int c0, const float* y1, const float* b1, int c1, const float* scale,
                        const float* shift, long long rows, float* out, cvc_stream_t stream);

typedef struct cvc_decode_desc {
    int B, beam, T, N, F, R, A, E, V;
    int unk_idx, attn_kind;
    float inv_temp;
    int stream_r, stream_f;
    int path;
    int qsplit;
    int ks_gate, ks_q, ks_o, ks_fc;
    const float *b_ih_att, *b_hh_att, *b_ih_lang, *b_hh_lang, *b_h, *w_a, *b_a, *b_o, *embed;
    const float* w_fc; int ld_w_fc;
    const void *w_att, *w_lang, *w_h, *w_o, *w_fc_frag;
    const float *fc, *conv, *pconv, *pool, *ppool; const uint8_t* mask;
    int64_t* words;
    float* att_steps;
    float* logprob;
    float* score; uint8_t* done; int64_t* parent;
    float *gate_fc;
    float *scores_r, *scores_f, *attn_f;
    float *q;
    float *q_parts;
    float *top2_part;
    float *xa[2], *xl[2], *ca[2], *cl[2];
    const float* xa0_init;
    void *xaf, *xlf, *xhf, *xff;
    long long xaf_stride, xlf_stride, xhf_stride, xff_stride;
    float *parts_gate, *parts_o, *parts_fc, *logits;
    float *h_att, *c_att, *h_lang, *c_lang, *c_att_prev, *c_lang_prev; const float* zero_state;
    float *beam_ws;
    int gsk_nwg;
    float *slab_att, *slab_lang, *slab_q, *slab_o;
    const float* emb_gate;
    unsigned* sel_counter;
    int att_w_cached;
    int lang_ksx;
    float* ksx_slab;
    unsigned* ksx_flags;
} cvc_decode_desc;
typedef struct cvc_decode_plan cvc_decode_plan;
CVC_API int cvc_decode_plan_create(const cvc_decode_desc* desc, cvc_decode_plan** plan);
CVC_API void cvc_decode_plan_destroy(cvc_decode_plan* plan);
CVC_API int cvc_decode_plan_set_features(cvc_decode_plan* plan, const float* fc, const float* conv, const float* pconv,
                                 const float* pool, const float* ppool, const uint8_t* mask);
CVC_API int cvc_decode_greedy(cvc_decode_plan* plan, cvc_stream_t stream);
CVC_API int cvc_decode_beam(cvc_decode_plan* plan, cvc_stream_t stream);

typedef struct cvc_grad_src {
    const float* p;
    long long ld, plane_stride;
    int nplanes;
} cvc_grad_src;

typedef struct cvc_lstm_step {
    const float* wp;
    const float* xq;
    int K, M, R;
    const float *b_ih, *b_hh;
    const float* gate_pre;
    const float* row_bias;
    const int64_t* row_index;
    const float* c_prev;
    float *c_out, *gates_out;
    float *h_out, *h_out2;
    float* h_drop_out;
    const uint32_t* rng_state; unsigned site; float p;
    float *h_dst1_q, *h_dst2_q;
    int w_cached;
} cvc_lstm_step;
CVC_API int cvc_packed_lstm_step_fwd(const cvc_lstm_step* s, cvc_stream_t stream);



CVC_API int cvc_lstm_pointwise_bwd4(const cvc_grad_src* d_h , const float* d_hd,
                            const uint32_t* rng_state, unsigned site, float p, const float* d_c, const float* gates,
                            const float* c_prev, const float* c_new, int M, int R, float* d_gates, float* d_c_prev,
                            float* d_gates_q, float* dg_sum ,
                            int q_row0 , cvc_stream_t stream);

typedef struct cvc_train_loop {
    int kind;
    int B, T, R;
    int A, N, F, attn_kind;
    float inv_temp;
    const float *wp_att, *wp_lang;
    const float *b_ih_att, *b_hh_att, *b_ih_lang, *b_hh_lang;
    const float *w_ih_att, *w_hh_att, *w_ih_lang, *w_hh_lang;
    int ld_ih_att, ld_ih_lang;
    const float *w_h, *b_h;
    const float* wp_h;
    int q_split;
    const float *w_a, *b_a;
    const float* gpre_att;
    const float* row_bias;
    const int64_t* row_index;
    const float* gpre_lang;
    const float *pool, *ppool, *conv, *pconv;
    const uint8_t* mask;
    const uint8_t* frame_mask;
    const uint32_t* rng_state; unsigned site0; float p;
    float* out;
    float* h_att;
    float* h_att_prev;
    float* h_lang_prev;
    float *c_att, *c_lang;
    float *g_att, *g_lang;
    float* ctx;
    float* q;
    float *attn_r, *attn_f;
    float* fm;
    float* scores_ws;
    float *xa[2], *xl[2];
    const float* d_out;
    const float* d_fm;
    float *dg_att, *dg_lang;
    float *dgsum_att, *dgsum_lang;
    float* dq;
    float* dwa_part;
    float *ds_r, *ds_f;
    float *d_pool, *d_ppool, *d_conv, *d_pconv;
    float* bwd_ws;
// ... 31 lines not shown
```

include/cvc_hip_blocks.h:

```cpp
#ifndef CVC_HIP_BLOCKS_H
#define CVC_HIP_BLOCKS_H
#include "cvc_hip.h"
#ifdef __cplusplus
extern "C" {
#endif

int cvc_attn_scores(int kind, const float* q, const float* w_a, const float* b_a, float inv_temp,
                    const cvc_attn_set* sets, int nsets, int nclip, int nq, int A, cvc_stream_t stream);
int cvc_attn_wsum(const cvc_attn_set* sets, int nsets, int nclip, int nq, int R, float* ctx_sum,
                  cvc_stream_t stream);
int cvc_attn_scores_qparts(int kind, const float* q_parts, int q_nparts, const float* q_bias, const float* w_a,
                           const float* b_a, float inv_temp, const cvc_attn_set* sets, int nsets, int nclip,
                           int nq, int A, cvc_stream_t stream);
int cvc_attn_wsum_quad(const cvc_attn_set* sets, int nsets, int nclip, int nq, int R, float* ctx_sum_q,
                       cvc_stream_t stream);
int cvc_attn_wsum_frag(const cvc_attn_set* sets, int nsets, int nclip, int nq, int R, void* ctx_frag,
                       long long frag_mblk_stride, cvc_stream_t stream);
int cvc_attn_wsum_quad_rm(const cvc_attn_set* sets, int nsets, int nclip, int R, float* ctx_sum_q, float* ctx_sum_rm,
                          cvc_stream_t stream);
int cvc_attn_bwd_pair(int kind, const cvc_grad_src* q, const float* q_bias, const float* w_a, float inv_temp,
                      const cvc_attn_set* sets, int nsets, const cvc_grad_src* d_ctx, int nclip, int nq, int A, int R,
                      float* d_q, float* d_q_q, float* d_w_part, float* const* d_proj, float* const* d_ctxfeat,
                      cvc_stream_t stream);
int cvc_ctxfeat_bwd_steps(const float* attn, const float* d_ctx_all, int T, int B, int n, int R, float* d_feat, cvc_stream_t stream);
// ... 100 lines not shown
int cvc_beam_select_groups_parts(const float* parts, int nparts, long long part_stride, const float* bias,
                                 const float* score_in, const uint8_t* done_in, int B, int beam, int V, int unk_idx, int t,
                                 const int64_t* hist_in, int64_t* hist_out, long long hist_stride, const cvc_constraint* c,
                                 int groups, float lambda, int64_t* parent, int64_t* word, float* score_out, uint8_t* done_out,
                                 int32_t* nbanned, float* workspace, cvc_stream_t stream);
int cvc_beam_rank(const int64_t* hist, long long hist_stride, const float* score, int B, int beam, int T, float alpha,
                  int64_t* order, float* norm, int32_t* len, cvc_stream_t stream);
int cvc_beam_select_force_parts(const float* parts, int nparts, long long part_stride, const float* bias,
                                const float* score_in, const uint8_t* done_in, int B, int beam, int V, int unk_idx, int t,
                                const int64_t* hist_in, int64_t* hist_out, long long hist_stride, const cvc_constraint* c,
                                const int32_t* force, int nforce, int64_t* parent, int64_t* word, float* score_out, uint8_t* done_out,
                                int32_t* nbanned, int32_t* nmet, float* workspace, cvc_stream_t stream);
int cvc_beam_rank_force(const int64_t* hist, long long hist_stride, const float* score, const int32_t* force, int nforce, int B,
                        int beam, int T, int V, int unk_idx, float alpha, int64_t* order, float* norm, int32_t* len, int32_t* nmet,
                        cvc_stream_t stream);
int cvc_beam_backtrack_from(const int64_t* words, const int64_t* parent, const float* att, int B, int beam, int T, int N,
                            const int64_t* start, long long start_stride, int64_t* seq, float* att_out, cvc_stream_t stream);
int cvc_forced_select_parts(const float* parts, int nparts, long long part_stride, const float* bias, int M, int V,
                            const int64_t* word, int word_stride, float* logprob, int32_t* rank, cvc_stream_t stream);
int cvc_tile_lstm_finish(const float* parts, int nparts, long long part_stride, const float* b_ih, const float* b_hh,
                         const float* gate_bias, int gb_div, const float* c_prev, int M, int R, float* c_out,
                         float* h_out, void* frag1, long long frag1_stride, void* frag2, long long frag2_stride,
                         cvc_stream_t stream);
int cvc_tile_lstm_finish_embgate(const float* parts, int nparts, long long part_stride, const float* b_ih, const float* b_hh,
                                 const float* gate_bias, int gb_div, const float* emb_gate, const int64_t* word, int V,
                                 const float* c_prev, int M, int R, float* c_out, float* h_out, void* frag1,
                                 long long frag1_stride, void* frag2, long long frag2_stride, cvc_stream_t stream);
int cvc_tile_reorder_pack(const int64_t* parent, const int64_t* word, int beam, const float* h_att, const float* c_att,
                          const float* h_lang, const float* c_lang, const float* table, int E, int V,
                          float* c_att_prev, float* c_lang_prev, void* xa, long long xa_stride, void* xl_hlang,
                          long long xl_stride, int rows, int R, cvc_stream_t stream);
int cvc_decode_num_launches(const cvc_decode_plan* plan);
int cvc_gemm_force_generic(int on);
int cvc_tile_gemm_loaders(int on);
int cvc_gru_persistent_waves8(int on);
int cvc_relu_dropout_fwd(const float* x, const float* bias, long long rows, int N, const uint32_t* rng_state, unsigned site,
                         float p, float* y, cvc_stream_t stream);
int cvc_relu_dropout_bwd(const float* dy, const float* y, long long n, const uint32_t* rng_state, unsigned site, float p, float* dx,
                         cvc_stream_t stream);
long long cvc_bn_workspace(long long rows, int C);
int cvc_bn_relu_train_fwd(const float* x, const float* gamma, const float* beta, float eps, float momentum, float* running_mean,
                          float* running_var, long long rows, int C, float* y, float* save_mean, float* save_invstd,
                          float* workspace, cvc_stream_t stream);
int cvc_bn_relu_train_bwd(const float* x, const float* dy, const float* y, const float* gamma, const float* save_mean,
                          const float* save_invstd, long long rows, int C, float* dx, float* dgamma, float* dbeta,
                          float* workspace, cvc_stream_t stream);
int cvc_class_softmax_bwd(const float* p_rows, const float* d_rows, const float* d_sim, const uint8_t* pad, int B, int N, int C,
                          float* d_logits, cvc_stream_t stream);
int cvc_layernorm_cat_bwd(const float* const* xs, const long long* ldx, const int* widths, int nseg, long long rows, float eps,
                          const float* d_out, long long ld_out, float* const* dxs, const long long* lddx, cvc_stream_t stream);

int cvc_attn_weighted_rows(const float* w, const float* X, int nclip, int nq, int n, int R, float scale, float* out, cvc_stream_t stream);

int cvc_stable_order(const int64_t* key, int n, int64_t* order, cvc_stream_t stream);
long long cvc_col_sum_ws(int S, int n);
int cvc_col_sum(const float* x, long long ld, int S, int n, float* out, float* out2, float* ws, cvc_stream_t stream);

int cvc_lstm_persistent_sync_words(void);
int cvc_lstm_seq_persistent_fwd(const float* wp, const float* gi, long long gi_ld_m, long long gi_ld_t, const float* b_ih,
                                const float* b_hh, int M, int F, int H, int ndir, float* hq, float* y, long long y_ld_m,
                                long long y_ld_t, unsigned* sync, cvc_stream_t stream);
int cvc_lstm_seq_persistent_train_fwd(const float* wp, const float* gi, long long gi_ld_m, long long gi_ld_t, const float* b_ih,
                                      const float* b_hh, int M, int F, int H, int ndir, float* hq, float* y, long long y_ld_m,
                                      long long y_ld_t, float* gates, long long g_ld_m, long long g_ld_t, float* c, long long c_ld_m,
                                      long long c_ld_t, unsigned* sync, cvc_stream_t stream);
int cvc_lstm_seq_fwd(const float* wp, const float* gi, long long gi_ld_m, long long gi_ld_t, const float* b_ih, const float* b_hh,
                     int M, int F, int H, int ndir, float* hq, float* y, long long y_ld_m, long long y_ld_t, cvc_stream_t stream);
int cvc_lstm_seq_train_fwd(const float* wp, const float* gi, long long gi_ld_m, long long gi_ld_t, const float* b_ih,
                           const float* b_hh, int M, int F, int H, int ndir, float* hq, float* y, long long y_ld_m, long long y_ld_t,
                           float* gates, long long g_ld_m, long long g_ld_t, float* c, long long c_ld_m, long long c_ld_t,
                           cvc_stream_t stream);
int cvc_lstm_seq_bwd_work(int M, int H, int ndir);
int cvc_lstm_seq_bwd(const float* dy, long long dy_ld_m, long long dy_ld_t, const float* gates, long long g_ld_m, long long g_ld_t,
                     const float* c, long long c_ld_m, long long c_ld_t, const float* w_hh, int M, int F, int H, int ndir, float* dg,
                     float* work, cvc_stream_t stream);

int cvc_packed_lstm_bf16w_fwd(const uint16_t* wp, long long w_blk_stride, const float* xq, int K, const float* b_ih,
                              const float* b_hh, const float* gate_bias, const float* emb_gate, const int64_t* word,
                              const float* c_prev_q, int M, int R, float* h_dst1_q, float* h_dst2_q, float* c_out_q,
                              int w_cached, cvc_stream_t stream);
int cvc_packed_linear_bf16w_fwd(const uint16_t* wp, const float* xq, int K, const float* bias, int M, int Nout, int ksplit,
                                float* y, int ldy, float* top2_part, cvc_stream_t stream);

#ifdef __cplusplus
}
#endif
#endif
```

Measured before the change: 332,800 decode-steps/s.

## Fuse word selection into logits GEMM via atomic packed argmax keys

Replaces the per-step top2_final launch with packed 64-bit (value, index) keys that the vocab logits GEMM reduces per block and merges with atomic max into a few slots. The next step's attention-LSTM kernel decodes the chosen word straight from those keys. Per-block max/sum-exp partials are kept so one finalize kernel at the end writes all words and log-probs. This drops one launch and one dependent serial kernel per decode step, at the cost of atomics, an extra key read in the gate kernel, and a new default tail mode.

```diff
diff --git a/cyclical-visual-captioning_amd/csrc/blocks.hip b/cyclical-visual-captioning_amd/csrc/blocks.hip
--- a/cyclical-visual-captioning_amd/csrc/blocks.hip
+++ b/cyclical-visual-captioning_amd/csrc/blocks.hip
@@ -74,6 +74,9 @@
     CVC_B(cvc_lstm_seq_bwd),
     CVC_B(cvc_packed_lstm_bf16w_fwd),
     CVC_B(cvc_packed_linear_bf16w_fwd),
+    CVC_B(cvc_packed_linear_keys_fwd),
+    CVC_B(cvc_packed_lstm_embgate_keys_fwd),
+    CVC_B(cvc_keys_finalize),
 #ifdef CVC_EXPERIMENTAL
     CVC_B(cvc_gsk_plan),
     CVC_B(cvc_gsk_gemm),
diff --git a/cyclical-visual-captioning_amd/csrc/decode_driver.hip b/cyclical-visual-captioning_amd/csrc/decode_driver.hip
--- a/cyclical-visual-captioning_amd/csrc/decode_driver.hip
+++ b/cyclical-visual-captioning_amd/csrc/decode_driver.hip
@@ -101,10 +101,20 @@
     CVC_TRY(cvc_linear_fwd(&seg, 1, d.b_ih_att, d.b_hh_att, rows, 4 * R, d.gate_fc, 4 * R, st));
     const long long ws_att = (long long)(2 * R / 4) * 128, ws_lang = (long long)(3 * R / 4) * 128;
     const bool split2 = cvc_gemm_packed_split(-1) == 2;
+    const bool fused = d.tail != 0;
+    const int nblk_v = (V + 31) / 32;
+    unsigned long long* key_unk0 = d.tail_keys + (size_t)d.T * 64 * 4;
+    if (fused)
+        CVC_TRY(reset(d.tail_keys, nullptr, (size_t)d.T * 64 * 5 * sizeof(unsigned long long), st));
     for (int t = 0; t < d.T; ++t) {
         const int rd = t & 1, wr = (t + 1) & 1;
         float *XA_r = d.xa[rd], *XA_w = d.xa[wr], *XL_r = d.xl[rd], *XL_w = d.xl[wr];
         const bool first = t == 0 && split2;
+        if (fused && t > 0)
+            CVC_TRY(cvc_packed_lstm_embgate_keys_fwd((const float*)d.w_att, ws_att, XA_r, 2 * R, nullptr, nullptr, d.gate_fc, d.emb_gate,
+                                                     d.tail_keys + (size_t)(t - 1) * 64 * 4, key_unk0 + (size_t)(t - 1) * 64, d.unk_idx,
+                                                     d.ca[rd], rows, R, quad_off(XL_r, R), quad_off(XA_w, R), d.ca[wr], d.att_w_cached, st));
+        else
         CVC_TRY(cvc_packed_lstm_embgate_ex_fwd((const float*)d.w_att, ws_att, XA_r, first ? 32 : 2 * R, nullptr, nullptr, d.gate_fc,
                                                d.emb_gate, d.words + (size_t)t * rows, d.ca[rd], rows, R, quad_off(XL_r, R),
                                                quad_off(XA_w, R), d.ca[wr], d.att_w_cached, st));
@@ -124,10 +134,17 @@
         else
         CVC_TRY(cvc_packed_lstm_fwd((const float*)d.w_lang, XL_r, 3 * R, d.b_ih_lang, d.b_hh_lang, nullptr, d.cl[rd], rows, R, XA_w,
                                     quad_off(XL_w, 2 * R), d.cl[wr], st));
+        if (fused) {
+            CVC_TRY(cvc_packed_linear_keys_fwd((const float*)d.w_o, XA_w, R, d.b_o, rows, V, d.unk_idx, d.tail_keys + (size_t)t * 64 * 4,
+                                               key_unk0 + (size_t)t * 64, d.tail_ms + (size_t)t * nblk_v * 64 * 2, st));
+            continue;
+        }
         CVC_TRY(cvc_packed_linear_fwd((const float*)d.w_o, XA_w, R, d.b_o, rows, V, 1, nullptr, V, d.top2_part, st));
-        CVC_TRY(cvc_top2_final(d.top2_part, (V + 31) / 32, rows, d.unk_idx, d.words + (size_t)(t + 1) * rows, 1,
+        CVC_TRY(cvc_top2_final(d.top2_part, nblk_v, rows, d.unk_idx, d.words + (size_t)(t + 1) * rows, 1,
                                d.logprob ? d.logprob + (size_t)t * rows : nullptr, nullptr, 0, nullptr, 0, st));
     }
+    if (fused)
+        CVC_TRY(cvc_keys_finalize(d.tail_keys, key_unk0, d.tail_ms, nblk_v, d.T, rows, d.unk_idx, d.words + rows, d.logprob, st));
     p->launches = n;
     return 0;
 }
@@ -264,6 +281,9 @@
             (!d.xa0_init && !d.emb_gate))
             return CVC_E_BADARG;
         if (d.emb_gate != nullptr && d.gsk_nwg > 0) return CVC_E_BADARG;
+        if (d.tail != 0 && (d.tail != 1 || !d.emb_gate || d.lang_ksx || !d.tail_keys || ((uintptr_t)d.tail_keys & 15) || !d.tail_ms || d.unk_idx < 0 ||
+                            cvc_gemm_packed_split(-1) != 2))
+            return CVC_E_BADARG;
         if (d.lang_ksx && (!d.ksx_slab || !d.ksx_flags || d.R != 2048 || d.T < 2 || d.gsk_nwg > 0)) return CVC_E_BADARG;
         if (d.gsk_nwg < 0 || (d.gsk_nwg > 0 && ((d.R & 63) || !d.slab_att || !d.slab_lang || !d.slab_q || !d.slab_o))) return CVC_E_BADARG;
     } else if (d.path == 1) {
diff --git a/cyclical-visual-captioning_amd/csrc/gemm_packed.hip b/cyclical-visual-captioning_amd/csrc/gemm_packed.hip
--- a/cyclical-visual-captioning_amd/csrc/gemm_packed.hip
+++ b/cyclical-visual-captioning_amd/csrc/gemm_packed.hip
@@ -2,6 +2,7 @@
 #include "gemm_split.h"
 #include "gsk.h"
 #include "dropout_rng.h"
+#include "sel_keys.h"
 
 struct PackedArgs {
     const float* wp;
@@ -42,6 +43,9 @@
     DropSpec h3_drop;
     long long wstride;
     GskSegs early;
+    unsigned long long* keys;
+    unsigned long long* key_unk;
+    float* ms_part;
 };
 
 #ifdef CVC_TS
@@ -96,8 +100,10 @@
     return s;
 }
 
-template <int MT, bool LSTM, int DEPTH, bool SPLIT, int NW, bool GRU = false, int NB = 1, bool SLAB = false, bool WC = false, bool WB16 = false>
+template <int MT, bool LSTM, int DEPTH, bool SPLIT, int NW, bool GRU = false, int NB = 1, bool SLAB = false, bool WC = false, bool WB16 = false,
+          bool KEYS = false>
 __global__ __launch_bounds__(NW * 64) void skinny_gemm_packed_kernel(PackedArgs a) {
+    static_assert(!KEYS || (SPLIT && NW == 8 && !GRU && NB == 1 && !SLAB && !WB16), "keys forms: 8-wave split-product form, fp32 weights");
     static_assert(!WB16 || (SPLIT && NW == 8 && !GRU && NB == 1 && !SLAB), "bf16-stored weights: 8-wave split-product form only");
     using Frag = std::conditional_t<WB16, BFrag<MT>, PFrag<MT>>;
     using WT = std::conditional_t<WB16, uint16_t, float>;
@@ -192,7 +198,20 @@
     if constexpr (LSTM && !GRU) {
         if (a.emb_gate != nullptr && tid < NB * 2 * 64) {
             const int em0 = tid & 63;
-            const long long eword = a.word[em0 < a.M ? em0 : a.M - 1];
+            long long eword;
+            if constexpr (KEYS) {
+                const int er = em0 < a.M ? em0 : a.M - 1;
+                unsigned long long kq[KEY_SLOTS];
+#pragma unroll
+                for (int s = 0; s < KEY_SLOTS; ++s) kq[s] = a.keys[s * KEY_ROWS + er];
+                const unsigned long long ku = a.key_unk[er];
+                unsigned long long kb = 0ull;
+#pragma unroll
+                for (int s = 0; s < KEY_SLOTS; ++s) kb = kq[s] > kb ? kq[s] : kb;
+                eword = sel_key_word(kb, ku, a.sel_unk);
+            } else {
+                eword = a.word[em0 < a.M ? em0 : a.M - 1];
+            }
             const float* trow = a.emb_gate + (size_t)eword * 4 * a.R + (size_t)((int)blockIdx.x * NB + (tid >> 7)) * 8 + ((tid >> 6) & 1) * 4;
 #pragma unroll
             for (int g = 0; g < 4; ++g) eadd4[g] = ld4(trow + (size_t)g * a.R);
@@ -374,7 +393,7 @@
 #pragma unroll
     for (int c = 0; c < ECPW; ++c) {
         const int n = (int)blockIdx.x * 32 + wave * ECPW + c;
-        ebias[c] = (!LSTM && a.top2_part != nullptr && a.bias != nullptr) ? a.bias[n < a.Nout ? n : a.Nout - 1] : 0.f;
+        ebias[c] = (!LSTM && (KEYS || a.top2_part != nullptr) && a.bias != nullptr) ? a.bias[n < a.Nout ? n : a.Nout - 1] : 0.f;
     }
 
 #pragma unroll
@@ -484,7 +503,48 @@
                 y[(size_t)m * a.ldy + n] = v;
             }
         }
-        if (a.top2_part != nullptr) {
+        if constexpr (KEYS) {
+            float* scratch = red + NW * 32 * LDM;
+            unsigned long long kb = 0ull, ku = 0ull;
+            float mx = -__builtin_inff(), se = 0.f;
+            const int m = lane < MT * 32 ? lane : MT * 32 - 1;
+            constexpr int CPW = 32 / NW;
+#pragma unroll
+            for (int c = 0; c < CPW; ++c) {
+                const int nl = wave * CPW + c, n = n0 + nl;
+                if (n >= a.Nout) break;
+                const float v = sum_partials<NW>(red, nl, LDM, m) + ebias[c];
+                const unsigned long long k = sel_key(v, n);
+                if (n == a.sel_unk) ku = k;
+                else kb = k > kb ? k : kb;
+                const float nm = fmaxf(mx, v);
+                se = se * __expf(mx - nm) + __expf(v - nm);
+                mx = nm;
+            }
+            float* r4 = scratch + ((size_t)wave * 64 + lane) * 6;
+            r4[0] = __uint_as_float((uint32_t)kb); r4[1] = __uint_as_float((uint32_t)(kb >> 32));
+            r4[2] = __uint_as_float((uint32_t)ku); r4[3] = __uint_as_float((uint32_t)(ku >> 32));
+            r4[4] = mx; r4[5] = se;
+            __syncthreads();
+            if (wave == 0 && lane < M) {
+                for (int w = 1; w < NW; ++w) {
+                    const float* q4 = scratch + ((size_t)w * 64 + lane) * 6;
+                    const unsigned long long k1 = ((unsigned long long)__float_as_uint(q4[1]) << 32) | __float_as_uint(q4[0]);
+                    const unsigned long long k2 = ((unsigned long long)__float_as_uint(q4[3]) << 32) | __float_as_uint(q4[2]);
+                    kb = k1 > kb ? k1 : kb;
+                    ku = k2 > ku ? k2 : ku;
+                    const float nm = fmaxf(mx, q4[4]);
+                    se = (nm == -__builtin_inff()) ? 0.f : se * __expf(mx - nm) + q4[5] * __expf(q4[4] - nm);
+                    mx = nm;
+                }
+                float* ms = a.ms_part + ((size_t)blockIdx.x * 64 + lane) * 2;
+                ms[0] = mx; ms[1] = se;
+                if (kb != 0ull)
+                    (void)__hip_atomic_fetch_max(a.keys + (blockIdx.x & (KEY_SLOTS - 1)) * KEY_ROWS + lane, kb, __ATOMIC_RELAXED,
+                                                 __HIP_MEMORY_SCOPE_AGENT);
+                if (ku != 0ull) a.key_unk[lane] = ku;
+            }
+        } else if (a.top2_part != nullptr) {
             float* scratch = red + NW * 32 * LDM;
             float v1 = -__builtin_inff(), v2 = -__builtin_inff(), mx = -__builtin_inff(), se = 0.f;
             int i1 = 0x7fffffff, i2 = 0x7fffffff;
@@ -959,6 +1019,49 @@
     return launch_packed<false>(a, (Nout + 31) / 32, (hipStream_t)stream);
 }
 
+extern "C" int cvc_packed_linear_keys_fwd(const float* wp, const float* xq, int K, const float* bias, int M, int Nout, int unk_idx,
+                                          unsigned long long* keys, unsigned long long* key_unk, float* ms_part, cvc_stream_t stream) {
+    if (!wp || !xq || (K & 31) || K < 32 || Nout < 1 || M < 1 || M > 64 || !keys || !key_unk || !ms_part || unk_idx < 0) return CVC_E_BADARG;
+    if (((uintptr_t)keys & 15) || ((uintptr_t)key_unk & 7)) return CVC_E_BADARG;
+    if (cvc_gemm_split_mode != 2) return CVC_E_BADARG;
+    PackedArgs a{};
+    a.wp = wp; a.xq = xq; a.nquad = K / 4; a.M = M; a.Nout = Nout; a.R = 0; a.wstride = (long long)a.nquad * 128;
+    a.bias = bias; a.ksplit = 1; a.sel_unk = unk_idx; a.keys = keys; a.key_unk = key_unk; a.ms_part = ms_part;
+    const dim3 grid((Nout + 31) / 32);
+    hipStream_t st = (hipStream_t)stream;
+    if (M <= 32) hipLaunchKernelGGL((skinny_gemm_packed_kernel<1, false, CVC_PACKED_DEPTH8, true, 8, false, 1, false, false, false, true>), grid, dim3(512), 0, st, a);
+    else hipLaunchKernelGGL((skinny_gemm_packed_kernel<2, false, CVC_PACKED_DEPTH8, true, 8, false, 1, false, false, false, true>), grid, dim3(512), 0, st, a);
+    return cvc_launch_status();
+}
+
+extern "C" int cvc_packed_lstm_embgate_keys_fwd(const float* wp, long long w_blk_stride, const float* xq, int K, const float* b_ih,
+                                                const float* b_hh, const float* gate_bias, const float* emb_gate,
+                                                const unsigned long long* keys, const unsigned long long* key_unk, int unk_idx,
+                                                const float* c_prev_q, int M, int R, float* h_dst1_q, float* h_dst2_q, float* c_out_q,
+                                                int w_cached, cvc_stream_t stream) {
+    if (!wp || !xq || !c_prev_q || !c_out_q || !emb_gate || !keys || !key_unk || (K & 31) || K < 32 || R < 8 || (R & 7) || M < 1 || M > 64 ||
+        unk_idx < 0)
+        return CVC_E_BADARG;
+    if (w_blk_stride != 0 && (w_blk_stride < (long long)(K / 4) * 128 || (w_blk_stride & 3))) return CVC_E_BADARG;
+    if (((uintptr_t)keys & 15) || ((uintptr_t)key_unk & 7)) return CVC_E_BADARG;
+    if (cvc_gemm_split_mode != 2) return CVC_E_BADARG;
+    PackedArgs a{};
+    a.wp = wp; a.xq = xq; a.nquad = K / 4; a.M = M; a.Nout = 4 * R; a.R = R; a.wstride = w_blk_stride ? w_blk_stride : (long long)a.nquad * 128;
+    a.bias = b_ih; a.bias2 = b_hh; a.gate_bias = gate_bias; a.c_prev_q = c_prev_q; a.c_out_q = c_out_q;
+    a.h_dst1_q = h_dst1_q; a.h_dst2_q = h_dst2_q; a.ksplit = 1; a.emb_gate = emb_gate; a.w_cached = w_cached ? 1 : 0;
+    a.keys = const_cast<unsigned long long*>(keys); a.key_unk = const_cast<unsigned long long*>(key_unk); a.sel_unk = unk_idx;
+    const dim3 grid(R / 8);
+    hipStream_t st = (hipStream_t)stream;
+    if (a.w_cached) {
+        if (M > 32) hipLaunchKernelGGL((skinny_gemm_packed_kernel<2, true, CVC_PACKED_DEPTH8, true, 8, false, 1, false, true, false, true>), grid, dim3(512), 0, st, a);
+        else hipLaunchKernelGGL((skinny_gemm_packed_kernel<1, true, CVC_PACKED_DEPTH8, true, 8, false, 1, false, true, false, true>), grid, dim3(512), 0, st, a);
+    } else {
+        if (M > 32) hipLaunchKernelGGL((skinny_gemm_packed_kernel<2, true, CVC_PACKED_DEPTH8, true, 8, false, 1, false, false, false, true>), grid, dim3(512), 0, st, a);
+        else hipLaunchKernelGGL((skinny_gemm_packed_kernel<1, true, CVC_PACKED_DEPTH8, true, 8, false, 1, false, false, false, true>), grid, dim3(512), 0, st, a);
+    }
+    return cvc_launch_status();
+}
+
 extern "C" int cvc_packed_linear_bf16w_fwd(const uint16_t* wp, const float* xq, int K, const float* bias, int M, int Nout,
                                            int ksplit, float* y, int ldy, float* top2_part, cvc_stream_t stream) {
     if (!wp || !xq || (K & 31) || K < 32 || Nout < 1 || ksplit < 1 || (!y && !top2_part) || M < 1 || M > 64) return CVC_E_BADARG;
diff --git a/cyclical-visual-captioning_amd/csrc/sel_keys.h b/cyclical-visual-captioning_amd/csrc/sel_keys.h
--- /dev/null
+++ b/cyclical-visual-captioning_amd/csrc/sel_keys.h
@@ -0,0 +1,21 @@
+#pragma once
+#include <stdint.h>
+
+constexpr int KEY_SLOTS = 4;
+constexpr int KEY_ROWS = 64;
+
+__device__ __forceinline__ unsigned long long sel_key(float v, int n) {
+    if (!(v > -__builtin_inff())) return 0ull;
+    uint32_t u = __float_as_uint(v);
+    if (u == 0x80000000u) u = 0u;
+    u = (u & 0x80000000u) ? ~u : (u | 0x80000000u);
+    return ((unsigned long long)u << 32) | (uint32_t)(0x7fffffff - n);
+}
+__device__ __forceinline__ float sel_key_value(unsigned long long k) {
+    const uint32_t u = (uint32_t)(k >> 32);
+    return __uint_as_float((u & 0x80000000u) ? (u & 0x7fffffffu) : ~u);
+}
+__device__ __forceinline__ int sel_key_index(unsigned long long k) { return 0x7fffffff - (int)(uint32_t)(k & 0xffffffffull); }
+__device__ __forceinline__ int sel_key_word(unsigned long long best, unsigned long long kunk, int unk) {
+    return best != 0ull ? sel_key_index(best) : (kunk != 0ull ? unk : 0);
+}
diff --git a/cyclical-visual-captioning_amd/csrc/vocab.hip b/cyclical-visual-captioning_amd/csrc/vocab.hip
--- a/cyclical-visual-captioning_amd/csrc/vocab.hip
+++ b/cyclical-visual-captioning_amd/csrc/vocab.hip
@@ -1,4 +1,5 @@
 #include "row_block.h"
+#include "sel_keys.h"
 #include "gsk.h"
 #include "dropout_rng.h"
 #include <math.h>
@@ -214,6 +215,32 @@
     }
 }
 
+__global__ __launch_bounds__(WG) void keys_finalize_kernel(const unsigned long long* keys, const unsigned long long* key_unk, const float* ms_part,
+                                                           int nblocks, int T, int rows, int unk, int64_t* words, float* logprob) {
+    __shared__ float red[4];
+    const int item = blockIdx.x;
+    const int t = item / rows, row = item - t * rows;
+    const float* ms = ms_part + ((size_t)t * nblocks * 64 + row) * 2;
+    float mx = -INFINITY;
+    for (int b = threadIdx.x; b < nblocks; b += WG) mx = fmaxf(mx, ms[(size_t)b * 128]);
+    mx = block_max(mx, red);
+    float se = 0.f;
+    for (int b = threadIdx.x; b < nblocks; b += WG) se += ms[(size_t)b * 128 + 1] * expf(ms[(size_t)b * 128] - mx);
+    se = block_sum(se, red);
+    if (threadIdx.x == 0) {
+        const unsigned long long* kp = keys + (size_t)t * KEY_SLOTS * KEY_ROWS + row;
+        unsigned long long kb = 0ull;
+#pragma unroll
+        for (int s = 0; s < KEY_SLOTS; ++s) kb = kp[s * KEY_ROWS] > kb ? kp[s * KEY_ROWS] : kb;
+        const unsigned long long ku = key_unk[(size_t)t * KEY_ROWS + row];
+        words[item] = sel_key_word(kb, ku, unk);
+        if (logprob != nullptr) {
+            const float v = kb != 0ull ? sel_key_value(kb) : (ku != 0ull ? sel_key_value(ku) : -INFINITY);
+            logprob[item] = v - (mx + logf(se));
+        }
+    }
+}
+
 template <int ITEMS>
 __global__ __launch_bounds__(WG) void top2_slab_kernel(GskSegs g, const float* bias, int V, int unk, int64_t* word, int wstride,
                                                        float* logprob, const float* table, int E, float* emb_out, int emb_ld) {
@@ -506,6 +533,14 @@
     if (emb_out != nullptr && (!table || E < 4 || (E & 3) || (emb_ld & 3) || (emb_ld != 0 && emb_ld < E))) return CVC_E_BADARG;
     hipLaunchKernelGGL(top2_final_kernel, dim3(M), dim3(WG), 0, (hipStream_t)stream, part, nblocks, unk_idx, word, word_stride,
                        logprob, table, E, emb_out, emb_ld);
+    return cvc_launch_status();
+}
+
+extern "C" int cvc_keys_finalize(const unsigned long long* keys, const unsigned long long* key_unk, const float* ms_part, int nblocks, int T,
+                                 int rows, int unk_idx, int64_t* words, float* logprob, cvc_stream_t stream) {
+    if (!keys || !key_unk || !ms_part || !words || nblocks < 1 || T < 1 || rows < 1 || rows > KEY_ROWS || unk_idx < 0) return CVC_E_BADARG;
+    hipLaunchKernelGGL(keys_finalize_kernel, dim3(T * rows), dim3(WG), 0, (hipStream_t)stream, keys, key_unk, ms_part, nblocks, T, rows,
+                       unk_idx, words, logprob);
     return cvc_launch_status();
 }
 
diff --git a/cyclical-visual-captioning_amd/cvc/decode/engine.py b/cyclical-visual-captioning_amd/cvc/decode/engine.py
--- a/cyclical-visual-captioning_amd/cvc/decode/engine.py
+++ b/cyclical-visual-captioning_amd/cvc/decode/engine.py
@@ -55,7 +55,7 @@
                  sample_n: int = 1, temperature: Optional[float] = None, seed: Optional[int] = None, weights_dtype: str = "fp32",
                  top_k: int = 0, top_p: float = 1.0, forced_n: int = 0, no_repeat_ngram: int = 0, no_immediate_repeat: bool = False,
                  min_len: int = 0, ban_words=None, bad_endings=None, beam_groups: int = 1, diversity: float = 0.0,
-                 length_penalty: float = 0.0, force_n: int = 0, beam_history: bool = False):
+                 length_penalty: float = 0.0, force_n: int = 0, tail: Optional[str] = None, beam_history: bool = False):
         W = self.W = weights
         self.T, self.unk, self.beam = int(T), int(unk_idx), int(beam)
         if weights_dtype not in WEIGHTS_DTYPES:
@@ -308,6 +308,21 @@
             self._alloc_packed()
         elif self.tile:
             self._alloc_tile()
+        fused_ok = (self.packed and self.embgate and not self.given and not self.bf16w and not self.gsk and not self.gate_ksplit and
+                    not self.lang_ksx and self.beam == 1 and self.unk >= 0 and hip.gemm_packed_split(-1) == 2)
+        if tail is None:
+            tail = TAIL_DEFAULT if fused_ok else "launch"
+        if tail not in TAILS:
+            raise RuntimeError(f"DecodeEngine: tail must be one of {TAILS} (or None), got {tail!r}")
+        if tail == "fused" and not fused_ok:
+            raise RuntimeError('DecodeEngine: tail="fused" covers plain greedy decode on the packed embedding-gate schedule only (beam = 1, '
+                               "<= 64 rows, fp32 weights, no sampling / forced / constrained mode, no gsk / gate_ksplit / lang_ksx, "
+                               "cvc_gemm_packed_split(2))")
+        self.tail = tail
+        self.fused_tail = tail == "fused"
+        if self.fused_tail:
+            self.tail_keys = torch.zeros(self.T * 64 * 5, dtype=torch.int64, device=dev)
+            self.tail_ms = z(self.T, (V + 31) // 32, 64, 2)
         self._launches = self._build_launches()
         if driver and not self.given and not self.bf16w and not self.beam_hist and (self.tile or (self.packed and not (self.ks_att or self.ks_lang))):
             self._bind_driver()
@@ -343,6 +358,8 @@
                 d.att_w_cached = int(self.att_w_cached)
             if self.lang_ksx:
                 d.lang_ksx, d.ksx_slab, d.ksx_flags = 1, ptr(self.ksx_slab), ptr(self.ksx_flags)
+            if self.fused_tail:
+                d.tail, d.tail_keys, d.tail_ms = 1, ptr(self.tail_keys), ptr(self.tail_ms)
             if self.gsk:
                 d.gsk_nwg = self.gsk_nwg
                 d.slab_att, d.slab_lang, d.slab_q, d.slab_o = (ptr(self.slab_att), ptr(self.slab_lang), ptr(self.slab_q),
@@ -394,6 +411,8 @@
             self.cA[0].zero_()
             self.cL[0].zero_()
             self.words[0].zero_()
+            if self.fused_tail:
+                self.tail_keys.zero_()
             return
         for bufs in (self.h_att, self.c_att, self.h_lang, self.c_lang):
             bufs[0].zero_()
@@ -598,7 +617,7 @@
             torch.cuda.current_stream().wait_stream(s)
             self.check_ksx()
         key = (self.packed, self.tile, self.beam > 1, self.sampling, self.weights_dtype, self.trunc, self.forced, self.constrained,
-               self.beam_hist, self.grouped, self.ranked, self.forcing)
+               self.beam_hist, self.grouped, self.ranked, self.forcing, self.fused_tail)
         if key not in DecodeEngine._warm:
             saved = self.rng.clone() if self.sampling else None
             s = torch.cuda.Stream()
diff --git a/cyclical-visual-captioning_amd/cvc/decode/path_packed.py b/cyclical-visual-captioning_amd/cvc/decode/path_packed.py
--- a/cyclical-visual-captioning_amd/cvc/decode/path_packed.py
+++ b/cyclical-visual-captioning_amd/cvc/decode/path_packed.py
@@ -138,14 +138,23 @@
         else:
             att_fn, linear_fn = L.cvc_packed_lstm_embgate_ex_fwd, L.cvc_packed_linear_fwd
             w_att, att_stride, embgate, w_h, w_o = W.p_att2, (2 * R // 4) * 128, W.t_embgate, W.p_h, W.p_o
+        fused = self.fused_tail
+        if fused:
+            key_at = lambda t: self.tail_keys.data_ptr() + t * 64 * 4 * 8
+            unk_at = lambda t: self.tail_keys.data_ptr() + (self.T * 64 * 4 + t * 64) * 8
         for t in range(self.T):
             rd, wr = t & 1, (t + 1) & 1
             XA_r, XA_w, XL_r, XL_w = self.XA[rd], self.XA[wr], self.XL[rd], self.XL[wr]
             first = t == 0 and (self.bf16w or hip.gemm_packed_split(-1) == 2)
-            out.append(("att_lstm", att_fn, (ptr(w_att), att_stride, ptr(XA_r), 32 if first else 2 * R, None, None,
-                                             ptr(self.gate_fc), ptr(embgate), ptr(self.words[t]), ptr(self.cA[rd]),
-                                             rows, R, qoff(XL_r, R), qoff(XA_w, R), ptr(self.cA[wr]),
-                                             1 if self.att_w_cached else 0)))
+            if fused and t > 0:
+                out.append(("att_lstm", L.cvc_packed_lstm_embgate_keys_fwd, (
+                    ptr(w_att), att_stride, ptr(XA_r), 2 * R, None, None, ptr(self.gate_fc), ptr(embgate), key_at(t - 1), unk_at(t - 1),
+                    self.unk, ptr(self.cA[rd]), rows, R, qoff(XL_r, R), qoff(XA_w, R), ptr(self.cA[wr]), 1 if self.att_w_cached else 0)))
+            else:
+                out.append(("att_lstm", att_fn, (ptr(w_att), att_stride, ptr(XA_r), 32 if first else 2 * R, None, None,
+                                                 ptr(self.gate_fc), ptr(embgate), ptr(self.words[t]), ptr(self.cA[rd]),
+                                                 rows, R, qoff(XL_r, R), qoff(XA_w, R), ptr(self.cA[wr]),
+                                                 1 if self.att_w_cached else 0)))
             out.append(("h2attn", linear_fn, (ptr(w_h), qoff(XL_r, R), R, None, rows, A, self.QSPLIT, ptr(self.q_parts), A, None)))
             sets = (hip.AttnSet * 2)()
             sets[0] = self._region_set(t)
@@ -172,9 +181,15 @@
             if self.given:
                 out.append(("logits", linear_fn, (ptr(w_o), ptr(XA_w), R, ptr(W.b_o), rows, V, 1, ptr(self.logits), V, None)))
                 out.append(self._word_select_sampled(t, ptr(self.logits), 1, 0, None))
+            elif fused:
+                out.append(("logits", L.cvc_packed_linear_keys_fwd, (ptr(w_o), ptr(XA_w), R, ptr(W.b_o), rows, V, self.unk, key_at(t),
+                                                                     unk_at(t), ptr(self.tail_ms[t]))))
             else:
                 out.append(("logits", linear_fn, (ptr(w_o), ptr(XA_w), R, ptr(W.b_o), rows, V, 1, None, V, ptr(self.top2_part))))
                 out.append(("word_select", L.cvc_top2_final, (ptr(self.top2_part), nblk_v, rows, self.unk, ptr(self.words[t + 1]), 1,
                                                               ptr(self.logprob[t]), None, 0, None, 0)))
             self._keep.append(sets)
+        if fused:
+            out.append(("tail_finalize", L.cvc_keys_finalize, (key_at(0), unk_at(0), ptr(self.tail_ms), nblk_v, self.T, rows, self.unk,
+                                                               ptr(self.words[1]), ptr(self.logprob))))
         return out
diff --git a/cyclical-visual-captioning_amd/cvc/decode/weights.py b/cyclical-visual-captioning_amd/cvc/decode/weights.py
--- a/cyclical-visual-captioning_amd/cvc/decode/weights.py
+++ b/cyclical-visual-captioning_amd/cvc/decode/weights.py
@@ -184,6 +184,10 @@
 
 CACHE_BUDGET = int(os.environ.get("CVC_CACHE_BUDGET_MB", "208")) << 20
 LANG_KSX_DEFAULT = os.environ.get("CVC_LANG_KSX", "0") == "1"
+TAILS = ("launch", "fused")
+TAIL_DEFAULT = os.environ.get("CVC_DECODE_TAIL", "fused")
+if TAIL_DEFAULT not in TAILS:
+    TAIL_DEFAULT = "fused"
 CACHE_LANG_GATE_WEIGHTS = os.environ.get("CVC_LANG_W_CACHED", "1") != "0"
 CACHE_GATE_WEIGHTS = os.environ.get("CVC_ATT_W_CACHED", "1") != "0"
 
diff --git a/cyclical-visual-captioning_amd/cvc/hip.py b/cyclical-visual-captioning_amd/cvc/hip.py
--- a/cyclical-visual-captioning_amd/cvc/hip.py
+++ b/cyclical-visual-captioning_amd/cvc/hip.py
@@ -67,7 +67,8 @@
         [(n, C.c_void_p) for n in ("h_att", "c_att", "h_lang", "c_lang", "c_att_prev", "c_lang_prev", "zero_state")] +
         [("beam_ws", C.c_void_p)] +
         [("gsk_nwg", C.c_int)] + [(n, C.c_void_p) for n in ("slab_att", "slab_lang", "slab_q", "slab_o", "emb_gate", "sel_counter")] +
-        [("att_w_cached", C.c_int), ("lang_ksx", C.c_int), ("ksx_slab", C.c_void_p), ("ksx_flags", C.c_void_p)])
+        [("att_w_cached", C.c_int), ("lang_ksx", C.c_int), ("ksx_slab", C.c_void_p), ("ksx_flags", C.c_void_p)] +
+        [("tail", C.c_int), ("tail_keys", C.c_void_p), ("tail_ms", C.c_void_p)])
 
 class GradSrc(C.Structure):
     _fields_ = [("p", C.c_void_p), ("ld", C.c_longlong), ("plane_stride", C.c_longlong), ("nplanes", C.c_int)]
@@ -236,6 +237,9 @@
     "cvc_beam_rank_force": [_P, _LL, _P, _P, _I, _I, _I, _I, _I, _I, _F, _P, _P, _P, _P, _P],
     "cvc_packed_lstm_bf16w_fwd": [_P, _LL, _P, _I, _P, _P, _P, _P, _P, _P, _I, _I, _P, _P, _P, _I, _P],
     "cvc_packed_linear_bf16w_fwd": [_P, _P, _I, _P, _I, _I, _I, _P, _I, _P, _P],
+    "cvc_packed_linear_keys_fwd": [_P, _P, _I, _P, _I, _I, _I, _P, _P, _P, _P],
+    "cvc_packed_lstm_embgate_keys_fwd": [_P, _LL, _P, _I, _P, _P, _P, _P, _P, _P, _I, _P, _I, _I, _P, _P, _P, _I, _P],
+    "cvc_keys_finalize": [_P, _P, _P, _I, _I, _I, _I, _P, _P, _P],
     "cvc_gather_rows": [_P, _P, _I, _I, _I, _P, _P],
     "cvc_tile_rows_alloc": [_I],
     "cvc_tile_gemm_loaders": [_I],
@@ -275,7 +279,8 @@
     "cvc_tile_gemm_loaders", "cvc_gru_persistent_waves8", "cvc_relu_dropout_fwd", "cvc_relu_dropout_bwd", "cvc_bn_workspace",
     "cvc_bn_relu_train_fwd", "cvc_bn_relu_train_bwd", "cvc_class_softmax_bwd", "cvc_layernorm_cat_bwd", "cvc_stable_order", "cvc_col_sum", "cvc_col_sum_ws", "cvc_attn_weighted_rows",
     "cvc_lstm_persistent_sync_words", "cvc_lstm_seq_persistent_fwd", "cvc_lstm_seq_persistent_train_fwd", "cvc_lstm_seq_fwd", "cvc_lstm_seq_train_fwd", "cvc_lstm_seq_bwd_work", "cvc_lstm_seq_bwd",
-    "cvc_packed_lstm_bf16w_fwd", "cvc_packed_linear_bf16w_fwd"}
+    "cvc_packed_lstm_bf16w_fwd", "cvc_packed_linear_bf16w_fwd",
+    "cvc_packed_linear_keys_fwd", "cvc_packed_lstm_embgate_keys_fwd", "cvc_keys_finalize"}
 EXPERIMENTAL = {
     "cvc_gsk_plan", "cvc_gsk_gemm", "cvc_attn_scores_qslab", "cvc_top2_slab", "cvc_packed_lstm_ks_slices", "cvc_packed_lstm_ks_fwd",
     "cvc_packed_lstm_ksf_fwd", "cvc_packed_lstm_ksx_local", "cvc_packed_lstm_ksx_fwd", "cvc_packed_lstm_wg_blocks",
diff --git a/include/cvc_hip.h b/include/cvc_hip.h
--- a/include/cvc_hip.h
+++ b/include/cvc_hip.h
@@ -240,6 +240,9 @@
     int lang_ksx;
     float* ksx_slab;
     unsigned* ksx_flags;
+    int tail;
+    unsigned long long* tail_keys;
+    float* tail_ms;
 } cvc_decode_desc;
 typedef struct cvc_decode_plan cvc_decode_plan;
 CVC_API int cvc_decode_plan_create(const cvc_decode_desc* desc, cvc_decode_plan** plan);
diff --git a/include/cvc_hip_blocks.h b/include/cvc_hip_blocks.h
--- a/include/cvc_hip_blocks.h
+++ b/include/cvc_hip_blocks.h
@@ -206,6 +206,16 @@
 int cvc_packed_linear_bf16w_fwd(const uint16_t* wp, const float* xq, int K, const float* bias, int M, int Nout, int ksplit,
                                 float* y, int ldy, float* top2_part, cvc_stream_t stream);
 
+int cvc_packed_linear_keys_fwd(const float* wp, const float* xq, int K, const float* bias, int M, int Nout, int unk_idx,
+                               unsigned long long* keys, unsigned long long* key_unk, float* ms_part, cvc_stream_t stream);
+int cvc_packed_lstm_embgate_keys_fwd(const float* wp, long long w_blk_stride, const float* xq, int K, const float* b_ih,
+                                     const float* b_hh, const float* gate_bias, const float* emb_gate,
+                                     const unsigned long long* keys, const unsigned long long* key_unk, int unk_idx,
+                                     const float* c_prev_q, int M, int R, float* h_dst1_q, float* h_dst2_q, float* c_out_q,
+                                     int w_cached, cvc_stream_t stream);
+int cvc_keys_finalize(const unsigned long long* keys, const unsigned long long* key_unk, const float* ms_part, int nblocks, int T,
+                      int rows, int unk_idx, int64_t* words, float* logprob, cvc_stream_t stream);
+
 #ifdef __cplusplus
 }
 #endif
```

New measurement: 338,700 decode-steps/s (median of 6 runs). 1.02x the previous value.
